# jac0626/Neighbor-Aware-Reinforcement-Learning-Fosters-Cooperation-in-Spatial-Public-Goods-Games-

Measured on NVIDIA B200. Metric: site-updates/s, higher is better.
Workload: dtype f32

## Files before the change

### neighbor-aware-reinforcement-learning-fosters-cooperation-in-spatial-public-goods-games-_b200/csrc/spgg_capi.cu

```cuda
#include "../../include/spgg.h"
#include "spgg_kernels.cuh"
#include "spgg_dispatch.h"
#include "spgg_fast.cuh"
#include "spgg_resident.cuh"

#include <cudaTypedefs.h>

#include <algorithm>
#include <cmath>
#include <cstdarg>
#include <cstdio>
#include <cstdlib>
#include <cstring>
#include <memory>
#include <string>
#include <vector>

using namespace spgg;

static thread_local std::string g_err;

static int fail(int code, const char *fmt, ...) {
  char buf[512];
  va_list ap;
  va_start(ap, fmt);
  vsnprintf(buf, sizeof(buf), fmt, ap);
  va_end(ap);
  g_err = buf;
  return code;
}

#define CUDA_TRY(expr)                                                                  \
  do {                                                                                  \
    cudaError_t e_ = (expr);                                                            \
    if (e_ != cudaSuccess)                                                              \
      return fail(SPGG_E_CUDA, "%s failed: %s (%s:%d)", #expr, cudaGetErrorString(e_),  \
                  __FILE__, __LINE__);                                                  \
  } while (0)


struct spgg_handle {
  int device = 0;
  int n_rep = 1;
  int mode = MODE_F32_I8;
  int M = 1;
  int action = 0;
  std::vector<spgg_params_t> params;
  std::vector<RepConst> rc_host;
  Geom g{};
  int threads = 256;
  int gmax_ctas = 1;
  size_t smem_step = 0, smem_gmax = 0;
  RepConst *d_rc = nullptr;
  double *d_valtab = nullptr;
  bool lean = false;
  int gmax_ctas_gen = 1;
  void *d_Qb[2] = {nullptr, nullptr};
  int qcur = 0;
  void *Qcur() const { return d_Qb[qcur]; }
  bool spec = false;
  bool carry_valid = false;
  float *d_gcarry = nullptr;
  int *d_bad = nullptr;
  CUtensorMap qmaps[2];
  bool spec_on = true;
  long long spec_launches = 0, spec_failures = 0;
  long long spec_iterations = 0;
  bool in_rerun = false;
  float *d_gvec = nullptr;
  void *peer_code[2][2] = {{nullptr, nullptr}, {nullptr, nullptr}};
  void *peer_R[2][2] = {{nullptr, nullptr}, {nullptr, nullptr}};
  uint32_t *peer_S[2][2] = {{nullptr, nullptr}, {nullptr, nullptr}};
  int peer_rows[2] = {0, 0};
  bool peer_on = false;
  std::vector<void *> ipc_opened;
  unsigned *d_ring = nullptr;
  unsigned *ring_peer[SPGG_MAX_RING] = {nullptr};
  int ring_world = 0;
  int gen = 0;
  int last_gen = -1;
  int last_rel = -1, last_upd = 0, last_spec = 0, last_sel = 0;
  int pend_qcur0 = 0;
  std::vector<char> pend_cur_after, pend_q_after;
  void *d_R[2] = {nullptr, nullptr};
  void *d_code[2] = {nullptr, nullptr};
  uint32_t *d_S[2] = {nullptr, nullptr};
  int cur = 0;
  void *d_gmax = nullptr;
  double *d_stats = nullptr;
  double *d_partials = nullptr;
  unsigned *d_tickets = nullptr;
  int *d_stop = nullptr;
  double *d_eps = nullptr;
  uint32_t *d_thr = nullptr;
  int cap = 0;
  double *d_u = nullptr;
  uint8_t *d_b = nullptr;
  uint8_t *d_sc_S = nullptr;
  double *d_sc_R = nullptr, *d_sc_Q = nullptr;
  unsigned long long *d_sc_info = nullptr;
  bool fast = false;
  bool r_wide = false;
  FastMaps fmaps[2];
  bool resident = false;
  ResGeom rgeo{};
  size_t smem_res = 0;
  bool pend_resident = false;
  bool res_grid = false;
  unsigned char *d_gimg = nullptr;
  double *d_gpart = nullptr;
  unsigned *d_gnsel = nullptr;
  int gnsel_cap = 0;
  std::vector<double> eps_host;
  std::vector<uint32_t> thr_host;
  int replay_pairs = 1;
  long long replay_first = 0, replay_n = 0;
  long long iter = 0;
  std::vector<double> eps_cur;
  std::vector<long long> stop_at;
  std::vector<char> stale;
  long long launches = 0;
  bool pending = false;
  long long pend_t0 = 0;
  int pend_n = 0, pend_cur0 = 0, pend_rel = 0;
  cudaStream_t pend_stream = nullptr;
  CclScratch ccl;
  bool ccl_valid = false;
  int64_t ccl_n = 0;
  CclStripScratch ccl_strip;
  bool ccl_local = false;
  int ccl_which = 0, ccl_flags = 0;
  int64_t ccl_local_n = 0;
  unsigned long long *d_pair_cnt = nullptr;
  uint32_t *d_pair_tail = nullptr;
  size_t pair_cnt_n = 0, pair_tail_n = 0;
  void *d_blk = nullptr;
  size_t blk_bytes = 0;
  size_t elem_code() const { return mode == MODE_F64 ? 4 : 1; }
  size_t elem_R() const { return mode == MODE_F64 ? 8 : (mode == MODE_F32_F ? 4 : 1); }
  size_t elem_Q() const { return mode == MODE_F64 ? 8 : 4; }
  size_t elem_val() const { return mode == MODE_F64 ? 8 : 4; }
  int nq() const { return params[0].algorithm == SPGG_ALGO_DOUBLE_QLEARNING ? 8 : 4; }
  ~spgg_handle();
};

static bool int8_quantum(const spgg_params_t &p, double *rq, int *gi, int *li, int *mn, int *mx) {
  for (int k = 0; k <= 4; ++k) {
    const double s = (double)(1 << k);
    const double a = p.rep_gain_C * s, b = p.delta_R_D * s, c = p.R_min * s, d = p.R_max * s;
    if (a == std::floor(a) && b == std::floor(b) && c == std::floor(c) && d == std::floor(d) &&
        std::fabs(c) <= 127 && std::fabs(d) <= 127 && std::fabs(a) <= 127 && std::fabs(b) <= 127 &&
        c - b >= -128 && d + a <= 127) {
      *rq = 1.0 / s; *gi = (int)a; *li = (int)b; *mn = (int)c; *mx = (int)d;
      return true;
    }
  }
  return false;
}

static void build_repconst(const spgg_params_t &p, RepConst *rc) {
  memset(rc, 0, sizeof(*rc));
  rc->rc = p.r * p.c;
  for (int n = 0; n < 6; ++n) rc->g[n] = rc->rc * (double)n / 5.0;
  rc->cost = p.cost;
  rc->lo = p.r - 5.0;
  rc->span = 4.0 * p.r - rc->lo;
  rc->wP = p.wP;
  rc->wR = 1.0 - p.wP;
  rc->alpha = p.alpha; rc->gamma = p.gamma; rc->kappa = p.kappa; rc->leps = p.lambda_eps;
  rc->gainC = p.rep_gain_C; rc->lossD = p.delta_R_D; rc->rmin = p.R_min; rc->rmax = p.R_max;
  rc->alpha_f = (float)p.alpha; rc->gamma_f = (float)p.gamma; rc->kappa_f = (float)p.kappa;
  rc->leps_f = (float)p.lambda_eps;
  rc->gainC_f = (float)p.rep_gain_C; rc->lossD_f = (float)p.delta_R_D;
  rc->rmin_f = (float)p.R_min; rc->rmax_f = (float)p.R_max;
  rc->rq = 1.0;
  int8_quantum(p, &rc->rq, &rc->gain_i, &rc->loss_i, &rc->rmin_i, &rc->rmax_i);
  rc->seed_lo = (uint32_t)p.seed;
  rc->seed_hi = (uint32_t)(p.seed >> 32);
  for (uint32_t r = 0; r < 10; ++r) {
    rc->pkeys[2 * r] = rc->seed_lo + r * 0x9E3779B9u;
    rc->pkeys[2 * r + 1] = rc->seed_hi + r * 0xBB67AE85u;
  }
  rc->has_ratio = (rc->wR != 0.0);
  for (int code = 0; code < 128; ++code) {
    const int sn = code >> 2, C = (code >> 1) & 1, coop = code & 1;
    const double tot = rc->rc * (double)sn / 5.0 - (C ? 5.0 * p.cost : 0.0);
    const double P = (tot - rc->lo) / rc->span;
    const double rew = rc->wP * P + rc->wR * (coop ? 0.5 : 0.0);
    rc->rewtab[code] = (float)rew;
    rc->ratiotab[code] =
        coop ? (float)(std::fabs(rc->wR * 0.5) / (std::fabs(rew) + 1e-9) * 100.0) : 0.0f;
  }
}

template <class F>
static auto with_mode(int mode, F &&f) {
  switch (mode) {
    case MODE_F32_I8: return f(ModeF32I8{});
    case MODE_F32_F: return f(ModeF32F{});
    default: return f(ModeF64{});
  }
}

static size_t step_smem(int mode, int TR) {
  return with_mode(mode, [&](auto md) { return SmemLayout<decltype(md)>(TR).total; });
}

template <class... KArgsT, class... Args>
static cudaError_t launch_pdl(void (*kern)(KArgsT...), int grid, int block, size_t smem, cudaStream_t st,
                              Args... args) {
  cudaLaunchConfig_t cfg = {};
  cfg.gridDim = dim3((unsigned)grid);
  cfg.blockDim = dim3((unsigned)block);
  cfg.dynamicSmemBytes = smem;
  cfg.stream = st;
  cudaLaunchAttribute attr[1];
  attr[0].id = cudaLaunchAttributeProgrammaticStreamSerialization;
  attr[0].val.programmaticStreamSerializationAllowed = 1;
  cfg.attrs = attr;
  cfg.numAttrs = 1;
  return cudaLaunchKernelEx(&cfg, kern, args...);
}

typedef void (*fast_fn_t)(const FastMaps, KArgs);
template <int M, bool ACTION, bool PART>
static fast_fn_t pick_fast3(int upd, int sel) {
  if (upd) return sel ? k_step_fast<M, ACTION, true, true, PART> : k_step_fast<M, ACTION, true, false, PART>;
  return k_step_fast<M, ACTION, false, true, PART>;
}
template <int M, bool ACTION>
static fast_fn_t pick_fast2(int upd, int sel, bool part) {
  return part ? pick_fast3<M, ACTION, true>(upd, sel) : pick_fast3<M, ACTION, false>(upd, sel);
}
static fast_fn_t pick_fast(int M, int action, int upd, int sel, bool part) {
  if (M == 2) return action ? pick_fast2<2, true>(upd, sel, part) : pick_fast2<2, false>(upd, sel, part);
  return action ? pick_fast2<1, true>(upd, sel, part) : pick_fast2<1, false>(upd, sel, part);
}
static size_t fast_smem(int M) { return M == 2 ? FastSmem<2>::kTotal : FastSmem<1>::kTotal; }
typedef void (*gfast_fn_t)(const CUtensorMap, GArgs);
static gfast_fn_t pick_gfast(int M) { return M == 2 ? k_gmax_fast<2> : k_gmax_fast<1>; }
static size_t gfast_smem(int M) { return M == 2 ? GmaxSmem<2>::kTotal : GmaxSmem<1>::kTotal; }

typedef void (*res_fn_t)(RArgs);
template <bool FULL>
static res_fn_t pick_res2(int M, int action) {
  if (M == 2) return action ? k_resident<2, true, FULL> : k_resident<2, false, FULL>;
  return action ? k_resident<1, true, FULL> : k_resident<1, false, FULL>;
}
static res_fn_t pick_res(int M, int action, int L) {
  return (L % 4 == 0) ? pick_res2<true>(M, action) : pick_res2<false>(M, action);
}
template <bool FULL>
static res_fn_t pick_resg2(int M, int action) {
  if (M == 2) return action ? k_resident<2, true, FULL, true> : k_resident<2, false, FULL, true>;
  return action ? k_resident<1, true, FULL, true> : k_resident<1, false, FULL, true>;
}
static res_fn_t pick_res_grid(int M, int action, int L) {
  return (L % 4 == 0) ? pick_resg2<true>(M, action) : pick_resg2<false>(M, action);
}
static ResGeom resident_geom(int L, int cs, size_t smem_limit, int grid = 0) {
  ResGeom rg{};
  rg.grid = grid;
  if (L < 2 * cs) cs = 1;
  rg.rows_max = (L + cs - 1) / cs;
  rg.prow = rg.rows_max + 4;
  rg.QR = (L + 3) / 4;
  rg.pitch = (RG + rg.QR * 4 + RG + 15) / 16 * 16;
  const int quads = rg.rows_max * rg.QR;
  rg.threads = std::max(64, std::min(RES_THREADS, (quads + 31) / 32 * 32));
  rg.CS = (ResSmem(rg).total <= smem_limit) ? cs : 0;
  return rg;
}

static PFN_cuTensorMapEncodeTiled_v12000 tensor_map_encoder() {
  static PFN_cuTensorMapEncodeTiled_v12000 encode = nullptr;
  if (!encode) {
    void *fn = nullptr;
    cudaDriverEntryPointQueryResult q;
    const cudaError_t e = cudaGetDriverEntryPoint("cuTensorMapEncodeTiled", &fn, cudaEnableDefault, &q);
    if (e != cudaSuccess || !fn || q != cudaDriverEntryPointSuccess) {
      fail(SPGG_E_CUDA, "cuTensorMapEncodeTiled not available (%s)", cudaGetErrorString(e));
      return nullptr;
    }
    encode = (PFN_cuTensorMapEncodeTiled_v12000)fn;
  }
  return encode;
}

static int make_map(CUtensorMap *map, void *base, uint64_t row_bytes, uint64_t n_rows, uint64_t n_rep,
                    uint64_t rep_stride_bytes, uint32_t box_bytes, uint32_t box_rows, uint64_t visible_bytes = 0) {
  const PFN_cuTensorMapEncodeTiled_v12000 encode = tensor_map_encoder();
  if (!encode) return SPGG_E_CUDA;
  const cuuint64_t dims[3] = {visible_bytes ? visible_bytes : row_bytes, n_rows, n_rep};
  const cuuint64_t strides[2] = {row_bytes, rep_stride_bytes};
  const cuuint32_t box[3] = {box_bytes, box_rows, 1};
  const cuuint32_t estr[3] = {1, 1, 1};
  CUresult r = encode(map, CU_TENSOR_MAP_DATA_TYPE_UINT8, 3, base, dims, strides, box, estr,
                      CU_TENSOR_MAP_INTERLEAVE_NONE, CU_TENSOR_MAP_SWIZZLE_NONE,
                      CU_TENSOR_MAP_L2_PROMOTION_L2_128B, CU_TENSOR_MAP_FLOAT_OOB_FILL_NONE);
  if (r != CUDA_SUCCESS) return fail(SPGG_E_CUDA, "cuTensorMapEncodeTiled failed (%d)", (int)r);
  return SPGG_OK;
}

static int make_map_q(CUtensorMap *map, void *base, uint64_t L, uint64_t n_rows, uint64_t n_rep) {
  const PFN_cuTensorMapEncodeTiled_v12000 encode = tensor_map_encoder();
  if (!encode) return SPGG_E_CUDA;
  const cuuint64_t dims[4] = {128, L / 8, n_rows, n_rep};
  const cuuint64_t strides[3] = {128, L * 16, n_rows * L * 16};
  const cuuint32_t box[4] = {128, TC / 8, (cuuint32_t)FastSmem<1>::kRowsPerWarp, 1};
  const cuuint32_t estr[4] = {1, 1, 1, 1};
  CUresult r = encode(map, CU_TENSOR_MAP_DATA_TYPE_UINT8, 4, base, dims, strides, box, estr,
                      CU_TENSOR_MAP_INTERLEAVE_NONE, CU_TENSOR_MAP_SWIZZLE_128B,
                      CU_TENSOR_MAP_L2_PROMOTION_L2_128B, CU_TENSOR_MAP_FLOAT_OOB_FILL_NONE);
  if (r != CUDA_SUCCESS) return fail(SPGG_E_CUDA, "cuTensorMapEncodeTiled (Q) failed (%d)", (int)r);
  return SPGG_OK;
}

extern "C" int spgg_abi_version(void) { return SPGG_ABI_VERSION; }
extern "C" const char *spgg_last_error(void) { return g_err.c_str(); }

spgg_handle::~spgg_handle() {
  for (void *p : ipc_opened) cudaIpcCloseMemHandle(p);
  cudaFree(d_rc); cudaFree(d_valtab); cudaFree(d_Qb[0]); cudaFree(d_Qb[1]); cudaFree(d_gcarry); cudaFree(d_bad); cudaFree(d_gvec); cudaFree(d_ring);
  for (int i = 0; i < 2; ++i) { cudaFree(d_R[i]); cudaFree(d_code[i]); cudaFree(d_S[i]); }
  cudaFree(d_gmax); cudaFree(d_stats); cudaFree(d_partials); cudaFree(d_tickets);
  cudaFree(d_stop); cudaFree(d_eps); cudaFree(d_thr); cudaFree(d_u); cudaFree(d_b);
  cudaFree(d_sc_S); cudaFree(d_sc_R); cudaFree(d_sc_Q); cudaFree(d_sc_info);
  cudaFree(d_gimg); cudaFree(d_gpart); cudaFree(d_gnsel);
  ccl_free(&ccl);
  ccl_strip_free(&ccl_strip);
  cudaFree(d_pair_cnt); cudaFree(d_pair_tail);
  cudaFree(d_blk);
}

extern "C" void spgg_destroy(spgg_t *h) {
  if (!h) return;
  cudaSetDevice(h->device);
  cudaDeviceSynchronize();
  delete h;
}

extern "C" int spgg_create(const spgg_params_t *params, int n_replicas, int device, spgg_t **out) {
  if (!params || !out || n_replicas < 1) return fail(SPGG_E_INVALID, "spgg_create: null argument or n_replicas < 1");
  const spgg_params_t &p0 = params[0];
  if (p0.L < 4) return fail(SPGG_E_INVALID, "L must be >= 4 (got %d)", p0.L);
  if (p0.rows < 2 * GH || p0.rows > p0.L)
    return fail(SPGG_E_INVALID, "rows must be in [%d, L] (got %d)", 2 * GH, p0.rows);
  if (p0.M != 1 && p0.M != 2) return fail(SPGG_E_INVALID, "M must be 1 or 2 (got %d)", p0.M);
  if (p0.state_mode != SPGG_STATE_REPUTATION && p0.state_mode != SPGG_STATE_ACTION)
    return fail(SPGG_E_INVALID, "Unknown state_representation code %d", p0.state_mode);
  if (p0.precision != SPGG_PREC_FP32 && p0.precision != SPGG_PREC_FP64)
    return fail(SPGG_E_INVALID, "unknown precision %d", p0.precision);
  if (p0.algorithm != SPGG_ALGO_QLEARNING && p0.algorithm != SPGG_ALGO_SARSA &&
      p0.algorithm != SPGG_ALGO_EXPECTED_SARSA && p0.algorithm != SPGG_ALGO_DOUBLE_QLEARNING)
    return fail(SPGG_E_UNSUPPORTED, "algorithm code %d is not built into the fused kernel", p0.algorithm);
  if (p0.row0 < 0 || p0.row0 + p0.rows > p0.L) return fail(SPGG_E_INVALID, "row0/rows outside the lattice");
  for (int r = 1; r < n_replicas; ++r) {
    const spgg_params_t &p = params[r];
    if (p.L != p0.L || p.rows != p0.rows || p.row0 != p0.row0 || p.M != p0.M ||
        p.state_mode != p0.state_mode || p.precision != p0.precision ||
        p.algorithm != p0.algorithm || p.r_storage != p0.r_storage)
      return fail(SPGG_E_INVALID, "replica %d differs in a batch-invariant field (L, rows, M, state, precision)", r);
  }
  int ndev = 0;
  CUDA_TRY(cudaGetDeviceCount(&ndev));
  if (device < 0 || device >= ndev) return fail(SPGG_E_CUDA, "device %d not available (%d devices)", device, ndev);
  CUDA_TRY(cudaSetDevice(device));

  std::unique_ptr<spgg_handle> hp(new spgg_handle());
  spgg_handle *h = hp.get();
  h->device = device;
  h->n_rep = n_replicas;
  h->params.assign(params, params + n_replicas);
  h->M = p0.M;
  h->action = p0.state_mode == SPGG_STATE_ACTION;
  h->rc_host.resize(n_replicas);
  bool all_i8 = true;
  for (int r = 0; r < n_replicas; ++r) {
    build_repconst(params[r], &h->rc_host[r]);
    double rq; int a, b, c, d;
    all_i8 = all_i8 && int8_quantum(params[r], &rq, &a, &b, &c, &d);
  }
  if (p0.precision == SPGG_PREC_FP64) h->mode = MODE_F64;
  else if (p0.r_storage == SPGG_RSTORE_FP32) h->mode = MODE_F32_F;
  else if (p0.r_storage == SPGG_RSTORE_INT8) {
    if (!all_i8) return fail(SPGG_E_INVALID, "reputation parameters are not representable in int8 units");
    h->mode = MODE_F32_I8;
  } else h->mode = all_i8 ? MODE_F32_I8 : MODE_F32_F;

  Geom &g = h->g;
  g.L = p0.L; g.rows = p0.rows; g.row0 = p0.row0; g.wrap_rows = (p0.rows == p0.L);
  g.pitchB = CPAD + (p0.L + 15) / 16 * 16 + CPAD;
  g.pitchW = WPAD + ((p0.L + 31) / 32 + 3) / 4 * 4 + WPAD;
  {
    bool ok = (h->mode == MODE_F32_I8) && (g.L % 32 == 0) && (g.L >= TC) && (g.rows % FTR == 0) &&
              p0.algorithm == SPGG_ALGO_QLEARNING && getenv("SPGG_NO_FAST") == nullptr;
    for (int r = 0; r < n_replicas && ok; ++r)
      ok = h->rc_host[r].rmin_i >= -15 && h->rc_host[r].rmax_i <= 15 && h->rc_host[r].gain_i >= 0 &&
           h->rc_host[r].loss_i >= 0;
    h->fast = ok;
  }
  {
    cudaDeviceProp prop0;
    CUDA_TRY(cudaGetDeviceProperties(&prop0, device));
    res_fn_t rf = pick_res(h->M, h->action, h->g.L);
    cudaFuncAttributes fa;
    CUDA_TRY(cudaFuncGetAttributes(&fa, rf));
    const size_t lim = prop0.sharedMemPerBlockOptin - fa.sharedSizeBytes - 1024;
    const bool eligible = (h->mode == MODE_F32_I8) && g.wrap_rows && p0.row0 == 0 &&
                          p0.algorithm == SPGG_ALGO_QLEARNING && getenv("SPGG_NO_RESIDENT") == nullptr;
    ResGeom rg = resident_geom(g.L, 8, lim);
    if (eligible && g.L >= 32 && (rg.CS == 0 || n_replicas <= 4) && getenv("SPGG_RES_CS8") == nullptr) {
      const ResGeom rg16 = resident_geom(g.L, 16, lim);
      if (rg16.CS == 16 &&
          cudaFuncSetAttribute(rf, cudaFuncAttributeNonPortableClusterSizeAllowed, 1) == cudaSuccess &&
          cudaFuncSetAttribute(rf, cudaFuncAttributeMaxDynamicSharedMemorySize, (int)lim) == cudaSuccess) {
        cudaLaunchConfig_t cfg = {};
        cfg.gridDim = dim3(16u * (unsigned)n_replicas);
        cfg.blockDim = dim3((unsigned)rg16.threads);
        cfg.dynamicSmemBytes = ResSmem(rg16).total;
        cudaLaunchAttribute attr[1];
        attr[0].id = cudaLaunchAttributeClusterDimension;
        attr[0].val.clusterDim.x = 16; attr[0].val.clusterDim.y = 1; attr[0].val.clusterDim.z = 1;
        cfg.attrs = attr; cfg.numAttrs = 1;
        int n_clusters = 0;
        if (cudaOccupancyMaxActiveClusters(&n_clusters, rf, &cfg) == cudaSuccess && n_clusters >= 1) rg = rg16;
      }
      (void)cudaGetLastError();
    }
    h->resident = eligible && rg.CS > 0;
    if (h->resident) {
      h->rgeo = rg;
      h->smem_res = ResSmem(rg).total;
      CUDA_TRY(cudaFuncSetAttribute(rf, cudaFuncAttributeMaxDynamicSharedMemorySize, (int)lim));
    } else if (eligible && n_replicas == 1 && getenv("SPGG_NO_RESIDENT_GRID") == nullptr) {
      res_fn_t gf = pick_res_grid(h->M, h->action, h->g.L);
      cudaFuncAttributes gfa;
      CUDA_TRY(cudaFuncGetAttributes(&gfa, gf));
      const size_t glim = prop0.sharedMemPerBlockOptin - gfa.sharedSizeBytes - 1024;
      int coop = 0;
      CUDA_TRY(cudaDeviceGetAttribute(&coop, cudaDevAttrCooperativeLaunch, device));
      const int nb_ctas = std::min(prop0.multiProcessorCount, g.L / 2);
      ResGeom gg = resident_geom(g.L, nb_ctas, glim, 1);
      if (coop && nb_ctas >= RES_RING && gg.CS == nb_ctas &&
          cudaFuncSetAttribute(gf, cudaFuncAttributeMaxDynamicSharedMemorySize, (int)glim) == cudaSuccess) {
        int occ_g = 0;
        if (cudaOccupancyMaxActiveBlocksPerMultiprocessor(&occ_g, gf, gg.threads, ResSmem(gg).total) == cudaSuccess &&
            (long long)occ_g * prop0.multiProcessorCount >= nb_ctas) {
          h->resident = true;
          h->res_grid = true;
          h->rgeo = gg;
          h->smem_res = ResSmem(gg).total;
        }
      }
      (void)cudaGetLastError();
    }
  }
  g.TR = h->fast ? FTR : (g.rows >= 512 ? 16 : (g.rows >= 64 ? 8 : 4));
  h->threads = h->fast ? FTHREADS : 32 * std::min(8, g.TR);
  g.n_tx = (g.L + TC - 1) / TC;
  g.n_ty = (g.rows + g.TR - 1) / g.TR;
  g.n_rep = n_replicas;
  g.plane_stride = (long long)(g.rows + 2 * GH) * g.pitchB;
  g.bits_stride = (long long)(g.rows + 2 * GH) * g.pitchW;
  g.site_stride = (long long)g.rows * g.L;
  h->smem_step = step_smem(h->mode, g.TR);
  h->smem_gmax = (h->elem_val() * (size_t)(g.TR + 2 * HR) * SMW + 15) / 16 * 16 + 512;

  cudaDeviceProp prop;
  CUDA_TRY(cudaGetDeviceProperties(&prop, device));
  int occ = 1;
  h->lean = !h->fast && p0.algorithm == 0 && getenv("SPGG_NO_LEAN") == nullptr;
  if (h->lean) h->smem_step = step_smem(h->mode, LEAN_TR_MAX);
  for (int replay = 0; replay < 2; ++replay) {
    step_fn_t f = pick_step(h->mode, h->M, h->action, replay);
    CUDA_TRY(cudaFuncSetAttribute(f, cudaFuncAttributeMaxDynamicSharedMemorySize, (int)h->smem_step));
    if (!replay)
      CUDA_TRY(cudaOccupancyMaxActiveBlocksPerMultiprocessor(&occ, f, h->threads, h->smem_step));
    if (h->lean) {
      step_fn_t fl = pick_lean(h->mode, h->M, h->action, replay);
      CUDA_TRY(cudaFuncSetAttribute(fl, cudaFuncAttributeMaxDynamicSharedMemorySize, (int)h->smem_step));
      if (!replay)
        CUDA_TRY(cudaOccupancyMaxActiveBlocksPerMultiprocessor(&occ, fl, h->threads, h->smem_step));
    }
  }
  if (h->fast) {
    for (int v = 0; v < 3; ++v) {
      fast_fn_t fv = pick_fast(h->M, h->action, v != 2, v != 1, g.L % TC != 0);
      CUDA_TRY(cudaFuncSetAttribute(fv, cudaFuncAttributeMaxDynamicSharedMemorySize, (int)fast_smem(h->M)));
    }
    fast_fn_t ff = pick_fast(h->M, h->action, 1, 1, g.L % TC != 0);
    CUDA_TRY(cudaOccupancyMaxActiveBlocksPerMultiprocessor(&occ, ff, FTHREADS, fast_smem(h->M)));
    CUDA_TRY(cudaFuncSetAttribute(pick_gfast(h->M), cudaFuncAttributeMaxDynamicSharedMemorySize, (int)gfast_smem(h->M)));
    int gocc = 1;
    CUDA_TRY(cudaOccupancyMaxActiveBlocksPerMultiprocessor(&gocc, pick_gfast(h->M), GWARPS * 32, gfast_smem(h->M)));
    const long long n_tiles_g = (long long)((p0.L + TC - 1) / TC) * (p0.rows / FTR);
    h->gmax_ctas = (int)std::max<long long>(1, std::min<long long>((n_tiles_g + GWARPS - 1) / GWARPS,
                       ((long long)prop.multiProcessorCount * std::max(1, gocc)) / n_replicas));
  }
  CUDA_TRY(cudaFuncSetAttribute(pick_gmax_lean(h->mode, h->M), cudaFuncAttributeMaxDynamicSharedMemorySize,
                                (int)h->smem_gmax));
  if (occ < 1) return fail(SPGG_E_CUDA, "kernel does not fit on an SM (smem %zu)", h->smem_step);
  const long long n_tiles = (long long)g.n_tx * g.n_ty;
  long long per_rep = std::max<long long>(1, ((long long)prop.multiProcessorCount * occ) / n_replicas);
  g.ctas_per_rep = (int)std::min<long long>(n_tiles, per_rep);
  {
    int gocc = 1;
    CUDA_TRY(cudaOccupancyMaxActiveBlocksPerMultiprocessor(&gocc, pick_gmax_lean(h->mode, h->M), h->threads, h->smem_gmax));
    h->gmax_ctas_gen = (int)std::min<long long>(n_tiles, std::max<long long>(1, ((long long)prop.multiProcessorCount * std::max(1, gocc)) / n_replicas));
  }
  if (h->fast && (g.site_stride / ((long long)g.ctas_per_rep * FTHREADS)) > 60000) h->fast = false;
  h->spec = h->fast && getenv("SPGG_NO_SPEC") == nullptr;

  const size_t nQ = (size_t)n_replicas * g.site_stride * h->nq() * h->elem_Q();
  const size_t nR = (size_t)n_replicas * g.plane_stride * h->elem_R();
  const size_t nC = (size_t)n_replicas * g.plane_stride * h->elem_code();
  const size_t nS = (size_t)n_replicas * g.bits_stride * 4;
#define ALLOC(ptr, bytes)                                                                   \
  do {                                                                                      \
    cudaError_t e_ = cudaMalloc((void **)&(ptr), (bytes));                                  \
    if (e_ != cudaSuccess)                                                                  \
      return fail(SPGG_E_CUDA, "cudaMalloc(%zu bytes) failed: %s", (size_t)(bytes), cudaGetErrorString(e_)); \
    cudaMemset((ptr), 0, (bytes));                                                          \
  } while (0)
  ALLOC(h->d_rc, sizeof(RepConst) * n_replicas);
  ALLOC(h->d_Qb[0], nQ);
  if (h->spec) { ALLOC(h->d_Qb[1], nQ); ALLOC(h->d_gcarry, sizeof(float) * n_replicas); ALLOC(h->d_bad, sizeof(int)); }
  for (int i = 0; i < 2; ++i) { ALLOC(h->d_R[i], nR); ALLOC(h->d_code[i], nC); ALLOC(h->d_S[i], nS); }
  ALLOC(h->d_partials, sizeof(double) * (size_t)n_replicas * g.ctas_per_rep * NSTAT);
  ALLOC(h->d_tickets, sizeof(unsigned) * n_replicas);
  ALLOC(h->d_stop, sizeof(int) * n_replicas);
  if (h->res_grid) {
    ALLOC(h->d_gimg, (size_t)h->rgeo.CS * 6 * h->rgeo.prow * h->rgeo.pitch);
    ALLOC(h->d_gpart, sizeof(double) * (size_t)RES_RING * h->rgeo.CS * RES_NRED);
  }
#undef ALLOC
  if (h->fast) {
    const int rowsCR = FTR + 2 * h->M, rowsS = FTR + 4;
    const uint64_t nrows = (uint64_t)(g.rows + 2 * GH);
    for (int i = 0; i < 2; ++i) {
      FastMaps &fm = h->fmaps[i];
      int e = make_map(&fm.ld_code, h->d_code[i], (uint64_t)g.pitchB, nrows, n_replicas, (uint64_t)g.plane_stride, FROWB, rowsCR);
      if (!e) e = make_map(&fm.ld_R, h->d_R[i], (uint64_t)g.pitchB, nrows, n_replicas, (uint64_t)g.plane_stride, FROWB, rowsCR);
      if (!e) e = make_map(&fm.ld_S, h->d_S[i], (uint64_t)g.pitchW * 4, nrows, n_replicas, (uint64_t)g.bits_stride * 4, FSROWB, rowsS);
      if (!e) e = make_map(&fm.st_code, h->d_code[i ^ 1], (uint64_t)g.pitchB, nrows, n_replicas, (uint64_t)g.plane_stride, TC, FTR, (uint64_t)(CPAD + g.L));
      if (!e) e = make_map(&fm.st_R, h->d_R[i ^ 1], (uint64_t)g.pitchB, nrows, n_replicas, (uint64_t)g.plane_stride, TC, FTR, (uint64_t)(CPAD + g.L));
      if (!e) e = make_map(&fm.st_S, h->d_S[i ^ 1], (uint64_t)g.pitchW * 4, nrows, n_replicas, (uint64_t)g.bits_stride * 4, TC / 8, FTR);
      if (!e) e = make_map_q(&h->qmaps[i], h->d_Qb[(i == 1 && h->spec) ? 1 : 0], (uint64_t)g.L, (uint64_t)g.rows, (uint64_t)n_replicas);
      if (e) return e;
    }
  }
  CUDA_TRY(cudaMemcpy(h->d_rc, h->rc_host.data(), sizeof(RepConst) * n_replicas, cudaMemcpyHostToDevice));
  if (h->mode == MODE_F64) {
    const size_t vb = sizeof(double) * 2 * ((size_t)n_replicas << VALTAB_BITS);
    if (cudaMalloc((void **)&h->d_valtab, vb) != cudaSuccess)
      return fail(SPGG_E_CUDA, "cudaMalloc(%zu bytes) failed (reward table)", vb);
    CUDA_TRY(launch_build_valtab(h->d_rc, h->d_valtab, n_replicas));
  }
  std::vector<int> neg(n_replicas, -1);
  CUDA_TRY(cudaMemcpy(h->d_stop, neg.data(), sizeof(int) * n_replicas, cudaMemcpyHostToDevice));
  if (h->spec) {
    const int none = 0x7fffffff;
    CUDA_TRY(cudaMemcpy(h->d_bad, &none, sizeof(int), cudaMemcpyHostToDevice));
  }
  h->eps_cur.resize(n_replicas);
  for (int r = 0; r < n_replicas; ++r) h->eps_cur[r] = params[r].epsilon;
  h->stop_at.assign(n_replicas, -1);
  h->stale.assign(n_replicas, 0);
  *out = hp.release();
  return SPGG_OK;
}

static int launch_step(spgg_handle *h, int do_update, int do_select, cudaStream_t st, bool allow_spec);

static int rewind_to_failed_launch(spgg_handle *h, int bad) {
  h->spec_failures += 1;
  if (h->spec_failures > 8 && h->spec_failures * 16 > h->spec_iterations) h->spec_on = false;
  const int none = 0x7fffffff;
  CUDA_TRY(cudaMemcpy(h->d_bad, &none, sizeof(int), cudaMemcpyHostToDevice));
  std::vector<int> stop(h->n_rep);
  CUDA_TRY(cudaMemcpy(stop.data(), h->d_stop, sizeof(int) * h->n_rep, cudaMemcpyDeviceToHost));
  for (int r = 0; r < h->n_rep; ++r)
    if (stop[r] == (int)(h->pend_t0 + bad) + 1) stop[r] = -1;
  CUDA_TRY(cudaMemcpy(h->d_stop, stop.data(), sizeof(int) * h->n_rep, cudaMemcpyHostToDevice));
  h->cur = h->pend_cur_after[bad - 1];
  h->qcur = h->pend_q_after[bad - 1];
  h->carry_valid = true;
  h->pend_rel = bad - 1;
  return SPGG_OK;
}

static int rerun_failed_speculation(spgg_handle *h) {
  for (;;) {
    int bad = 0x7fffffff;
    CUDA_TRY(cudaMemcpy(&bad, h->d_bad, sizeof(int), cudaMemcpyDeviceToHost));
    if (bad == 0x7fffffff) return SPGG_OK;
    if (bad < 1 || bad > h->pend_n) return fail(SPGG_E_STATE, "speculation bookkeeping out of range (%d of %d)", bad, h->pend_n);
    int rcode0 = rewind_to_failed_launch(h, bad);
    if (rcode0) return rcode0;
    h->in_rerun = true;
    const int n = h->pend_n;
    for (int s = bad; s <= n; ++s) {
      h->pend_rel += 1;
      int rcode = launch_step(h, 1, s < n ? 1 : 0, h->pend_stream, true);
      if (rcode) return rcode;
      if (!h->spec_on && s < n) {
        for (++s; s <= n; ++s) {
          rcode = spgg_phase_gmax(h, h->pend_stream);
          if (!rcode) rcode = launch_step(h, 1, s < n ? 1 : 0, h->pend_stream, false);
          if (rcode) return rcode;
        }
      }
    }
    h->in_rerun = false;
    CUDA_TRY(cudaStreamSynchronize(h->pend_stream));
    CUDA_TRY(cudaGetLastError());
  }
}

static int finish_pending(spgg_handle *h) {
  if (!h->pending) return SPGG_OK;
  CUDA_TRY(cudaSetDevice(h->device));
  CUDA_TRY(cudaStreamSynchronize(h->pend_stream));
  CUDA_TRY(cudaGetLastError());
  if (h->spec && h->g.wrap_rows && h->pend_rel == h->pend_n && !h->pend_resident) {
    int rcode = rerun_failed_speculation(h);
    if (rcode) return rcode;
  }
  std::vector<int> stop(h->n_rep);
  CUDA_TRY(cudaMemcpy(stop.data(), h->d_stop, sizeof(int) * h->n_rep, cudaMemcpyDeviceToHost));
  const long long t_end = h->pend_t0 + h->pend_rel;
  for (int r = 0; r < h->n_rep; ++r) {
    h->stop_at[r] = stop[r];
    const long long done = (stop[r] >= 0 && stop[r] < t_end) ? (long long)stop[r] : t_end;
    double e = h->eps_cur[r];
    for (long long t = h->pend_t0; t < done; ++t)
      e = std::max(e * h->params[r].epsilon_decay, h->params[r].epsilon_min);
    h->eps_cur[r] = e;
  }
  if (h->pend_resident) {
    h->iter = (h->n_rep == 1 && stop[0] >= 0 && stop[0] < t_end) ? (long long)stop[0] : t_end;
    h->pend_resident = false;
  } else if (h->n_rep == 1 && stop[0] >= 0 && stop[0] < t_end) {
    h->cur = h->pend_cur0 ^ (int)((stop[0] - h->pend_t0) & 1);
    h->qcur = h->pend_q_after[(size_t)(stop[0] - h->pend_t0)];
    h->iter = stop[0];
  } else {
    if (h->n_rep > 1) {
      for (int r = 0; r < h->n_rep; ++r) {
        if (stop[r] >= 0 && stop[r] < t_end) {
          const long long k = (long long)stop[r] - h->pend_t0;
          const int src = k >= 0 ? (h->pend_cur0 ^ (int)(k & 1)) : h->pend_cur0;
          if (src != h->cur) {
            const Geom &g = h->g;
            CUDA_TRY(cudaMemcpy((char *)h->d_R[h->cur] + (size_t)r * g.plane_stride * h->elem_R(),
                                (char *)h->d_R[src] + (size_t)r * g.plane_stride * h->elem_R(),
                                (size_t)g.plane_stride * h->elem_R(), cudaMemcpyDeviceToDevice));
            CUDA_TRY(cudaMemcpy(h->d_S[h->cur] + (size_t)r * g.bits_stride,
                                h->d_S[src] + (size_t)r * g.bits_stride,
                                (size_t)g.bits_stride * 4, cudaMemcpyDeviceToDevice));
          }
          const int qsrc = k >= 0 ? h->pend_q_after[(size_t)k] : h->pend_qcur0;
          if (qsrc != h->qcur) {
            const size_t qb = (size_t)h->g.site_stride * h->nq() * h->elem_Q();
            CUDA_TRY(cudaMemcpy((char *)h->d_Qb[h->qcur] + (size_t)r * qb, (char *)h->d_Qb[qsrc] + (size_t)r * qb, qb,
                                cudaMemcpyDeviceToDevice));
          }
        }
      }
    }
    h->iter = t_end;
  }
  h->pending = false;
  return SPGG_OK;
}

extern "C" int spgg_sync(spgg_t *h) {
  if (!h) return fail(SPGG_E_INVALID, "null handle");
  return finish_pending(h);
}

static int stage_rows(const spgg_handle *h) {
  const long long budget = 32ll << 20;
  return (int)std::max<long long>(1, std::min<long long>(h->g.rows, budget / h->g.L));
}

static int ensure_scratch(spgg_handle *h, bool want_q) {
  const size_t n = (size_t)stage_rows(h) * h->g.L;
  if (!h->d_sc_S) {
    CUDA_TRY(cudaMalloc((void **)&h->d_sc_S, n));
    CUDA_TRY(cudaMalloc((void **)&h->d_sc_R, n * sizeof(double)));
    CUDA_TRY(cudaMalloc((void **)&h->d_sc_info, 3 * sizeof(unsigned long long)));
  }
  if (want_q && !h->d_sc_Q) CUDA_TRY(cudaMalloc((void **)&h->d_sc_Q, n * h->nq() * sizeof(double)));
  return SPGG_OK;
}

static void begin_new_run(spgg_handle *h, int rep) {
  if (h->iter != 0) {
    h->iter = 0;
    std::fill(h->stale.begin(), h->stale.end(), 1);
  }
  h->stale[rep] = 0;
  h->carry_valid = false;
  if (h->d_ring) {
    cudaMemset(h->d_ring, 0, sizeof(unsigned) * RING_SLOTS * RING_WORDS);
    h->gen = 0;
    h->last_gen = -1;
  }
}

extern "C" int spgg_set_state(spgg_t *h, int rep, const uint8_t *S, const double *R, const double *Q) {
  if (!h || !S || !R || !Q) return fail(SPGG_E_INVALID, "spgg_set_state: null argument");
  if (rep < 0 || rep >= h->n_rep) return fail(SPGG_E_INVALID, "replica %d out of range", rep);
  int rcode = finish_pending(h);
  if (rcode) return rcode;
  h->ccl_valid = h->ccl_local = false;
  CUDA_TRY(cudaSetDevice(h->device));
  rcode = ensure_scratch(h, true);
  if (rcode) return rcode;
  const Geom &g = h->g;
  const RepConst &rc = h->rc_host[rep];
  CUDA_TRY(cudaMemset(h->d_sc_info, 0, 3 * sizeof(unsigned long long)));
  const int chunk = stage_rows(h);
  for (int i0 = 0; i0 < g.rows; i0 += chunk) {
    const int nr = std::min(chunk, g.rows - i0);
    const size_t n = (size_t)nr * g.L, off = (size_t)i0 * g.L;
    CUDA_TRY(cudaMemcpyAsync(h->d_sc_S, S + off, n, cudaMemcpyHostToDevice, 0));
    CUDA_TRY(cudaMemcpyAsync(h->d_sc_R, R + off, n * sizeof(double), cudaMemcpyHostToDevice, 0));
    CUDA_TRY(cudaMemcpyAsync(h->d_sc_Q, Q + off * h->nq(), n * h->nq() * sizeof(double), cudaMemcpyHostToDevice, 0));
    const int grid = (int)std::min<long long>(148 * 16, ((long long)nr * ((g.L + 31) / 32) * 32 + 255) / 256);
    with_mode(h->mode, [&](auto md) {
      k_import_rows<decltype(md)><<<std::max(1, grid), 256>>>(g, rep, i0, nr, h->d_sc_S, h->d_sc_R, h->d_sc_Q,
          h->Qcur(), h->d_R[h->cur], h->d_S[h->cur], rc.rq, h->d_sc_info, h->nq());
    });
    CUDA_TRY(cudaGetLastError());
    h->launches += 1;
  }
  unsigned long long info[3];
  CUDA_TRY(cudaMemcpy(info, h->d_sc_info, sizeof(info), cudaMemcpyDeviceToHost));
  if (info[0] == 1) return fail(SPGG_E_INVALID, "strategy array holds values other than 0/1");
  if (info[0] == 2)
    return fail(SPGG_E_INVALID, "R is not representable in int8 units of %g; use r_storage=FP32", rc.rq);
  if (info[2] && h->fast) {
    if (!g.wrap_rows)
      return fail(SPGG_E_INVALID, "R outside [%g, %g] (int8 units -16..15 of %g): a strip on the fast path "
                  "cannot hold it", -16.0 * rc.rq, 15.0 * rc.rq, rc.rq);
    h->r_wide = true;
  }
  begin_new_run(h, rep);
  h->eps_cur[rep] = h->params[rep].epsilon;
  int stop = -1;
  if (g.wrap_rows && (info[1] == 0 || info[1] == (unsigned long long)g.site_stride))
    stop = (int)h->iter;
  h->stop_at[rep] = stop;
  CUDA_TRY(cudaMemcpy(h->d_stop + rep, &stop, sizeof(int), cudaMemcpyHostToDevice));
  return SPGG_OK;
}

extern "C" int spgg_get_state(spgg_t *h, int rep, uint8_t *S, double *R, double *Q) {
  if (!h) return fail(SPGG_E_INVALID, "null handle");
  if (rep < 0 || rep >= h->n_rep) return fail(SPGG_E_INVALID, "replica %d out of range", rep);
  int rcode = finish_pending(h);
  if (rcode) return rcode;
  CUDA_TRY(cudaSetDevice(h->device));
  rcode = ensure_scratch(h, Q != nullptr);
  if (rcode) return rcode;
  const Geom &g = h->g;
  const RepConst &rc = h->rc_host[rep];
  const int chunk = stage_rows(h);
  for (int i0 = 0; i0 < g.rows; i0 += chunk) {
    const int nr = std::min(chunk, g.rows - i0);
    const size_t n = (size_t)nr * g.L, off = (size_t)i0 * g.L;
    const int grid = (int)std::min<long long>(148 * 16, ((long long)n + 255) / 256);
    with_mode(h->mode, [&](auto md) {
      k_export_rows<decltype(md)><<<std::max(1, grid), 256>>>(g, rep, i0, nr, S ? h->d_sc_S : nullptr,
          R ? h->d_sc_R : nullptr, Q ? h->d_sc_Q : nullptr, h->Qcur(), h->d_R[h->cur], h->d_S[h->cur], rc.rq, h->nq());
    });
    CUDA_TRY(cudaGetLastError());
    h->launches += 1;
    if (S) CUDA_TRY(cudaMemcpyAsync(S + off, h->d_sc_S, n, cudaMemcpyDeviceToHost, 0));
    if (R) CUDA_TRY(cudaMemcpyAsync(R + off, h->d_sc_R, n * sizeof(double), cudaMemcpyDeviceToHost, 0));
    if (Q) CUDA_TRY(cudaMemcpyAsync(Q + off * h->nq(), h->d_sc_Q, n * h->nq() * sizeof(double), cudaMemcpyDeviceToHost, 0));
    CUDA_TRY(cudaStreamSynchronize(0));
  }
  return SPGG_OK;
}

extern "C" int spgg_set_replay(spgg_t *h, int n_steps, const double *u, const uint8_t *b) {
  return spgg_set_replay_pairs(h, n_steps, 1, u, b);
}

extern "C" int spgg_set_replay_pairs(spgg_t *h, int n_steps, int n_pairs, const double *u, const uint8_t *b) {
  if (!h) return fail(SPGG_E_INVALID, "null handle");
  const int want_pairs = h->params[0].algorithm == SPGG_ALGO_SARSA ? 3
                         : (h->params[0].algorithm == SPGG_ALGO_DOUBLE_QLEARNING ? 2 : 1);
  if (n_steps > 0 && n_pairs != want_pairs)
    return fail(SPGG_E_INVALID, "this TD rule consumes %d draw pair(s) per iteration, got %d", want_pairs, n_pairs);
  if (h->n_rep != 1) return fail(SPGG_E_UNSUPPORTED, "replay draws are supported for a single replica");
  int rcode = finish_pending(h);
  if (rcode) return rcode;
  CUDA_TRY(cudaSetDevice(h->device));
  cudaFree(h->d_u); cudaFree(h->d_b);
  h->d_u = nullptr; h->d_b = nullptr; h->replay_n = 0;
  if (n_steps <= 0) return SPGG_OK;
  if (!u || !b) return fail(SPGG_E_INVALID, "spgg_set_replay: null draw arrays");
  const size_t n = (size_t)n_steps * n_pairs * h->g.site_stride;
  h->replay_pairs = n_pairs;
  CUDA_TRY(cudaMalloc((void **)&h->d_u, n * sizeof(double)));
  CUDA_TRY(cudaMalloc((void **)&h->d_b, n));
  CUDA_TRY(cudaMemcpy(h->d_u, u, n * sizeof(double), cudaMemcpyHostToDevice));
  CUDA_TRY(cudaMemcpy(h->d_b, b, n, cudaMemcpyHostToDevice));
  h->replay_first = h->iter;
  h->replay_n = n_steps;
  return SPGG_OK;
}

static int ensure_tables(spgg_handle *h, int n_steps) {
  const int need = n_steps + 1;
  if (need <= h->cap) return SPGG_OK;
  cudaFree(h->d_gmax); cudaFree(h->d_stats); cudaFree(h->d_eps); cudaFree(h->d_thr); cudaFree(h->d_gvec);
  h->d_gmax = nullptr; h->d_stats = nullptr; h->d_eps = nullptr; h->d_thr = nullptr; h->d_gvec = nullptr;
  h->cap = 0;
  CUDA_TRY(cudaMalloc(&h->d_gmax, h->elem_val() * (size_t)h->n_rep * need));
  CUDA_TRY(cudaMalloc((void **)&h->d_stats, sizeof(double) * (size_t)h->n_rep * need * NSTAT));
  CUDA_TRY(cudaMalloc((void **)&h->d_eps, sizeof(double) * (size_t)h->n_rep * (need + 1)));
  CUDA_TRY(cudaMalloc((void **)&h->d_thr, sizeof(uint32_t) * (size_t)h->n_rep * (need + 1)));
  if (h->spec && !h->g.wrap_rows) CUDA_TRY(cudaMalloc((void **)&h->d_gvec, sizeof(float) * 4 * (size_t)need));
  h->cap = need;
  return SPGG_OK;
}

static uint32_t thr24(double eps) {
  double t = std::ceil(eps * 16777216.0);
  if (t < 0) t = 0;
  if (t > 16777216.0) t = 16777216.0;
  return (uint32_t)t;
}

extern "C" int spgg_begin_steps(spgg_t *h, int n_steps, void *stream_) {
  if (!h) return fail(SPGG_E_INVALID, "null handle");
  if (n_steps < 1) return fail(SPGG_E_INVALID, "n_steps must be >= 1");
  int rcode = finish_pending(h);
  if (rcode) return rcode;
  h->ccl_valid = h->ccl_local = false;
  for (int r = 0; r < h->n_rep; ++r)
    if (h->stale[r])
      return fail(SPGG_E_STATE, "replica %d still holds the state of the previous run: give every replica of a "
                                "batch a state (spgg_set_state / spgg_init_random) before stepping", r);
  CUDA_TRY(cudaSetDevice(h->device));
  cudaStream_t st = (cudaStream_t)stream_;
  rcode = ensure_tables(h, n_steps);
  if (rcode) return rcode;
  std::vector<double> &eps = h->eps_host;
  std::vector<uint32_t> &thr = h->thr_host;
  eps.assign((size_t)(h->cap + 1) * h->n_rep, 0.0);
  thr.assign(eps.size(), 0u);
  for (int r = 0; r < h->n_rep; ++r) {
    double e = h->eps_cur[r];
    for (int idx = 1; idx <= n_steps + 1 && idx <= h->cap; ++idx) {
      eps[(size_t)idx * h->n_rep + r] = e;
      thr[(size_t)idx * h->n_rep + r] = thr24(e);
      e = std::max(e * h->params[r].epsilon_decay, h->params[r].epsilon_min);
    }
  }
  CUDA_TRY(cudaMemcpyAsync(h->d_eps, eps.data(), eps.size() * sizeof(double), cudaMemcpyHostToDevice, st));
  CUDA_TRY(cudaMemcpyAsync(h->d_thr, thr.data(), thr.size() * sizeof(uint32_t), cudaMemcpyHostToDevice, st));
  CUDA_TRY(cudaMemsetAsync(h->d_gmax, 0, h->elem_val() * (size_t)h->n_rep * h->cap, st));
  CUDA_TRY(cudaMemsetAsync(h->d_stats, 0, sizeof(double) * (size_t)h->n_rep * h->cap * NSTAT, st));
  if (h->d_gvec) CUDA_TRY(cudaMemsetAsync(h->d_gvec, 0, sizeof(float) * 4 * (size_t)h->cap, st));
  h->pending = true;
  h->pend_t0 = h->iter;
  h->pend_n = n_steps;
  h->pend_cur0 = h->cur;
  h->pend_qcur0 = h->qcur;
  h->in_rerun = false;
  h->pend_cur_after.assign((size_t)n_steps + 1, (char)h->cur);
  h->pend_q_after.assign((size_t)n_steps + 1, (char)h->qcur);
  h->pend_rel = 0;
  h->pend_stream = st;
  return SPGG_OK;
}

static bool launch_replays(const spgg_handle *h, long long j, int do_select) {
  const long long draw = j - h->replay_first;
  return do_select && h->d_u && draw >= 0 && draw < h->replay_n;
}
static bool can_speculate(const spgg_handle *h, int do_select) {
  return h->fast && h->spec && h->spec_on && h->carry_valid &&
         !launch_replays(h, h->pend_t0 + h->pend_rel + 1, do_select);
}

static int launch_step(spgg_handle *h, int do_update, int do_select, cudaStream_t st, bool allow_spec) {
  const long long j = h->pend_t0 + h->pend_rel;
  const long long draw = j - h->replay_first;
  const bool replay = launch_replays(h, j, do_select);
  KArgs a;
  a.g = h->g;
  a.rc = h->d_rc;
  a.Q = h->Qcur();
  a.R_in = h->d_R[h->cur]; a.R_out = h->d_R[h->cur ^ 1];
  a.code_in = h->d_code[h->cur]; a.code_out = h->d_code[h->cur ^ 1];
  a.S_in = h->d_S[h->cur]; a.S_out = h->d_S[h->cur ^ 1];
  a.gmax = h->d_gmax; a.stats = h->d_stats; a.partials = h->d_partials;
  a.valtab = h->d_valtab;
  a.tickets = h->d_tickets; a.stop_at = h->d_stop;
  a.eps_tab = h->d_eps; a.thr_tab = h->d_thr;
  const size_t np_ = (size_t)h->replay_pairs, ss = (size_t)h->g.site_stride;
  a.u = replay ? h->d_u + (size_t)draw * np_ * ss : nullptr;
  a.b = replay ? h->d_b + (size_t)draw * np_ * ss : nullptr;
  a.algo = h->params[0].algorithm;
  const long long ue = j - 1 - h->replay_first;
  const bool upd_replay = do_update && np_ >= 2 && h->d_u && ue >= 0 && ue < h->replay_n;
  a.u2 = upd_replay ? h->d_u + ((size_t)ue * np_ + 1) * ss : nullptr;
  a.b2 = upd_replay ? h->d_b + ((size_t)ue * np_ + 1) * ss : nullptr;
  a.u3 = (upd_replay && np_ == 3) ? h->d_u + ((size_t)ue * 3 + 2) * ss : nullptr;
  a.b3 = (upd_replay && np_ == 3) ? h->d_b + ((size_t)ue * 3 + 2) * ss : nullptr;
  a.j = (int)j; a.rel = h->pend_rel; a.cap = h->cap;
  a.do_update = do_update; a.do_select = do_select;
  const bool use_fast = h->fast && !replay && !(do_select && h->r_wide);
  a.spec = 0; a.gcarry = nullptr; a.bad_at = nullptr; a.gvec = nullptr;
  for (int d = 0; d < 2; ++d) {
    const bool on = h->peer_on && use_fast && do_select;
    a.peer_code[d] = on ? h->peer_code[d][h->cur ^ 1] : nullptr;
    a.peer_R[d] = on ? h->peer_R[d][h->cur ^ 1] : nullptr;
    a.peer_S[d] = on ? h->peer_S[d][h->cur ^ 1] : nullptr;
    a.peer_rows[d] = h->peer_rows[d];
  }
  a.ring_world = 0; a.gen = 0;
  for (int p = 0; p < SPGG_MAX_RING; ++p) a.ring_peer[p] = nullptr;
  if (h->ring_world > 0 && use_fast && h->d_gvec && (do_update || do_select)) {
    a.ring_world = h->ring_world;
    a.gen = h->gen;
    for (int p = 0; p < h->ring_world; ++p) a.ring_peer[p] = h->ring_peer[p];
  }
  if (use_fast && h->spec && !h->g.wrap_rows && h->n_rep == 1) a.gvec = h->d_gvec;
  if (use_fast && h->spec) {
    a.gcarry = h->d_gcarry;
    a.bad_at = h->d_bad;
    a.spec = (allow_spec && do_update && h->spec_on && h->carry_valid) ? 1 : 0;
  }
#ifdef SPGG_TRACE
  {
    static unsigned long long *d_trace = nullptr;
    static int n_dump = 0;
    const int n_cta = h->g.ctas_per_rep * h->n_rep;
    if (!d_trace) { cudaMalloc(&d_trace, sizeof(unsigned long long) * 4 * 65536); cudaMemset(d_trace, 0, sizeof(unsigned long long) * 4 * 65536); }
    else if (getenv("SPGG_TRACE_FILE") && n_dump < 3 && do_update && do_select) {
      std::vector<unsigned long long> t(4 * (size_t)n_cta);
      cudaDeviceSynchronize();
      cudaMemcpy(t.data(), d_trace, t.size() * 8, cudaMemcpyDeviceToHost);
      char name[256]; snprintf(name, sizeof(name), "%s.%d", getenv("SPGG_TRACE_FILE"), n_dump++);
      FILE *f = fopen(name, "wb"); if (f) { fwrite(t.data(), 8, t.size(), f); fclose(f); }
    }
    a.trace = d_trace;
  }
#endif
  if (use_fast) {
    if (!do_update && !do_select) return SPGG_OK;
    fast_fn_t ff = pick_fast(h->M, h->action, do_update, do_select, h->g.L % TC != 0);
    FastMaps fm = h->fmaps[h->cur];
    const int q_out = (do_update && h->spec) ? (h->qcur ^ 1) : h->qcur;
    fm.q_ld = h->qmaps[h->qcur];
    fm.q_st = h->qmaps[q_out];
    if (a.spec) {
      static const int poison = getenv("SPGG_SPEC_TEST_POISON") ? atoi(getenv("SPGG_SPEC_TEST_POISON")) : 0;
      if (poison > 0 && !h->in_rerun && h->spec_launches % poison == poison - 1) a.spec = 2;
    }
    CUDA_TRY(launch_pdl(ff, h->g.ctas_per_rep * h->n_rep, FTHREADS, fast_smem(h->M), st, fm, a));
    h->qcur = q_out;
    if (do_update) {
      h->carry_valid = h->spec;
      if (a.spec) {
        h->spec_launches += 1;
        if (!h->in_rerun) h->spec_iterations += 1;
      }
    }
  } else {
    if (do_update) h->carry_valid = false;
    step_fn_t f = (h->lean && do_update) ? pick_lean(h->mode, h->M, h->action, replay ? 1 : 0)
                                          : pick_step(h->mode, h->M, h->action, replay ? 1 : 0);
    const int grid = h->g.ctas_per_rep * h->n_rep;
    if ((long long)h->g.n_tx * h->g.n_ty * h->n_rep <= 160) CUDA_TRY(launch_pdl(f, grid, h->threads, h->smem_step, st, a));
    else f<<<grid, h->threads, h->smem_step, st>>>(a);
  }
  CUDA_TRY(cudaGetLastError());
  h->launches += 1;
  h->last_rel = h->pend_rel; h->last_upd = do_update; h->last_spec = a.spec; h->last_sel = do_select;
  h->last_gen = a.ring_world > 0 ? h->gen++ : -1;
  if (do_select) {
    h->cur ^= 1;
    h->r_wide = false;
  }
  if (h->pend_rel >= 0 && h->pend_rel < (int)h->pend_cur_after.size()) {
    h->pend_cur_after[h->pend_rel] = (char)h->cur;
    h->pend_q_after[h->pend_rel] = (char)h->qcur;
  }
  return SPGG_OK;
}

extern "C" int spgg_phase_kernel(spgg_t *h, int do_update, int do_select, void *stream_) {
  if (!h || !h->pending) return fail(SPGG_E_STATE, "spgg_phase_kernel outside begin/end");
  return launch_step(h, do_update, do_select, (cudaStream_t)stream_, false);
}

extern "C" int spgg_phase_iteration(spgg_t *h, int do_select, void *stream_) {
  if (!h || !h->pending) return fail(SPGG_E_STATE, "spgg_phase_iteration outside begin/end");
  if (h->pend_rel >= h->pend_n) return fail(SPGG_E_STATE, "the chunk announced to spgg_begin_steps is complete");
  int rcode = SPGG_OK;
  if (can_speculate(h, do_select)) h->pend_rel += 1;
  else rcode = spgg_phase_gmax(h, stream_);
  if (!rcode) rcode = launch_step(h, 1, do_select, (cudaStream_t)stream_, true);
  return rcode;
}

extern "C" int spgg_phase_gmax(spgg_t *h, void *stream_) {
  if (!h || !h->pending) return fail(SPGG_E_STATE, "spgg_phase_gmax outside begin/end");
  cudaStream_t st = (cudaStream_t)stream_;
  h->pend_rel += 1;
  GArgs a;
  a.g = h->g;
  a.rc = h->d_rc;
  a.code_in = h->d_code[h->cur];
  a.gmax = h->d_gmax;
  a.valtab = h->d_valtab;
  a.stop_at = h->d_stop;
  a.j = (int)(h->pend_t0 + h->pend_rel); a.rel = h->pend_rel; a.cap = h->cap;
  if (h->fast) {
    CUDA_TRY(launch_pdl(pick_gfast(h->M), h->gmax_ctas * h->n_rep, GWARPS * 32, gfast_smem(h->M), st,
                        h->fmaps[h->cur].ld_code, a));
  } else {
    gmax_fn_t f = pick_gmax_lean(h->mode, h->M);
    a.g.ctas_per_rep = h->gmax_ctas_gen;
    const int grid = h->gmax_ctas_gen * h->n_rep;
    if ((long long)h->g.n_tx * h->g.n_ty * h->n_rep <= 160) CUDA_TRY(launch_pdl(f, grid, h->threads, h->smem_gmax, st, a));
    else f<<<grid, h->threads, h->smem_gmax, st>>>(a);
  }
  CUDA_TRY(cudaGetLastError());
  h->launches += 1;
  return SPGG_OK;
}

extern "C" void *spgg_gmax_device_ptr(spgg_t *h) {
  if (!h || !h->pending) return nullptr;
  return (char *)h->d_gmax + h->elem_val() * (size_t)h->pend_rel;
}

extern "C" int spgg_end_steps(spgg_t *h, void *stream_) {
  (void)stream_;
  if (!h || !h->pending) return fail(SPGG_E_STATE, "spgg_end_steps without spgg_begin_steps");
  return SPGG_OK;
}

static int resident_chunk(spgg_handle *h, int n_steps, cudaStream_t st) {
  RArgs a;
  a.g = h->g;
  a.rg = h->rgeo;
  a.rc = h->d_rc;
  a.Q = h->Qcur();
  a.R = h->d_R[h->cur];
  a.S = h->d_S[h->cur];
  a.stats = h->d_stats;
  a.stop_at = h->d_stop;
  a.thr_tab = h->d_thr;
  a.t0 = (int)h->pend_t0;
  a.n_steps = n_steps;
  a.cap = h->cap;
#ifdef SPGG_RES_TRACE
  {
    static long long *d_tr = nullptr;
    const int n_cta = h->rgeo.CS * h->n_rep;
    if (!d_tr) { cudaMalloc(&d_tr, sizeof(long long) * 8 * 4096); cudaMemset(d_tr, 0, sizeof(long long) * 8 * 4096); }
    else if (getenv("SPGG_RES_TRACE_PRINT")) {
      std::vector<long long> t(8 * (size_t)n_cta);
      cudaDeviceSynchronize();
      cudaMemcpy(t.data(), d_tr, t.size() * 8, cudaMemcpyDeviceToHost);
      for (int c = 0; c < std::min(n_cta, 16); ++c) {
        fprintf(stderr, "res_trace cta %2d:", c);
        for (int z = 0; z < 7; ++z) fprintf(stderr, " %10lld", t[(size_t)c * 8 + z]);
        fprintf(stderr, "\n");
      }
    }
    a.trace = d_tr;
  }
#endif
  a.gimg = h->d_gimg;
  a.gpart = h->d_gpart;
  a.gnsel = nullptr;
  a.gmaxtab = reinterpret_cast<float *>(h->d_gmax);
  cudaLaunchConfig_t cfg = {};
  cfg.gridDim = dim3((unsigned)(h->rgeo.CS * h->n_rep));
  cfg.blockDim = dim3((unsigned)h->rgeo.threads);
  cfg.dynamicSmemBytes = h->smem_res;
  cfg.stream = st;
  cudaLaunchAttribute attr[1];
  cfg.attrs = attr;
  cfg.numAttrs = 1;
  if (h->res_grid) {
    if (h->gnsel_cap < h->cap) {
      cudaFree(h->d_gnsel);
      h->d_gnsel = nullptr; h->gnsel_cap = 0;
      CUDA_TRY(cudaMalloc((void **)&h->d_gnsel, sizeof(unsigned) * (size_t)h->cap));
      h->gnsel_cap = h->cap;
    }
    CUDA_TRY(cudaMemsetAsync(h->d_gnsel, 0, sizeof(unsigned) * (size_t)h->cap, st));
    a.gnsel = h->d_gnsel;
    attr[0].id = cudaLaunchAttributeCooperative;
    attr[0].val.cooperative = 1;
    CUDA_TRY(cudaLaunchKernelEx(&cfg, pick_res_grid(h->M, h->action, h->g.L), a));
  } else {
    attr[0].id = cudaLaunchAttributeClusterDimension;
    attr[0].val.clusterDim.x = (unsigned)h->rgeo.CS;
    attr[0].val.clusterDim.y = 1;
    attr[0].val.clusterDim.z = 1;
    CUDA_TRY(cudaLaunchKernelEx(&cfg, pick_res(h->M, h->action, h->g.L), a));
  }
  {
    const int n_rows = n_steps + 1, total = n_rows * h->n_rep;
    k_resident_rows<<<(total + 127) / 128, 128, 0, st>>>(h->d_rc, h->d_stats, h->n_rep, h->cap, n_rows);
    CUDA_TRY(cudaGetLastError());
  }
  h->launches += 2;
  h->pend_rel = n_steps;
  h->pend_resident = true;
  return SPGG_OK;
}

extern "C" int spgg_step(spgg_t *h, int n_steps, void *stream_) {
  int rcode = spgg_begin_steps(h, n_steps, stream_);
  if (rcode) return rcode;
  if (h->resident && !h->d_u) {
    rcode = resident_chunk(h, n_steps, (cudaStream_t)stream_);
    if (rcode) return rcode;
    return spgg_end_steps(h, stream_);
  }
  rcode = spgg_phase_kernel(h, 0, 1, stream_);
  for (int s = 1; s <= n_steps && !rcode; ++s) rcode = spgg_phase_iteration(h, s < n_steps ? 1 : 0, stream_);
  if (rcode) return rcode;
  return spgg_end_steps(h, stream_);
}

extern "C" int spgg_get_stats(spgg_t *h, int rep, int first, int n, double *rows_out) {
  if (!h || !rows_out) return fail(SPGG_E_INVALID, "spgg_get_stats: null argument");
  if (rep < 0 || rep >= h->n_rep) return fail(SPGG_E_INVALID, "replica %d out of range", rep);
  int rcode = finish_pending(h);
  if (rcode) return rcode;
  if (first < 0 || n < 0 || first + n > h->cap) return fail(SPGG_E_INVALID, "rows [%d,%d) outside the last chunk (%d rows)", first, first + n, h->cap);
  CUDA_TRY(cudaSetDevice(h->device));
  CUDA_TRY(cudaMemcpy(rows_out, h->d_stats + ((size_t)rep * h->cap + first) * NSTAT,
                      sizeof(double) * (size_t)n * NSTAT, cudaMemcpyDeviceToHost));
  return SPGG_OK;
}

extern "C" int spgg_query(spgg_t *h, int rep, spgg_status_t *out) {
  if (!h || !out) return fail(SPGG_E_INVALID, "spgg_query: null argument");
  if (rep < 0 || rep >= h->n_rep) return fail(SPGG_E_INVALID, "replica %d out of range", rep);
  int rcode = finish_pending(h);
  if (rcode) return rcode;
  out->iteration = (h->stop_at[rep] >= 0 && h->stop_at[rep] < h->iter) ? h->stop_at[rep] : h->iter;
  out->stopped_at = h->stop_at[rep];
  out->epsilon = h->eps_cur[rep];
  out->n_replicas = h->n_rep;
  out->r_is_int8 = h->mode == MODE_F32_I8;
  out->kernel_launches = h->launches;
  out->speculative_launches = h->spec_launches;
  out->speculation_failures = h->spec_failures;
  return SPGG_OK;
}

extern "C" int spgg_describe(spgg_t *h, char *buf, int n) {
  if (!h) return fail(SPGG_E_INVALID, "null handle");
  char tmp[256];
  const char *arith = h->mode == MODE_F64 ? "fp64 Q and R" : (h->mode == MODE_F32_F ? "fp32 Q, fp32 R" : "fp32 Q, int8 R");
  int len;
  if (h->resident && h->res_grid)
    len = snprintf(tmp, sizeof(tmp), "resident: cooperative grid of %d CTAs x %d threads, %zu KB shared memory per CTA, "
                   "ghost rows through L2 (%s)", h->rgeo.CS, h->rgeo.threads, h->smem_res >> 10, arith);
  else if (h->resident)
    len = snprintf(tmp, sizeof(tmp), "resident: cluster of %d CTAs x %d threads per replica, %zu KB shared memory per CTA, "
                   "ghost rows through DSMEM (%s)", h->rgeo.CS, h->rgeo.threads, h->smem_res >> 10, arith);
  else if (h->fast)
    len = snprintf(tmp, sizeof(tmp), "fast: TMA-staged %dx%d tiles, %d persistent CTAs per replica, %s (%s)",
                   FTR, TC, h->g.ctas_per_rep,
                   (h->spec && h->spec_on) ? "one launch per iteration (speculative global maximum, verified)"
                                           : "two launches per iteration (k_gmax_fast + k_step_fast)", arith);
  else
    len = snprintf(tmp, sizeof(tmp), "general: %dx%d tiles, %d CTAs per replica, two launches per iteration (k_gmax_lean + %s) (%s)", h->g.TR, TC,
                   h->g.ctas_per_rep, h->lean ? "k_step_lean" : "k_step", arith);
  if (buf && n > 0) {
    strncpy(buf, tmp, (size_t)n - 1);
    buf[n - 1] = 0;
  }
  return len + 1;
}

extern "C" int spgg_init_random(spgg_t *h, int rep, uint64_t seed) {
  if (!h) return fail(SPGG_E_INVALID, "null handle");
  if (rep < 0 || rep >= h->n_rep) return fail(SPGG_E_INVALID, "replica %d out of range", rep);
  int rcode = finish_pending(h);
  if (rcode) return rcode;
  h->ccl_valid = h->ccl_local = false;
  CUDA_TRY(cudaSetDevice(h->device));
  const uint32_t lo = (uint32_t)seed, hi = (uint32_t)(seed >> 32);
  const int grid = 148 * 8;
  with_mode(h->mode, [&](auto md) {
    k_init_random<decltype(md)><<<grid, 256>>>(h->g, rep, h->Qcur(), h->d_R[h->cur], h->d_S[h->cur], lo, hi, h->nq());
  });
  CUDA_TRY(cudaGetLastError());
  CUDA_TRY(cudaDeviceSynchronize());
  h->launches += 1;
  begin_new_run(h, rep);
  h->eps_cur[rep] = h->params[rep].epsilon;
  int stop = -1;
  h->stop_at[rep] = -1;
  CUDA_TRY(cudaMemcpy(h->d_stop + rep, &stop, sizeof(int), cudaMemcpyHostToDevice));
  return SPGG_OK;
}

extern "C" int spgg_set_progress(spgg_t *h, int64_t iteration, const double *epsilon) {
  if (!h || !epsilon) return fail(SPGG_E_INVALID, "spgg_set_progress: null argument");
  if (iteration < 0 || iteration > 0x7fffffff - (1 << 20))
    return fail(SPGG_E_INVALID, "iteration %lld outside the 31-bit Philox counter word", (long long)iteration);
  int rcode = finish_pending(h);
  if (rcode) return rcode;
  for (int r = 0; r < h->n_rep; ++r) {
    if (h->stale[r]) return fail(SPGG_E_STATE, "replica %d has no state of the run being resumed", r);
    if (!(epsilon[r] >= 0.0 && epsilon[r] <= 1.0)) return fail(SPGG_E_INVALID, "epsilon[%d] = %g outside [0, 1]", r, epsilon[r]);
  }
  if (h->iter != 0) return fail(SPGG_E_STATE, "spgg_set_progress follows the state uploads of a resumed run");
  h->ccl_valid = h->ccl_local = false;
  CUDA_TRY(cudaSetDevice(h->device));
  h->iter = (long long)iteration;
  h->replay_first = h->iter;
  for (int r = 0; r < h->n_rep; ++r) {
    h->eps_cur[r] = epsilon[r];
    if (h->stop_at[r] >= 0) h->stop_at[r] = h->iter;
  }
  std::vector<int> stop(h->stop_at.begin(), h->stop_at.end());
  CUDA_TRY(cudaMemcpy(h->d_stop, stop.data(), sizeof(int) * h->n_rep, cudaMemcpyHostToDevice));
  return SPGG_OK;
}

extern "C" int spgg_state_digest(spgg_t *h, int rep, uint64_t out[3]) {
  if (!h || !out) return fail(SPGG_E_INVALID, "spgg_state_digest: null argument");
  if (rep < 0 || rep >= h->n_rep) return fail(SPGG_E_INVALID, "replica %d out of range", rep);
  int rcode = finish_pending(h);
  if (rcode) return rcode;
  CUDA_TRY(cudaSetDevice(h->device));
  unsigned long long *d_out = nullptr;
  CUDA_TRY(cudaMalloc((void **)&d_out, 3 * sizeof(unsigned long long)));
  CUDA_TRY(cudaMemset(d_out, 0, 3 * sizeof(unsigned long long)));
  const int grid = 148 * 8;
  const double rq = h->rc_host[rep].rq;
  with_mode(h->mode, [&](auto md) {
    k_state_digest<decltype(md)><<<grid, 256>>>(h->g, rep, h->Qcur(), h->d_R[h->cur], h->d_S[h->cur], h->nq(), rq, d_out);
  });
  cudaError_t e = cudaGetLastError();
  if (e == cudaSuccess) e = cudaMemcpy(out, d_out, 3 * sizeof(unsigned long long), cudaMemcpyDeviceToHost);
  cudaFree(d_out);
  if (e != cudaSuccess) return fail(SPGG_E_CUDA, "spgg_state_digest: %s", cudaGetErrorString(e));
  h->launches += 1;
  return SPGG_OK;
}

extern "C" int spgg_r_histogram(spgg_t *h, int rep, int n_bins, const double *edges, int64_t *counts) {
  if (!h || !edges || !counts) return fail(SPGG_E_INVALID, "spgg_r_histogram: null argument");
  if (rep < 0 || rep >= h->n_rep) return fail(SPGG_E_INVALID, "replica %d out of range", rep);
  if (n_bins < 1 || n_bins > 64) return fail(SPGG_E_INVALID, "n_bins must be in [1, 64] (got %d)", n_bins);
  int rcode = finish_pending(h);
  if (rcode) return rcode;
  CUDA_TRY(cudaSetDevice(h->device));
  double *d_edges = nullptr;
  unsigned long long *d_cnt = nullptr;
  CUDA_TRY(cudaMalloc((void **)&d_edges, sizeof(double) * 65));
  if (cudaMalloc((void **)&d_cnt, sizeof(unsigned long long) * 64) != cudaSuccess) { cudaFree(d_edges); return fail(SPGG_E_CUDA, "cudaMalloc failed"); }
  cudaMemcpy(d_edges, edges, sizeof(double) * (n_bins + 1), cudaMemcpyHostToDevice);
  cudaMemset(d_cnt, 0, sizeof(unsigned long long) * 64);
  const double rq = h->rc_host[rep].rq;
  const int grid = 148 * 8;
  with_mode(h->mode, [&](auto md) {
    k_r_histogram<decltype(md)><<<grid, 256>>>(h->g, rep, h->d_R[h->cur], rq, n_bins, d_edges, d_cnt);
  });
  unsigned long long host_cnt[64];
  cudaError_t e = cudaGetLastError();
  if (e == cudaSuccess) e = cudaMemcpy(host_cnt, d_cnt, sizeof(unsigned long long) * 64, cudaMemcpyDeviceToHost);
  cudaFree(d_edges); cudaFree(d_cnt);
  if (e != cudaSuccess) return fail(SPGG_E_CUDA, "spgg_r_histogram: %s", cudaGetErrorString(e));
  for (int i = 0; i < n_bins; ++i) counts[i] = (int64_t)host_cnt[i];
  h->launches += 1;
  return SPGG_OK;
}

extern "C" int spgg_clusters(spgg_t *h, int rep, int which, int flags, int64_t *n_clusters) {
  if (!h || !n_clusters) return fail(SPGG_E_INVALID, "spgg_clusters: null argument");
  if (rep < 0 || rep >= h->n_rep) return fail(SPGG_E_INVALID, "replica %d out of range", rep);
  if (which != 0 && which != 1) return fail(SPGG_E_INVALID, "which must be 0 (cooperators) or 1 (defectors), got %d", which);
  if (flags & ~SPGG_CLUSTER_PERIODIC) return fail(SPGG_E_INVALID, "unknown cluster flags 0x%x", flags);
  if (!h->g.wrap_rows) return fail(SPGG_E_UNSUPPORTED, "cluster labelling needs the whole lattice (rows == L), not a strip");
  if ((long long)h->g.rows * h->g.L >= (1ll << 31)) return fail(SPGG_E_UNSUPPORTED, "cluster labelling needs rows*L < 2^31");
  int rcode = finish_pending(h);
  if (rcode) return rcode;
  h->ccl_valid = h->ccl_local = false;
  CUDA_TRY(cudaSetDevice(h->device));
  cudaError_t e = ccl_alloc(&h->ccl, h->g.rows, h->g.L);
  if (e != cudaSuccess) {
    (void)cudaGetLastError();
    return fail(SPGG_E_CUDA, "spgg_clusters: scratch for L=%d: %s", h->g.L, cudaGetErrorString(e));
  }
  const Geom &g = h->g;
  const uint32_t *S = h->d_S[h->cur] + (size_t)rep * g.bits_stride + (size_t)GH * g.pitchW + WPAD;
  int64_t n = 0;
  e = launch_clusters(h->ccl, S, g.pitchW, which, flags & SPGG_CLUSTER_PERIODIC, &n);
  if (e != cudaSuccess) return fail(SPGG_E_CUDA, "spgg_clusters: %s", cudaGetErrorString(e));
  h->launches += 5;
  h->ccl.base = 0;
  h->ccl_n = n;
  h->ccl_valid = true;
  *n_clusters = n;
  return SPGG_OK;
}

extern "C" int spgg_cluster_sizes(spgg_t *h, int64_t *sizes, int64_t n) {
  if (!h || !sizes) return fail(SPGG_E_INVALID, "spgg_cluster_sizes: null argument");
  if (!h->ccl_valid) return fail(SPGG_E_STATE, "spgg_cluster_sizes: no spgg_clusters result for the current state");
  if (n != h->ccl_n) return fail(SPGG_E_INVALID, "spgg_cluster_sizes: n = %lld, the labelling found %lld clusters", (long long)n, (long long)h->ccl_n);
  CUDA_TRY(cudaSetDevice(h->device));
  if (n > 0) CUDA_TRY(cudaMemcpy(sizes, h->ccl.sizes, sizeof(int64_t) * (size_t)n, cudaMemcpyDeviceToHost));
  return SPGG_OK;
}

extern "C" int spgg_cluster_labels(spgg_t *h, int32_t *labels) {
  if (!h || !labels) return fail(SPGG_E_INVALID, "spgg_cluster_labels: null argument");
  if (!h->ccl_valid) return fail(SPGG_E_STATE, "spgg_cluster_labels: no spgg_clusters result for the current state");
  CUDA_TRY(cudaSetDevice(h->device));
  cudaError_t e = launch_cluster_labels(h->ccl);
  if (e == cudaSuccess)
    e = cudaMemcpy(labels, h->ccl.total, sizeof(int32_t) * (size_t)h->g.rows * h->g.L, cudaMemcpyDeviceToHost);
  if (e != cudaSuccess) return fail(SPGG_E_CUDA, "spgg_cluster_labels: %s", cudaGetErrorString(e));
  h->launches += 1;
  return SPGG_OK;
}

static int strip_clusters_supported(spgg_t *h, const char *fn) {
  if (h->n_rep != 1) return fail(SPGG_E_UNSUPPORTED, "%s: strip labelling serves single-replica handles", fn);
  if ((long long)h->g.L * h->g.L >= (1ll << 31))
    return fail(SPGG_E_UNSUPPORTED, "%s: global site indices need L*L < 2^31 (L=%d)", fn, h->g.L);
  return SPGG_OK;
}

extern "C" int64_t spgg_strip_cluster_record_bytes(spgg_t *h) {
  if (!h) return fail(SPGG_E_INVALID, "null handle");
  int rcode = strip_clusters_supported(h, "spgg_strip_cluster_record_bytes");
  return rcode ? rcode : ccl_record_bytes(h->g.L);
}

extern "C" int spgg_strip_clusters(spgg_t *h, int which, int flags, void *dev_record) {
  if (!h || !dev_record) return fail(SPGG_E_INVALID, "spgg_strip_clusters: null argument");
  if (which != 0 && which != 1) return fail(SPGG_E_INVALID, "which must be 0 (cooperators) or 1 (defectors), got %d", which);
  if (flags & ~SPGG_CLUSTER_PERIODIC) return fail(SPGG_E_INVALID, "unknown cluster flags 0x%x", flags);
  int rcode = strip_clusters_supported(h, "spgg_strip_clusters");
  if (rcode) return rcode;
  rcode = finish_pending(h);
  if (rcode) return rcode;
  h->ccl_valid = h->ccl_local = false;
  CUDA_TRY(cudaSetDevice(h->device));
  const Geom &g = h->g;
  cudaError_t e = ccl_alloc(&h->ccl, g.rows, g.L);
  if (e == cudaSuccess) e = ccl_strip_alloc(&h->ccl_strip, g.L, 0);
  if (e != cudaSuccess) {
    (void)cudaGetLastError();
    return fail(SPGG_E_CUDA, "spgg_strip_clusters: scratch for %d x %d sites: %s", g.rows, g.L, cudaGetErrorString(e));
  }
  const uint32_t *S = h->d_S[h->cur] + (size_t)GH * g.pitchW + WPAD;
  e = launch_strip_clusters(h->ccl, h->ccl_strip, S, g.pitchW, g.row0, which, flags & SPGG_CLUSTER_PERIODIC, dev_record,
                            &h->ccl_local_n);
  if (e != cudaSuccess) return fail(SPGG_E_CUDA, "spgg_strip_clusters: %s", cudaGetErrorString(e));
  h->launches += 9;
  h->ccl_local = true;
  h->ccl_which = which;
  h->ccl_flags = flags;
  return SPGG_OK;
}

extern "C" int spgg_strip_clusters_resolve(spgg_t *h, int world, int rank, const void *dev_records, int64_t *n_owned,
                                           int64_t *first_label, int64_t *n_total) {
  if (!h || !dev_records || !n_owned || !first_label || !n_total)
    return fail(SPGG_E_INVALID, "spgg_strip_clusters_resolve: null argument");
  if (world < 1 || rank < 0 || rank >= world) return fail(SPGG_E_INVALID, "rank %d outside a world of %d", rank, world);
  if (!h->ccl_local) return fail(SPGG_E_STATE, "spgg_strip_clusters_resolve: no spgg_strip_clusters pass of the current state");
  const Geom &g = h->g;
  const long long rb = ccl_record_bytes(g.L);
  std::vector<int> hd((size_t)world * CCL_REC_HDR);
  CUDA_TRY(cudaSetDevice(h->device));
  CUDA_TRY(cudaMemcpy2D(hd.data(), CCL_REC_HDR * sizeof(int), dev_records, (size_t)rb, CCL_REC_HDR * sizeof(int), world,
                        cudaMemcpyDeviceToHost));
  int next = 0;
  for (int k = 0; k < world; ++k) {
    const int *r = hd.data() + (size_t)k * CCL_REC_HDR;
    if (r[CCL_H_MAGIC] != CCL_REC_MAGIC) return fail(SPGG_E_INVALID, "record %d is not a strip cluster record", k);
    if (r[CCL_H_L] != g.L) return fail(SPGG_E_INVALID, "record %d: L = %d, this handle's L = %d", k, r[CCL_H_L], g.L);
    if (r[CCL_H_WHICH] != h->ccl_which || r[CCL_H_FLAGS] != h->ccl_flags)
      return fail(SPGG_E_INVALID, "record %d: which %d / flags 0x%x, this strip labelled which %d / flags 0x%x", k,
                  r[CCL_H_WHICH], r[CCL_H_FLAGS], h->ccl_which, h->ccl_flags);
    if (r[CCL_H_ROW0] != next || r[CCL_H_ROWS] < 1 || r[CCL_H_ROWS] > g.L - next)
      return fail(SPGG_E_INVALID, "record %d: rows [%d, %d) do not continue the strips above at row %d", k, r[CCL_H_ROW0],
                  r[CCL_H_ROW0] + r[CCL_H_ROWS], next);
    if (r[CCL_H_NPARTS] < 0 || r[CCL_H_NPARTS] > 2 * g.L || r[CCL_H_NLOCAL] < r[CCL_H_NPARTS])
      return fail(SPGG_E_INVALID, "record %d: %d boundary roots of %d roots", k, r[CCL_H_NPARTS], r[CCL_H_NLOCAL]);
    next += r[CCL_H_ROWS];
  }
  if (next != g.L) return fail(SPGG_E_INVALID, "the %d records cover rows [0, %d) of %d", world, next, g.L);
  const int *mine = hd.data() + (size_t)rank * CCL_REC_HDR;
  if (mine[CCL_H_ROW0] != g.row0 || mine[CCL_H_ROWS] != g.rows || mine[CCL_H_NLOCAL] != h->ccl_local_n)
    return fail(SPGG_E_INVALID, "record %d is not this strip's (rows [%d, %d))", rank, g.row0, g.row0 + g.rows);
  cudaError_t e = ccl_strip_alloc(&h->ccl_strip, g.L, world);
  if (e != cudaSuccess) {
    (void)cudaGetLastError();
    return fail(SPGG_E_CUDA, "spgg_strip_clusters_resolve: scratch for %d records: %s", world, cudaGetErrorString(e));
  }
  h->ccl_local = false;
  e = launch_strip_resolve(h->ccl, h->ccl_strip, dev_records, world, rank, h->ccl_flags & SPGG_CLUSTER_PERIODIC, n_owned,
                           first_label, n_total);
  if (e != cudaSuccess) return fail(SPGG_E_CUDA, "spgg_strip_clusters_resolve: %s", cudaGetErrorString(e));
  h->launches += 10;
  h->ccl_n = *n_owned;
  h->ccl_valid = true;
  return SPGG_OK;
}

static int pair_max_d(spgg_t *h, int max_d, const char *fn) {
  if (max_d < 1 || max_d > h->g.L / 2) return fail(SPGG_E_INVALID, "%s: max_d = %d outside [1, L/2 = %d]", fn, max_d, h->g.L / 2);
  return SPGG_OK;
}

static int pair_scratch(spgg_handle *h, int max_d, size_t tail_words) {
  const size_t n = 4 * (size_t)(max_d + 1);
  if (h->pair_cnt_n < n) {
    cudaFree(h->d_pair_cnt);
    h->d_pair_cnt = nullptr;
    h->pair_cnt_n = 0;
    CUDA_TRY(cudaMalloc((void **)&h->d_pair_cnt, n * sizeof(unsigned long long)));
    h->pair_cnt_n = n;
  }
  if (h->pair_tail_n < tail_words) {
    cudaFree(h->d_pair_tail);
    h->d_pair_tail = nullptr;
    h->pair_tail_n = 0;
    CUDA_TRY(cudaMalloc((void **)&h->d_pair_tail, tail_words * sizeof(uint32_t)));
    h->pair_tail_n = tail_words;
  }
  return SPGG_OK;
}

static const uint32_t *pair_plane(const spgg_handle *h, int rep) {
  const Geom &g = h->g;
  return h->d_S[h->cur] + (size_t)rep * g.bits_stride + (size_t)GH * g.pitchW + WPAD;
}

extern "C" int spgg_pair_counts(spgg_t *h, int rep, int max_d, int64_t *out) {
  if (!h || !out) return fail(SPGG_E_INVALID, "spgg_pair_counts: null argument");
  if (rep < 0 || rep >= h->n_rep) return fail(SPGG_E_INVALID, "replica %d out of range", rep);
  if (!h->g.wrap_rows)
    return fail(SPGG_E_UNSUPPORTED, "spgg_pair_counts needs the whole lattice (rows == L), not a strip: see spgg_strip_pair_counts");
  int rcode = pair_max_d(h, max_d, "spgg_pair_counts");
  if (rcode) return rcode;
  rcode = finish_pending(h);
  if (rcode) return rcode;
  CUDA_TRY(cudaSetDevice(h->device));
  rcode = pair_scratch(h, max_d, 0);
  if (rcode) return rcode;
  const Geom &g = h->g;
  const uint32_t *S = pair_plane(h, rep);
  cudaError_t e = launch_pair_counts(S, g.pitchW, g.rows, g.L, S, g.pitchW, max_d, h->d_pair_cnt, out);
  if (e != cudaSuccess) return fail(SPGG_E_CUDA, "spgg_pair_counts: %s", cudaGetErrorString(e));
  h->launches += 2;
  return SPGG_OK;
}

static int strip_pairs_supported(spgg_t *h, int max_d, int max_rows, const char *fn) {
  if (h->n_rep != 1) return fail(SPGG_E_UNSUPPORTED, "%s: strip pair counts serve single-replica handles", fn);
  int rcode = pair_max_d(h, max_d, fn);
  if (rcode) return rcode;
  if (max_rows < std::min(max_d, h->g.rows) || max_rows > max_d)
    return fail(SPGG_E_INVALID, "%s: max_rows = %d outside [min(max_d, rows) = %d, max_d = %d]", fn, max_rows,
                std::min(max_d, h->g.rows), max_d);
  return SPGG_OK;
}

extern "C" int64_t spgg_strip_pair_record_bytes(spgg_t *h, int max_d, int max_rows) {
  if (!h) return fail(SPGG_E_INVALID, "null handle");
  int rcode = strip_pairs_supported(h, max_d, max_rows, "spgg_strip_pair_record_bytes");
  return rcode ? rcode : pair_record_bytes(h->g.L, max_rows);
}

extern "C" int spgg_strip_pair_record(spgg_t *h, int max_d, int max_rows, void *dev_record) {
  if (!h || !dev_record) return fail(SPGG_E_INVALID, "spgg_strip_pair_record: null argument");
  int rcode = strip_pairs_supported(h, max_d, max_rows, "spgg_strip_pair_record");
  if (rcode) return rcode;
  rcode = finish_pending(h);
  if (rcode) return rcode;
  CUDA_TRY(cudaSetDevice(h->device));
  const Geom &g = h->g;
  cudaError_t e = launch_pair_record(pair_plane(h, 0), g.pitchW, g.row0, g.rows, g.L, max_d, max_rows, dev_record);
  if (e == cudaSuccess) e = cudaStreamSynchronize(0);
  if (e != cudaSuccess) return fail(SPGG_E_CUDA, "spgg_strip_pair_record: %s", cudaGetErrorString(e));
  h->launches += 1;
  return SPGG_OK;
}

extern "C" int spgg_strip_pair_counts(spgg_t *h, int world, int rank, const void *dev_records, int max_d, int max_rows,
                                      int64_t *out) {
  if (!h || !dev_records || !out) return fail(SPGG_E_INVALID, "spgg_strip_pair_counts: null argument");
  if (world < 1 || rank < 0 || rank >= world) return fail(SPGG_E_INVALID, "rank %d outside a world of %d", rank, world);
  int rcode = strip_pairs_supported(h, max_d, max_rows, "spgg_strip_pair_counts");
  if (rcode) return rcode;
  const Geom &g = h->g;
  const long long rb = pair_record_bytes(g.L, max_rows);
  std::vector<int> hd((size_t)world * PAIR_REC_HDR);
  CUDA_TRY(cudaSetDevice(h->device));
  for (int k = 0; k < world; ++k)
    CUDA_TRY(cudaMemcpy(hd.data() + (size_t)k * PAIR_REC_HDR, (const char *)dev_records + k * rb, PAIR_REC_HDR * sizeof(int),
                        cudaMemcpyDeviceToHost));
  int next = 0;
  for (int k = 0; k < world; ++k) {
    const int *r = hd.data() + (size_t)k * PAIR_REC_HDR;
    if (r[PAIR_H_MAGIC] != PAIR_REC_MAGIC) return fail(SPGG_E_INVALID, "record %d is not a strip pair record", k);
    if (r[PAIR_H_L] != g.L) return fail(SPGG_E_INVALID, "record %d: L = %d, this handle's L = %d", k, r[PAIR_H_L], g.L);
    if (r[PAIR_H_MAXD] != max_d || r[PAIR_H_MAXROWS] != max_rows)
      return fail(SPGG_E_INVALID, "record %d: max_d %d / max_rows %d, this call's max_d %d / max_rows %d", k, r[PAIR_H_MAXD],
                  r[PAIR_H_MAXROWS], max_d, max_rows);
    if (r[PAIR_H_ROW0] != next || r[PAIR_H_ROWS] < 1 || r[PAIR_H_ROWS] > g.L - next)
      return fail(SPGG_E_INVALID, "record %d: rows [%d, %d) do not continue the strips above at row %d", k, r[PAIR_H_ROW0],
                  r[PAIR_H_ROW0] + r[PAIR_H_ROWS], next);
    if (r[PAIR_H_NROWS] != std::min(max_d, r[PAIR_H_ROWS]) || r[PAIR_H_NROWS] > max_rows)
      return fail(SPGG_E_INVALID, "record %d holds %d rows, not min(max_d, rows) = %d within max_rows = %d", k,
                  r[PAIR_H_NROWS], std::min(max_d, r[PAIR_H_ROWS]), max_rows);
    next += r[PAIR_H_ROWS];
  }
  if (next != g.L) return fail(SPGG_E_INVALID, "the %d records cover rows [0, %d) of %d", world, next, g.L);
  const int *mine = hd.data() + (size_t)rank * PAIR_REC_HDR;
  if (mine[PAIR_H_ROW0] != g.row0 || mine[PAIR_H_ROWS] != g.rows)
    return fail(SPGG_E_INVALID, "record %d is not this strip's (rows [%d, %d))", rank, g.row0, g.row0 + g.rows);
  rcode = finish_pending(h);
  if (rcode) return rcode;
  const int nW = (g.L + 31) / 32;
  rcode = pair_scratch(h, max_d, (size_t)max_d * nW);
  if (rcode) return rcode;
  for (int t = 0, k = (rank + 1) % world; t < max_d; k = (k + 1) % world) {
    const int n = std::min(hd[(size_t)k * PAIR_REC_HDR + PAIR_H_NROWS], max_d - t);
    CUDA_TRY(cudaMemcpy(h->d_pair_tail + (size_t)t * nW, (const char *)dev_records + k * rb + PAIR_REC_HDR * sizeof(int),
                        (size_t)n * nW * sizeof(uint32_t), cudaMemcpyDeviceToDevice));
    t += n;
  }
  cudaError_t e = launch_pair_counts(pair_plane(h, 0), g.pitchW, g.rows, g.L, h->d_pair_tail, nW, max_d, h->d_pair_cnt, out);
  if (e != cudaSuccess) return fail(SPGG_E_CUDA, "spgg_strip_pair_counts: %s", cudaGetErrorString(e));
  h->launches += 2;
  return SPGG_OK;
}

extern "C" int spgg_block_fields(spgg_t *h, int rep, int b, int flags, int64_t *counts, double *sums) {
  if (!h || !counts || (flags && !sums)) return fail(SPGG_E_INVALID, "spgg_block_fields: null argument");
  if (rep < 0 || rep >= h->n_rep) return fail(SPGG_E_INVALID, "replica %d out of range", rep);
  if (flags & ~(SPGG_BLOCK_R | SPGG_BLOCK_Q)) return fail(SPGG_E_INVALID, "spgg_block_fields: unknown flags 0x%x", flags);
  const Geom &g = h->g;
  if (b < 1 || b > g.L) return fail(SPGG_E_INVALID, "spgg_block_fields: b = %d outside [1, L = %d]", b, g.L);
  const long long B = (g.L + b - 1) / b;
  if (B * B > BLK_MAX_BLOCKS)
    return fail(SPGG_E_INVALID, "spgg_block_fields: %lld x %lld blocks exceed 2^24 (b = %d, L = %d)", B, B, b, g.L);
  int rcode = finish_pending(h);
  if (rcode) return rcode;
  CUDA_TRY(cudaSetDevice(h->device));
  const bool want_r = flags & SPGG_BLOCK_R, want_q = flags & SPGG_BLOCK_Q;
  const BlockGeom q = block_geom(g.L, g.row0, g.rows, b);
  const size_t need = block_scratch_bytes(q, (want_r ? 1 : 0) + (want_q ? h->nq() : 0));
  if (h->blk_bytes < need) {
    cudaFree(h->d_blk);
    h->d_blk = nullptr;
    h->blk_bytes = 0;
    CUDA_TRY(cudaMalloc(&h->d_blk, need));
    h->blk_bytes = need;
  }
  const uint32_t *S = h->d_S[h->cur] + (size_t)rep * g.bits_stride + (size_t)GH * g.pitchW + WPAD;
  const void *R = (const char *)h->d_R[h->cur] + ((size_t)rep * g.plane_stride + (size_t)GH * g.pitchB + CPAD) * h->elem_R();
  const void *Q = (const char *)h->Qcur() + (size_t)rep * g.site_stride * h->nq() * h->elem_Q();
  const double rq = h->rc_host[rep].rq;
  const cudaError_t e = with_mode(h->mode, [&](auto md) {
    return launch_block_fields<decltype(md)>(q, g.pitchW, g.pitchB, S, R, Q, rq, h->nq(), want_r, want_q, h->d_blk,
                                             counts, sums);
  });
  if (e != cudaSuccess) return fail(SPGG_E_CUDA, "spgg_block_fields: %s", cudaGetErrorString(e));
  h->launches += flags ? 2 + (q.nrc * q.ncs > 1) : 1;
  return SPGG_OK;
}

extern "C" int spgg_ipc_export(spgg_t *h, unsigned char *handles ) {
  if (!h || !handles) return fail(SPGG_E_INVALID, "spgg_ipc_export: null argument");
  static_assert(sizeof(cudaIpcMemHandle_t) == 64, "IPC handle size");
  CUDA_TRY(cudaSetDevice(h->device));
  void *ptrs[6] = {h->d_code[0], h->d_code[1], h->d_R[0], h->d_R[1], h->d_S[0], h->d_S[1]};
  for (int i = 0; i < 6; ++i) {
    cudaIpcMemHandle_t hd;
    CUDA_TRY(cudaIpcGetMemHandle(&hd, ptrs[i]));
    memcpy(handles + 64 * i, &hd, 64);
  }
  return SPGG_OK;
}

extern "C" int spgg_ipc_attach(spgg_t *h, int which, const unsigned char *handles, int peer_rows, int same_as_other) {
  if (!h || (which != 0 && which != 1)) return fail(SPGG_E_INVALID, "spgg_ipc_attach: bad argument");
  if (!h->fast || h->n_rep != 1 || h->g.wrap_rows) return fail(SPGG_E_UNSUPPORTED, "peer-mapped halos serve single-replica strips on the TMA fast path");
  int rcode = finish_pending(h);
  if (rcode) return rcode;
  CUDA_TRY(cudaSetDevice(h->device));
  void *ptrs[6];
  if (same_as_other) {
    const int o = which ^ 1;
    ptrs[0] = h->peer_code[o][0]; ptrs[1] = h->peer_code[o][1]; ptrs[2] = h->peer_R[o][0];
    ptrs[3] = h->peer_R[o][1]; ptrs[4] = h->peer_S[o][0]; ptrs[5] = h->peer_S[o][1];
    if (!ptrs[0]) return fail(SPGG_E_STATE, "the other neighbour is not attached yet");
  } else {
    if (!handles) return fail(SPGG_E_INVALID, "spgg_ipc_attach: null handles");
    for (int i = 0; i < 6; ++i) {
      cudaIpcMemHandle_t hd;
      memcpy(&hd, handles + 64 * i, 64);
      cudaError_t e = cudaIpcOpenMemHandle(&ptrs[i], hd, cudaIpcMemLazyEnablePeerAccess);
      if (e != cudaSuccess) {
        (void)cudaGetLastError();
        return fail(SPGG_E_CUDA, "cudaIpcOpenMemHandle failed: %s", cudaGetErrorString(e));
      }
      h->ipc_opened.push_back(ptrs[i]);
    }
  }
  h->peer_code[which][0] = ptrs[0]; h->peer_code[which][1] = ptrs[1];
  h->peer_R[which][0] = ptrs[2]; h->peer_R[which][1] = ptrs[3];
  h->peer_S[which][0] = (uint32_t *)ptrs[4]; h->peer_S[which][1] = (uint32_t *)ptrs[5];
  h->peer_rows[which] = peer_rows;
  h->peer_on = h->peer_code[0][0] != nullptr && h->peer_code[1][0] != nullptr;
  return SPGG_OK;
}

extern "C" int spgg_ring_export(spgg_t *h, unsigned char *handle64) {
  if (!h || !handle64) return fail(SPGG_E_INVALID, "spgg_ring_export: null argument");
  CUDA_TRY(cudaSetDevice(h->device));
  if (!h->d_ring) {
    CUDA_TRY(cudaMalloc((void **)&h->d_ring, 2 << 20));
    CUDA_TRY(cudaMemset(h->d_ring, 0, 2 << 20));
  }
  cudaIpcMemHandle_t hd;
  CUDA_TRY(cudaIpcGetMemHandle(&hd, h->d_ring));
  memcpy(handle64, &hd, 64);
  return SPGG_OK;
}

extern "C" int spgg_ring_attach(spgg_t *h, int world, int rank, const unsigned char *handles ) {
  if (!h || !handles || world < 2 || world > SPGG_MAX_RING || rank < 0 || rank >= world)
    return fail(SPGG_E_INVALID, "spgg_ring_attach: bad argument (world %d, at most %d)", world, SPGG_MAX_RING);
  if (!h->d_ring || !h->peer_on) return fail(SPGG_E_STATE, "spgg_ring_attach follows spgg_ring_export and the neighbours' spgg_ipc_attach");
  CUDA_TRY(cudaSetDevice(h->device));
  for (int p = 0; p < world; ++p) {
    if (p == rank) { h->ring_peer[p] = h->d_ring; continue; }
    cudaIpcMemHandle_t hd;
    memcpy(&hd, handles + 64 * p, 64);
    void *ptr = nullptr;
    cudaError_t e = cudaIpcOpenMemHandle(&ptr, hd, cudaIpcMemLazyEnablePeerAccess);
    if (e != cudaSuccess) {
      (void)cudaGetLastError();
      h->ring_world = 0;
      return fail(SPGG_E_CUDA, "cudaIpcOpenMemHandle (ring of rank %d) failed: %s", p, cudaGetErrorString(e));
    }
    h->ipc_opened.push_back(ptr);
    h->ring_peer[p] = (unsigned *)ptr;
  }
  h->ring_world = world;
  h->gen = 0;
  return SPGG_OK;
}

extern "C" int spgg_strip_can_speculate(spgg_t *h, int do_select) {
  return (h && h->pending && h->d_gvec && h->n_rep == 1 && can_speculate(h, do_select)) ? 1 : 0;
}

extern "C" int spgg_strip_iteration(spgg_t *h, int do_select, void *stream_) {
  if (!h || !h->pending) return fail(SPGG_E_STATE, "spgg_strip_iteration outside begin/end");
  if (!spgg_strip_can_speculate(h, do_select)) return fail(SPGG_E_STATE, "this strip cannot guess the maximum now: run the exact pair");
  h->pend_rel += 1;
  return launch_step(h, 1, do_select, (cudaStream_t)stream_, true);
}

extern "C" void *spgg_strip_report_ptr(spgg_t *h) {
  if (!h || !h->pending || !h->d_gvec || h->last_rel < 0) return nullptr;
  return h->d_gvec + 4 * (size_t)h->last_rel;
}

extern "C" int spgg_strip_verify(spgg_t *h, void *stream_) {
  if (!h || !h->pending || !h->d_gvec || h->last_rel < 0) return fail(SPGG_E_STATE, "spgg_strip_verify: no strip launch to verify");
  if (h->last_gen >= 0)
    k_ring_verify<<<1, 32, 0, (cudaStream_t)stream_>>>(h->d_ring, h->last_gen, h->ring_world, h->d_gvec, h->last_rel,
                                                      (int)(h->pend_t0 + h->last_rel), h->last_upd, h->last_spec, h->last_sel,
                                                      h->d_gcarry, reinterpret_cast<float *>(h->d_gmax), h->d_bad, h->d_stop);
  else
    k_strip_verify<<<1, 32, 0, (cudaStream_t)stream_>>>(h->d_gvec, h->last_rel, (int)(h->pend_t0 + h->last_rel), h->last_upd,
                                                         h->last_spec, h->last_sel, h->d_gcarry,
                                                         reinterpret_cast<float *>(h->d_gmax), h->d_bad, h->d_stop);
  CUDA_TRY(cudaGetLastError());
  h->launches += 1;
  if (h->last_upd) h->carry_valid = true;
  return SPGG_OK;
}

extern "C" int spgg_strip_failed(spgg_t *h) {
  if (!h || !h->d_bad) return 0;
  int bad = 0x7fffffff;
  if (cudaMemcpy(&bad, h->d_bad, sizeof(int), cudaMemcpyDeviceToHost) != cudaSuccess) return fail(SPGG_E_CUDA, "spgg_strip_failed: copy failed");
  return bad == 0x7fffffff ? 0 : bad;
}

extern "C" int spgg_strip_rewind(spgg_t *h, int bad) {
  if (!h || !h->pending || !h->d_bad) return fail(SPGG_E_STATE, "spgg_strip_rewind outside a chunk");
  if (bad < 1 || bad > h->pend_n) return fail(SPGG_E_INVALID, "launch %d outside the chunk of %d", bad, h->pend_n);
  h->in_rerun = true;
  h->ccl_valid = h->ccl_local = false;
  if (h->d_ring) {
    CUDA_TRY(cudaMemset(h->d_ring, 0, sizeof(unsigned) * RING_SLOTS * RING_WORDS));
    h->gen = 0;
    h->last_gen = -1;
  }
  return rewind_to_failed_launch(h, bad);
}

extern "C" int64_t spgg_halo_bytes(spgg_t *h) {
  if (!h) return 0;
  const Geom &g = h->g;
  const int64_t per_rep = (int64_t)GH * g.pitchB * (int64_t)(h->elem_code() + h->elem_R()) + (int64_t)GH * g.pitchW * 4;
  return per_rep * h->n_rep;
}

extern "C" int spgg_halo_pack(spgg_t *h, void *to_up, void *to_down, void *stream_) {
  if (!h || !to_up || !to_down) return fail(SPGG_E_INVALID, "spgg_halo_pack: null argument");
  cudaStream_t st = (cudaStream_t)stream_;
  const long long rep_bytes = spgg_halo_bytes(h) / h->n_rep;
  const dim3 grid(std::max(1, std::min(64, (GH * h->g.pitchB + 255) / 256)), h->n_rep);
  with_mode(h->mode, [&](auto md) {
    k_halo_pack<decltype(md)><<<grid, 256, 0, st>>>(h->g, h->d_code[h->cur], h->d_R[h->cur], h->d_S[h->cur],
        (unsigned char *)to_up, (unsigned char *)to_down, rep_bytes);
  });
  CUDA_TRY(cudaGetLastError());
  h->launches += 1;
  return SPGG_OK;
}

extern "C" int spgg_halo_unpack(spgg_t *h, const void *from_up, const void *from_down, void *stream_) {
  if (!h || !from_up || !from_down) return fail(SPGG_E_INVALID, "spgg_halo_unpack: null argument");
  cudaStream_t st = (cudaStream_t)stream_;
  const long long rep_bytes = spgg_halo_bytes(h) / h->n_rep;
  const dim3 grid(std::max(1, std::min(64, (GH * h->g.pitchB + 255) / 256)), h->n_rep);
  with_mode(h->mode, [&](auto md) {
    k_halo_unpack<decltype(md)><<<grid, 256, 0, st>>>(h->g, h->d_code[h->cur], h->d_R[h->cur], h->d_S[h->cur],
        (const unsigned char *)from_up, (const unsigned char *)from_down, rep_bytes);
  });
  CUDA_TRY(cudaGetLastError());
  h->launches += 1;
  return SPGG_OK;
}
```

### neighbor-aware-reinforcement-learning-fosters-cooperation-in-spatial-public-goods-games-_b200/csrc/spgg_fast.cuh

```cuda
#pragma once
#include <cuda.h>

#include "spgg_kernels.cuh"

namespace spgg {

constexpr int FTR = 16;
constexpr int FROWB = 160;
constexpr int FROWW = FROWB / 4;
constexpr int FSROWB = 48;
constexpr int FTHREADS = 256;

template <int M>
struct FastSmem {
  static constexpr int kRowsCR = FTR + 2 * M;
  static constexpr int kRowsS = FTR + 4;
  static constexpr int kStageCode = 0;
  static constexpr int kStageR = (kRowsCR * FROWB + 127) / 128 * 128;
  static constexpr int kStageS = kStageR + (kRowsCR * FROWB + 127) / 128 * 128;
  static constexpr int kStageBytes = kStageS + (kRowsS * FSROWB + 127) / 128 * 128;
  static constexpr int kTxBytes = 2 * kRowsCR * FROWB + kRowsS * FSROWB;
  static constexpr int kOutCode = 2 * kStageBytes;
  static constexpr int kOutR = kOutCode + FTR * TC;
  static constexpr int kOutS = kOutR + FTR * TC;
  static constexpr int kOffC = kOutS + 256 + FROWB;
  static constexpr int kOffVal = kOffC + (FTR + 4) * FROWB + FROWB;
  static constexpr int kOffTab = kOffVal + kRowsCR * FROWB * 4;
  static constexpr int kOffBar = kOffTab + 256 * 4;
  static constexpr int kOffFlag = kOffBar + 40 * 8;
  static constexpr int kOffRc = kOffFlag + 16;
  static constexpr int kOffRed = (kOffRc + (int)sizeof(RepConst) + 127) / 128 * 128;
  static constexpr int kRowsPerWarp = FTR / (FTHREADS / 32);
  static constexpr int kQBufs = 2;
  static constexpr int kQBufBytes = kRowsPerWarp * TC * 16;
  static constexpr int kOffQ = (kOffRed + 8 * NSTAT * 8 + 1023) / 1024 * 1024;
  static constexpr int kTotal = kOffQ + (FTHREADS / 32) * kQBufs * kQBufBytes + 1024;
};

__device__ __forceinline__ uint32_t smem_u32(const void *p) {
  return (uint32_t)__cvta_generic_to_shared(p);
}
__device__ __forceinline__ void mbar_init(uint64_t *bar, uint32_t count) {
  asm volatile("mbarrier.init.shared::cta.b64 [%0], %1;" ::"r"(smem_u32(bar)), "r"(count));
}
__device__ __forceinline__ void mbar_expect_tx(uint64_t *bar, uint32_t bytes) {
  asm volatile("mbarrier.arrive.expect_tx.shared::cta.b64 _, [%0], %1;" ::"r"(smem_u32(bar)), "r"(bytes)
               : "memory");
}
__device__ __forceinline__ void mbar_wait(uint64_t *bar, uint32_t parity) {
  uint32_t done;
  uint32_t spins = 0;
  do {
    asm volatile(
        "{\n"
        ".reg .pred p;\n"
        "mbarrier.try_wait.parity.shared::cta.b64 p, [%1], %2;\n"
        "selp.u32 %0, 1, 0, p;\n"
        "}\n"
        : "=r"(done)
        : "r"(smem_u32(bar)), "r"(parity)
        : "memory");
    if (!done && ++spins > (1u << 28)) __trap();
  } while (!done);
}
__device__ __forceinline__ void tma_load_3d(void *dst, const CUtensorMap *map, uint64_t *bar, int c0,
                                            int c1, int c2) {
  asm volatile(
      "cp.async.bulk.tensor.3d.shared::cluster.global.mbarrier::complete_tx::bytes [%0], [%1, {%3, %4, %5}], [%2];"
      ::"r"(smem_u32(dst)), "l"(map), "r"(smem_u32(bar)), "r"(c0), "r"(c1), "r"(c2)
      : "memory");
}

__device__ __forceinline__ void bulk_load_1d(void *dst, const void *src, uint32_t bytes, uint64_t *bar) {
  asm volatile(
      "cp.async.bulk.shared::cluster.global.mbarrier::complete_tx::bytes [%0], [%1], %2, [%3];"
      ::"r"(smem_u32(dst)), "l"(src), "r"(bytes), "r"(smem_u32(bar))
      : "memory");
}
__device__ __forceinline__ void tma_store_3d(const CUtensorMap *map, const void *src, int c0, int c1, int c2) {
  asm volatile("cp.async.bulk.tensor.3d.global.shared::cta.bulk_group [%0, {%2, %3, %4}], [%1];"
               ::"l"(map), "r"(smem_u32(src)), "r"(c0), "r"(c1), "r"(c2)
               : "memory");
}
__device__ __forceinline__ uint64_t l2_evict_first_policy() {
  uint64_t pol;
  asm volatile("createpolicy.fractional.L2::evict_first.b64 %0, 1.0;" : "=l"(pol));
  return pol;
}
__device__ __forceinline__ void tma_load_4d_hint(void *dst, const CUtensorMap *map, uint64_t *bar, int c0,
                                                 int c1, int c2, int c3, uint64_t pol) {
  asm volatile(
      "cp.async.bulk.tensor.4d.shared::cluster.global.mbarrier::complete_tx::bytes.L2::cache_hint"
      " [%0], [%1, {%3, %4, %5, %6}], [%2], %7;"
      ::"r"(smem_u32(dst)), "l"(map), "r"(smem_u32(bar)), "r"(c0), "r"(c1), "r"(c2), "r"(c3), "l"(pol)
      : "memory");
}
__device__ __forceinline__ void tma_store_4d_hint(const CUtensorMap *map, const void *src, int c0, int c1,
                                                  int c2, int c3, uint64_t pol) {
  asm volatile(
      "cp.async.bulk.tensor.4d.global.shared::cta.bulk_group.L2::cache_hint [%0, {%2, %3, %4, %5}], [%1], %6;"
      ::"l"(map), "r"(smem_u32(src)), "r"(c0), "r"(c1), "r"(c2), "r"(c3), "l"(pol)
      : "memory");
}
template <int N>
__device__ __forceinline__ void tma_store_wait_read_n() {
  asm volatile("cp.async.bulk.wait_group.read %0;" ::"n"(N) : "memory");
}
__device__ __forceinline__ void tma_store_commit() { asm volatile("cp.async.bulk.commit_group;" ::: "memory"); }
__device__ __forceinline__ void tma_store_wait_read() { asm volatile("cp.async.bulk.wait_group.read 0;" ::: "memory"); }
__device__ __forceinline__ void tma_store_wait_all() { asm volatile("cp.async.bulk.wait_group 0;" ::: "memory"); }
__device__ __forceinline__ void fence_proxy_async() { asm volatile("fence.proxy.async.shared::cta;" ::: "memory"); }

__device__ __forceinline__ uint32_t sh_l1(uint32_t prev, uint32_t cur) { return __byte_perm(prev, cur, 0x6543); }
__device__ __forceinline__ uint32_t sh_r1(uint32_t cur, uint32_t next) { return __byte_perm(cur, next, 0x4321); }
__device__ __forceinline__ uint32_t sh_2(uint32_t a, uint32_t b) { return __byte_perm(a, b, 0x5432); }

struct FastMaps {
  CUtensorMap ld_code, ld_R, ld_S;
  CUtensorMap st_code, st_R, st_S;
  CUtensorMap q_ld, q_st;
};

template <int M, bool ACTION, bool UPD, bool SEL, bool PART = false>
__device__ __forceinline__ void step_fast_body(const FastMaps &tm, const KArgs &a) {
  typedef FastSmem<M> SM;
  constexpr int NK = (M == 2) ? 12 : 4;
  constexpr bool upd = UPD, sel = SEL;
  const Geom &g = a.g;
  const int rep = blockIdx.x / g.ctas_per_rep, cta = blockIdx.x % g.ctas_per_rep;

  extern __shared__ __align__(1024) unsigned char smem_fast[];
  unsigned char *smem = smem_fast + ((1024u - (smem_u32(smem_fast) & 1023u)) & 1023u);
  uint32_t *wC = reinterpret_cast<uint32_t *>(smem + SM::kOffC);
  float *sm_val = reinterpret_cast<float *>(smem + SM::kOffVal);
  float *sm_tab = reinterpret_cast<float *>(smem + SM::kOffTab);
  float *sm_ratio = sm_tab + 128;
  double *sm_red = reinterpret_cast<double *>(smem + SM::kOffRed);
  uint64_t *bars = reinterpret_cast<uint64_t *>(smem + SM::kOffBar);
  uint8_t *out_code = smem + SM::kOutCode;
  int8_t *out_R = reinterpret_cast<int8_t *>(smem + SM::kOutR);
  uint32_t *out_S = reinterpret_cast<uint32_t *>(smem + SM::kOutS);
  RepConst &s_rc = *reinterpret_cast<RepConst *>(smem + SM::kOffRc);
  int &s_is_last = *reinterpret_cast<int *>(smem + SM::kOffFlag);

  const int tid = threadIdx.x, lane = tid & 31, warp = tid >> 5;
#ifdef SPGG_TRACE
  unsigned long long t_start = 0;
  if (tid == 0) asm volatile("mov.u64 %0, %%globaltimer;" : "=l"(t_start));
#endif
  for (int i = tid; i < (int)(sizeof(RepConst) / 4); i += FTHREADS)
    reinterpret_cast<uint32_t *>(&s_rc)[i] = reinterpret_cast<const uint32_t *>(a.rc + rep)[i];
  if (tid == 0) {
    mbar_init(&bars[0], 1);
    mbar_init(&bars[1], 1);
    asm volatile("fence.mbarrier_init.release.cluster;" ::: "memory");
  }
  __syncthreads();
  for (int i = tid; i < 128; i += FTHREADS) {
    sm_tab[i] = s_rc.rewtab[i];
    sm_ratio[i] = s_rc.ratiotab[i];
  }
  const RepConst &rc = s_rc;

  float4 *Qp = reinterpret_cast<float4 *>(a.Q) + (long long)rep * g.site_stride;

  float inv_den = 0.f, gm_used = 0.f;
  if (upd) {
    gm_used = a.spec ? a.gcarry[rep] : reinterpret_cast<const float *>(a.gmax)[(long long)rep * a.cap + a.rel];
    if (a.spec == 2) gm_used = 123.0f;
    inv_den = __fdiv_rn(1.0f, __fadd_rn(gm_used, rc.leps_f));
  }
  float gbest = 0.f;
  const uint32_t thr = sel ? a.thr_tab[(long long)(a.rel + 1) * g.n_rep + rep] : 0u;
  const float alpha = rc.alpha_f, gamma = rc.gamma_f, kappa = rc.kappa_f;
  const int g31 = min(rc.gain_i, 31), l31 = min(rc.loss_i, 31);
  const uint32_t r_dsum = (uint32_t)(g31 + l31);
  const uint32_t r_k = (uint32_t)(32 - l31) * 0x01010101u;
  const uint32_t r_lo = (uint32_t)(rc.rmin_i + 48) * 0x01010101u, r_hi = (uint32_t)(rc.rmax_i + 48) * 0x01010101u;
  const bool has_ratio = rc.has_ratio != 0;

  uint32_t cls_n[4] = {0, 0, 0, 0}, cls_sn[4] = {0, 0, 0, 0};
  uint32_t grp[6] = {0, 0, 0, 0, 0, 0};
  uint32_t pk_best = 0;
  uint32_t n_sel = 0;
  int sum_r = 0;
  float sq0 = 0.f, sq1 = 0.f, sq2 = 0.f, sq3 = 0.f, sc0 = 0.f, sc1 = 0.f, sc2 = 0.f, sc3 = 0.f;
  float s_ni = 0.f, s_ratio = 0.f;

  const int n_tiles = g.n_tx * g.n_ty;
  const int d_ty = g.ctas_per_rep / g.n_tx, d_tx = g.ctas_per_rep - d_ty * g.n_tx;
  const int d_skew = (d_tx + d_ty) % g.n_tx;
  auto issue = [&](int ty_, int tx_, int st) {
    const int r0 = ty_ * FTR, c0 = tx_ * TC;
    unsigned char *base = smem + st * SM::kStageBytes;
    mbar_expect_tx(&bars[st], SM::kTxBytes);
    tma_load_3d(base + SM::kStageCode, &tm.ld_code, &bars[st], c0, r0 + GH - M, rep);
    tma_load_3d(base + SM::kStageR, &tm.ld_R, &bars[st], c0, r0 + GH - M, rep);
    tma_load_3d(base + SM::kStageS, &tm.ld_S, &bars[st], c0 >> 3, r0 + GH - 2, rep);
  };
  int ty = cta / g.n_tx, txs = cta - ty * g.n_tx;
  int tx = (txs + ty) % g.n_tx;
  if (tid == 0 && cta < n_tiles) issue(ty, tx, 0);

  uint64_t *qbar = bars + 2 + warp * SM::kQBufs;
  unsigned char *sQ = smem + SM::kOffQ + warp * (SM::kQBufs * SM::kQBufBytes);
  const uint64_t pol = l2_evict_first_policy();
  if (lane == 0) {
#pragma unroll
    for (int b = 0; b < SM::kQBufs; ++b) mbar_init(&qbar[b], 1);
    asm volatile("fence.mbarrier_init.release.cluster;" ::: "memory");
  }
  __syncwarp();
  auto q_issue = [&](int col8, int row, int buf) {
    mbar_expect_tx(&qbar[buf], SM::kQBufBytes);
    tma_load_4d_hint(sQ + buf * SM::kQBufBytes, &tm.q_ld, &qbar[buf], 0, col8, row, rep, pol);
  };
  int qoff[4];
#pragma unroll
  for (int k = 0; k < 4; ++k)
    qoff[k] = (lane >> 1) * 128 + ((((lane & 1) * 4 + k) ^ ((lane >> 1) & 7)) << 4);
  if (lane == 0 && cta < n_tiles) q_issue((tx * TC) >> 3, ty * FTR + warp * SM::kRowsPerWarp, 0);

  int tiles_done = 0, stage = 0;
  for (int tile = cta; tile < n_tiles; tile += g.ctas_per_rep, ++tiles_done, stage ^= 1) {
    const int r0 = ty * FTR, c0 = tx * TC;
    int nty = ty + d_ty, ntxs = txs + d_tx, ntx = tx + d_skew;
    if (ntxs >= g.n_tx) { ntxs -= g.n_tx; ++nty; ++ntx; }
    if (ntx >= g.n_tx) ntx -= g.n_tx;
    const bool has_next = tile + g.ctas_per_rep < n_tiles;
    if (tid == 0) {
      if (has_next) issue(nty, ntx, stage ^ 1);
      if (sel) tma_store_wait_read();
    }
    mbar_wait(&bars[stage], (uint32_t)(tiles_done >> 1) & 1u);
    const bool lv = !PART || (c0 + 4 * lane < g.L);
    const uint32_t vm = lv ? 0x01010101u : 0u;
    const unsigned char *st_base = smem + stage * SM::kStageBytes;
    const uint32_t *st_code = reinterpret_cast<const uint32_t *>(st_base + SM::kStageCode);
    const uint32_t *st_R = reinterpret_cast<const uint32_t *>(st_base + SM::kStageR);
    const uint32_t *st_S = reinterpret_cast<const uint32_t *>(st_base + SM::kStageS);

    const int t1 = tid - (FTHREADS - 128);
    if (t1 >= 0 && t1 < (FTR + 4) * 6) {
      const int row = t1 / 6, bw = t1 - row * 6 + 3;
      const uint32_t bits = ~st_S[row * (FSROWB / 4) + bw];
      uint32_t *dst = wC + row * FROWW + (bw - 4) * 8 + 4;
      if (bw == 3) {
        dst[7] = ((bits >> 28) * 0x00204081u) & 0x01010101u;
      } else if (bw == 8) {
        dst[0] = ((bits & 0xFu) * 0x00204081u) & 0x01010101u;
      } else {
        uint4 lo, hi;
        lo.x = (((bits >> 0) & 0xFu) * 0x00204081u) & 0x01010101u;
        lo.y = (((bits >> 4) & 0xFu) * 0x00204081u) & 0x01010101u;
        lo.z = (((bits >> 8) & 0xFu) * 0x00204081u) & 0x01010101u;
        lo.w = (((bits >> 12) & 0xFu) * 0x00204081u) & 0x01010101u;
        hi.x = (((bits >> 16) & 0xFu) * 0x00204081u) & 0x01010101u;
        hi.y = (((bits >> 20) & 0xFu) * 0x00204081u) & 0x01010101u;
        hi.z = (((bits >> 24) & 0xFu) * 0x00204081u) & 0x01010101u;
        hi.w = ((bits >> 28) * 0x00204081u) & 0x01010101u;
        *reinterpret_cast<uint4 *>(dst) = lo;
        *reinterpret_cast<uint4 *>(dst + 4) = hi;
      }
    }
    if (upd) {
      for (int e = tid; e < SM::kRowsCR * FROWW; e += FTHREADS) {
        const uint32_t cw = st_code[e];
        float4 v;
        v.x = sm_tab[(cw >> 1) & 0x7Fu];
        v.y = sm_tab[(cw >> 9) & 0x7Fu];
        v.z = sm_tab[(cw >> 17) & 0x7Fu];
        v.w = sm_tab[(cw >> 25) & 0x7Fu];
        *reinterpret_cast<float4 *>(sm_val + e * 4) = v;
      }
    }
    if (upd) {
      const int t2 = tid - 64;
      if (t2 >= 0 && t2 < FTR * 4 && (!PART || (c0 >> 5) + (t2 & 3) < ((g.L + 31) >> 5))) {
        const int row = (t2 >> 2) + 2, bw = (t2 & 3) + 4;
        const uint32_t *bp = st_S + row * (FSROWB / 4) + bw;
        const uint32_t c = bp[0], u = bp[-(FSROWB / 4)], d = bp[FSROWB / 4];
        const uint32_t l = (c << 1) | (bp[-1] >> 31), r = (c >> 1) | (bp[1] << 31);
        const uint32_t s1 = c ^ u ^ d, c1 = (c & u) | (d & (c | u));
        const uint32_t b0 = s1 ^ l ^ r, c2 = (s1 & l) | (r & (s1 | l));
        const uint32_t b1 = c1 ^ c2, b2 = c1 & c2;
        grp[0] += __popc(~b0 & ~b1 & ~b2); grp[1] += __popc(b0 & ~b1 & ~b2);
        grp[2] += __popc(~b0 & b1 & ~b2);  grp[3] += __popc(b0 & b1 & ~b2);
        grp[4] += __popc(~b0 & ~b1 & b2);  grp[5] += __popc(b0 & ~b1 & b2);
      }
    }
    __syncthreads();
    const uint8_t *bCode = reinterpret_cast<const uint8_t *>(st_code);
    const int qb = stage;
    __syncwarp();
    if (lane == 0) {
      if (upd) tma_store_wait_read_n<0>();
      if (has_next) q_issue((ntx * TC) >> 3, nty * FTR + warp * SM::kRowsPerWarp, qb ^ 1);
    }
    mbar_wait(&qbar[qb], (uint32_t)(tiles_done >> 1) & 1u);
#pragma unroll
    for (int r2 = 0; r2 < SM::kRowsPerWarp; ++r2) {
      const int rr = warp * SM::kRowsPerWarp + r2;
      uint32_t w4[4] = {0, 0, 0, 0};
      if (sel) {
        philox4x32_10_keys((uint32_t)((c0 >> 2) + lane), (uint32_t)(g.row0 + r0 + rr),
                           (uint32_t)(a.j + 1), 0u, s_rc.pkeys, w4);
      }
      const int wo = rr * FROWW + (CPAD / 4) + lane;
      const uint32_t RW = st_R[wo + M * FROWW];
      const uint32_t CW = wC[wo + 2 * FROWW];
      uint32_t StW;
      if constexpr (ACTION) {
        StW = CW;
      } else {
        const uint32_t *rp = st_R + wo + M * FROWW;
        auto bias = [](uint32_t x) { return (x ^ 0x10101010u) & 0x1F1F1F1Fu; };
        const uint32_t c = bias(RW), l = bias(rp[-1]), r = bias(rp[1]);
        const uint32_t u1 = bias(rp[-FROWW]), d1 = bias(rp[FROWW]);
        uint32_t sumA = c + u1 + d1 + sh_l1(l, c) + sh_r1(c, r);
        if constexpr (M == 1) {
          StW = ((sumA + 0x2F2F2F2Fu) >> 7) & 0x01010101u;
        } else {
          const uint32_t ul = bias(rp[-FROWW - 1]), ur = bias(rp[-FROWW + 1]);
          const uint32_t dl = bias(rp[FROWW - 1]), dr = bias(rp[FROWW + 1]);
          const uint32_t sumB = bias(rp[-2 * FROWW]) + bias(rp[2 * FROWW]) + sh_2(l, c) + sh_2(c, r) +
                                sh_l1(ul, u1) + sh_r1(u1, ur) + sh_l1(dl, d1);
          sumA += sh_r1(d1, dr);
          const uint32_t lo = (sumA & 0x00FF00FFu) + (sumB & 0x00FF00FFu);
          const uint32_t hi = ((sumA >> 8) & 0x00FF00FFu) + ((sumB >> 8) & 0x00FF00FFu);
          const uint32_t flo = ((lo + (0x8000u - 209u) * 0x00010001u) >> 15) & 0x00010001u;
          const uint32_t fhi = ((hi + (0x8000u - 209u) * 0x00010001u) >> 15) & 0x00010001u;
          StW = flo | (fhi << 8);
        }
      }
      sum_r = __dp4a((int)RW, (int)vm, sum_r);
      uint32_t codeW = 0;
      float vc[4], vu[4], vd[4], vl[2], vr[2], vu2[4], vd2[4], vul = 0.f, vur = 0.f, vdl = 0.f, vdr = 0.f;
      const int vb = (rr + M) * FROWB + CPAD + 4 * lane;
      if (upd) {
        codeW = st_code[wo + M * FROWW];
        {
          const uint32_t Cb = (codeW >> 2) & 0x01010101u, Ab = (codeW >> 1) & 0x01010101u;
          const uint32_t m3 = Cb & Ab & vm, m2 = (Cb & vm) ^ m3, m1 = (Ab & vm) ^ m3, m0 = vm & ~(Cb | Ab);
          const uint32_t sn = (codeW >> 3) & 0x1F1F1F1Fu;
          cls_n[0] = __dp4a(m0, 0x01010101u, cls_n[0]); cls_sn[0] = __dp4a(sn, m0, cls_sn[0]);
          cls_n[1] = __dp4a(m1, 0x01010101u, cls_n[1]); cls_sn[1] = __dp4a(sn, m1, cls_sn[1]);
          cls_n[2] = __dp4a(m2, 0x01010101u, cls_n[2]); cls_sn[2] = __dp4a(sn, m2, cls_sn[2]);
          cls_n[3] = __dp4a(m3, 0x01010101u, cls_n[3]); cls_sn[3] = __dp4a(sn, m3, cls_sn[3]);
        }
        const float4 c4 = *reinterpret_cast<const float4 *>(sm_val + vb);
        const float4 u4 = *reinterpret_cast<const float4 *>(sm_val + vb - FROWB);
        const float4 d4 = *reinterpret_cast<const float4 *>(sm_val + vb + FROWB);
        vc[0] = c4.x; vc[1] = c4.y; vc[2] = c4.z; vc[3] = c4.w;
        vu[0] = u4.x; vu[1] = u4.y; vu[2] = u4.z; vu[3] = u4.w;
        vd[0] = d4.x; vd[1] = d4.y; vd[2] = d4.z; vd[3] = d4.w;
        if constexpr (M == 2) {
          const float2 l2 = *reinterpret_cast<const float2 *>(sm_val + vb - 2);
          const float2 r2 = *reinterpret_cast<const float2 *>(sm_val + vb + 4);
          vl[0] = l2.x; vl[1] = l2.y; vr[0] = r2.x; vr[1] = r2.y;
          const float4 uu = *reinterpret_cast<const float4 *>(sm_val + vb - 2 * FROWB);
          const float4 dd = *reinterpret_cast<const float4 *>(sm_val + vb + 2 * FROWB);
          vu2[0] = uu.x; vu2[1] = uu.y; vu2[2] = uu.z; vu2[3] = uu.w;
          vd2[0] = dd.x; vd2[1] = dd.y; vd2[2] = dd.z; vd2[3] = dd.w;
          vul = sm_val[vb - FROWB - 1]; vur = sm_val[vb - FROWB + 4];
          vdl = sm_val[vb + FROWB - 1]; vdr = sm_val[vb + FROWB + 4];
        } else {
          vl[0] = 0.f; vl[1] = sm_val[vb - 1]; vr[0] = sm_val[vb + 4]; vr[1] = 0.f;
        }
      }
      unsigned char *qbuf = sQ + qb * SM::kQBufBytes + r2 * (TC * 16);
      uint32_t coopW = 0, rnewW = 0;
      float qfin[4];
      int eidx[4];
      const uint32_t rowoffW = StW << 3;
      const uint32_t coopCW = (codeW >> 1) & 0x01010101u;
      const uint32_t hitW = ~(StW ^ codeW) & 0x01010101u;
      const uint32_t hitCW = hitW & coopCW, hitDW = hitW ^ hitCW;
      if (upd) {
        float qe[4], na[4], nb_[4];
        const uint32_t eoffW = ((codeW & 0x01010101u) << 3) | ((((codeW >> 1) & 0x01010101u) ^ 0x01010101u) << 2);
#pragma unroll
        for (int k = 0; k < 4; ++k) {
          const unsigned char *qs = qbuf + qoff[k];
          eidx[k] = (int)__byte_perm(eoffW, 0, 0x4440 + k);
          qe[k] = *reinterpret_cast<const float *>(qs + eidx[k]);
          const float2 nrow = *reinterpret_cast<const float2 *>(qs + __byte_perm(rowoffW, 0, 0x4440 + k));
          na[k] = nrow.x; nb_[k] = nrow.y;
        }
#pragma unroll
        for (int k = 0; k < 4; ++k) {
          const uint32_t code = (codeW >> (8 * k)) & 0xFFu;
          const float vx = vc[k];
          float nv[NK];
          int no[NK];
          nv[0] = vu[k]; no[0] = -FROWB;
          nv[1] = vd[k]; no[1] = FROWB;
          nv[2] = (k == 0) ? vl[1] : vc[(k + 3) & 3]; no[2] = -1;
          nv[3] = (k == 3) ? vr[0] : vc[(k + 1) & 3]; no[3] = 1;
          if constexpr (M == 2) {
            nv[4] = vu2[k]; no[4] = -2 * FROWB;
            nv[5] = vd2[k]; no[5] = 2 * FROWB;
            nv[6] = (k == 0) ? vl[0] : (k == 1) ? vl[1] : vc[(k + 2) & 3]; no[6] = -2;
            nv[7] = (k == 2) ? vr[0] : (k == 3) ? vr[1] : vc[(k + 2) & 3]; no[7] = 2;
            nv[8] = (k == 0) ? vul : vu[(k + 3) & 3]; no[8] = -FROWB - 1;
            nv[9] = (k == 3) ? vur : vu[(k + 1) & 3]; no[9] = -FROWB + 1;
            nv[10] = (k == 0) ? vdl : vd[(k + 3) & 3]; no[10] = FROWB - 1;
            nv[11] = (k == 3) ? vdr : vd[(k + 1) & 3]; no[11] = FROWB + 1;
          }
          float best = __fsub_rn(nv[0], vx);
          int boff = no[0];
          bool second = false;
#pragma unroll
          for (int q = 1; q < NK; ++q) {
            const float d = __fsub_rn(nv[q], vx);
            if (d > best) { best = d; boff = no[q]; if constexpr (M == 2) second = (q >= 4); }
          }
          if (lv) gbest = fmaxf(gbest, best);
          const bool same = ((((uint32_t)bCode[vb + k + boff] ^ code) >> 1) & 1u) == 0u;
          const float td = __fsub_rn(__fmaf_rn(gamma, fmaxf(na[k], nb_[k]), vx), qe[k]);
          const float qtd = __fmaf_rn(alpha, td, qe[k]);
          const float lam = __fmul_rn(__fmul_rn(kappa, fmaxf(0.0f, best)), inv_den);
          const float nu = same ? lam : -lam;
          const float na2 = ((hitCW >> (8 * k)) & 1u) ? qtd : na[k];
          const float nb2 = ((hitDW >> (8 * k)) & 1u) ? qtd : nb_[k];
          const float td2 = __fsub_rn(__fmaf_rn(gamma, fmaxf(na2, nb2), vx), qtd);
          qfin[k] = __fadd_rn(qtd, nu);
          const float an = fabsf(nu);
          if (lv) {
            s_ni += __fdividef(an, fabsf(alpha * td2) + an + 1e-8f);
            if (has_ratio) s_ratio += sm_ratio[code >> 1];
            if (best > 0.f) pk_best += second ? 0x10001u : 1u;
          }
        }
#pragma unroll
        for (int k = 0; k < 4; ++k) *reinterpret_cast<float *>(qbuf + qoff[k] + eidx[k]) = qfin[k];
#pragma unroll
        for (int k = 0; k < 4; ++k) {
          const float4 qn = *reinterpret_cast<const float4 *>(qbuf + qoff[k]);
          const float m = ((codeW >> (8 * k + 2)) & 1u) ? 1.0f : 0.0f;
          if (lv) {
            sq0 += qn.x; sq1 += qn.y; sq2 += qn.z; sq3 += qn.w;
            sc0 = fmaf(m, qn.x, sc0); sc1 = fmaf(m, qn.y, sc1); sc2 = fmaf(m, qn.z, sc2); sc3 = fmaf(m, qn.w, sc3);
          }
        }
      }
      if (sel) {
#pragma unroll
        for (int k = 0; k < 4; ++k) {
          const float2 grow = *reinterpret_cast<const float2 *>(
              qbuf + qoff[k] + __byte_perm(rowoffW, 0, 0x4440 + k));
          const bool explore = (w4[k] >> 8) < thr;
          const int rnd = (int)(w4[k] & 1u);
          const int greedy = (grow.y > grow.x) ? 1 : 0;
          const int a_new = explore ? rnd : greedy;
          coopW |= (uint32_t)(a_new ^ 1) << (8 * k);
        }
        uint32_t x = ((RW ^ 0x10101010u) & 0x1F1F1F1Fu) + coopW * r_dsum + r_k;
        uint32_t m = ((((x | 0x80808080u) - r_lo) >> 7) & 0x01010101u) * 0xFFu;
        x = (x & m) | (r_lo & ~m);
        m = ((((r_hi | 0x80808080u) - x) >> 7) & 0x01010101u) * 0xFFu;
        x = (x & m) | (r_hi & ~m);
        rnewW = (x + 0x50505050u) ^ 0x80808080u;
      }
      if (sel) {
        const uint32_t *cp = wC + wo + 2 * FROWW;
        const uint32_t cl = cp[-1], cr = cp[1];
        const uint32_t u1 = cp[-FROWW], ul = cp[-FROWW - 1], ur = cp[-FROWW + 1];
        const uint32_t d1 = cp[FROWW], dl = cp[FROWW - 1], dr = cp[FROWW + 1];
        const uint32_t ring = u1 + d1 + sh_l1(cl, CW) + sh_r1(CW, cr) + sh_l1(ul, u1) + sh_r1(u1, ur) +
                              sh_l1(dl, d1) + sh_r1(d1, dr);
        const uint32_t far4 = cp[-2 * FROWW] + cp[2 * FROWW] + sh_2(cl, CW) + sh_2(CW, cr);
        const uint32_t SNW = 5u * CW + 2u * ring + far4;
        const int oo = rr * (TC / 4) + lane;
        reinterpret_cast<uint32_t *>(out_code)[oo] = (SNW << 3) | (CW << 2) | (coopW << 1) | StW;
        reinterpret_cast<uint32_t *>(out_R)[oo] = rnewW;
        const uint32_t nib = lv ? (((coopW * 0x01020408u) >> 24) & 0xFu) : 0u;
        uint32_t coopbits = nib << ((lane & 7) * 4);
        coopbits |= __shfl_xor_sync(0xffffffffu, coopbits, 1);
        coopbits |= __shfl_xor_sync(0xffffffffu, coopbits, 2);
        coopbits |= __shfl_xor_sync(0xffffffffu, coopbits, 4);
        if ((lane & 7) == 0) {
          out_S[rr * 4 + (lane >> 3)] = ~coopbits;
          n_sel += __popc(coopbits);
        }
      }
    }
    if (upd) {
      fence_proxy_async();
      __syncwarp();
      if (lane == 0) {
        tma_store_4d_hint(&tm.q_st, sQ + qb * SM::kQBufBytes, 0, c0 >> 3, r0 + warp * SM::kRowsPerWarp, rep, pol);
        tma_store_commit();
      }
    }
    if (sel) fence_proxy_async();
    __syncthreads();
    if (sel) {
      if (tid == 0) {
        tma_store_3d(&tm.st_code, out_code, CPAD + c0, r0 + GH, rep);
        tma_store_3d(&tm.st_R, out_R, CPAD + c0, r0 + GH, rep);
        if (!PART || c0 + TC <= g.L) tma_store_3d(&tm.st_S, out_S, (WPAD * 4) + (c0 >> 3), r0 + GH, rep);
        tma_store_commit();
      }
      const bool ecol0 = tx == 0, ecol1 = tx == g.n_tx - 1;
      const bool erow0 = g.wrap_rows && ty == 0, erow1 = g.wrap_rows && ty == g.n_ty - 1;
      const bool prow0 = a.peer_code[0] != nullptr && ty == 0, prow1 = a.peer_code[1] != nullptr && ty == g.n_ty - 1;
      const bool edge = ecol0 || ecol1 || erow0 || erow1 || prow0 || prow1;
      if (edge) {
        uint8_t *code_out = reinterpret_cast<uint8_t *>(a.code_out) + (long long)rep * g.plane_stride;
        int8_t *R_out = reinterpret_cast<int8_t *>(a.R_out) + (long long)rep * g.plane_stride;
        uint32_t *S_out = a.S_out + (long long)rep * g.bits_stride;
        for (int e = tid; e < 2 * FTR * GC + 2 * GH * TC; e += FTHREADS) {
          int rr, cc;
          bool on, peer = false;
          int side = 0;
          if (e < 2 * FTR * GC) {
            side = e >= FTR * GC;
            const int q = side ? e - FTR * GC : e;
            rr = q / GC;
            const int wl = PART ? min(TC, g.L - c0) : TC;
            cc = side ? wl - GC + (q % GC) : q % GC;
            on = side ? ecol1 : ecol0;
          } else {
            const int q0 = e - 2 * FTR * GC;
            side = q0 >= GH * TC;
            const int q = side ? q0 - GH * TC : q0;
            rr = side ? FTR - GH + q / TC : q / TC;
            cc = q % TC;
            const bool exists = !PART || c0 + cc < g.L;
            on = exists && (side ? erow1 : erow0);
            peer = exists && (side ? prow1 : prow0);
          }
          const int o = rr * TC + cc;
          if (on) {
            store_cell<uint8_t>(code_out, g, r0 + rr, c0 + cc, out_code[o]);
            store_cell<int8_t>(R_out, g, r0 + rr, c0 + cc, out_R[o]);
          }
          if (peer) {
            const int pi = side ? (rr - FTR) : (a.peer_rows[0] + rr);
            store_cell<uint8_t>(reinterpret_cast<uint8_t *>(a.peer_code[side]), g, pi, c0 + cc, out_code[o]);
            store_cell<int8_t>(reinterpret_cast<int8_t *>(a.peer_R[side]), g, pi, c0 + cc, out_R[o]);
          }
        }
        for (int e = tid; e < FTR * 4; e += FTHREADS) {
          const int rr = e >> 2, wi = (c0 >> 5) + (e & 3);
          if (PART && wi >= ((g.L + 31) >> 5)) continue;
          if (ecol0 || ecol1 || erow0 || erow1) store_bits_word(S_out, g, r0 + rr, wi, out_S[e]);
          if (prow0 && rr < GH) store_bits_word(a.peer_S[0], g, a.peer_rows[0] + rr, wi, out_S[e]);
          if (prow1 && rr >= FTR - GH) store_bits_word(a.peer_S[1], g, rr - FTR, wi, out_S[e]);
        }
        __syncthreads();
      }
    }
    ty = nty; txs = ntxs; tx = ntx;
  }

#ifdef SPGG_TRACE
  if (tid == 0 && a.trace) {
    unsigned long long t_end; unsigned smid;
    asm volatile("mov.u64 %0, %%globaltimer;" : "=l"(t_end));
    asm volatile("mov.u32 %0, %%smid;" : "=r"(smid));
    unsigned long long *tr = a.trace + (size_t)blockIdx.x * 4;
    tr[0] = t_start; tr[1] = t_end; tr[2] = smid; tr[3] = (unsigned long long)tiles_done;
  }
#endif
  double v[NSTAT];
#pragma unroll
  for (int z = 0; z < NSTAT; ++z) v[z] = 0.0;
  const double n0 = (double)cls_n[0], n1 = (double)cls_n[1], n2 = (double)cls_n[2], n3 = (double)cls_n[3];
  v[ST_NC_OLD] = n2 + n3; v[ST_N_CD] = n2; v[ST_N_DC] = n1; v[ST_NC_NEW] = n1 + n3;
  v[ST_SUM_P] = n0; v[ST_SUM_P_C] = n1; v[ST_SUM_P_D] = n2; v[ST_SUM_WP_P] = n3;
#pragma unroll
  for (int z = 0; z < 4; ++z) v[ST_X_SN0 + z] = (double)cls_sn[z];
  v[ST_SUM_RATIO] = (double)s_ratio;
#pragma unroll
  for (int z = 0; z < 6; ++z) v[ST_GROUP0 + z] = (double)grp[z];
  v[ST_SUM_R] = (double)sum_r;
  v[ST_SUM_Q + 0] = (double)sq0; v[ST_SUM_Q + 1] = (double)sq1; v[ST_SUM_Q + 2] = (double)sq2; v[ST_SUM_Q + 3] = (double)sq3;
  v[ST_SUM_Q_C + 0] = (double)sc0; v[ST_SUM_Q_C + 1] = (double)sc1; v[ST_SUM_Q_C + 2] = (double)sc2; v[ST_SUM_Q_C + 3] = (double)sc3;
  v[ST_SUM_NI] = (double)s_ni * 100.0;
  v[ST_N_BEST_POS] = (double)(pk_best & 0xffffu);
  v[ST_N_BEST_2ND] = (double)(pk_best >> 16);
  v[ST_X_NSEL] = (double)n_sel;
  __syncthreads();
  block_reduce_bfly<NSTAT>(v, sm_red);
  double *part = a.partials + ((long long)rep * g.ctas_per_rep + cta) * NSTAT;
  if (tid < NSTAT) part[tid] = sm_red[tid];
  if (a.peer_code[0] != nullptr || a.peer_code[1] != nullptr) __threadfence_system();
  if (upd) {
#pragma unroll
    for (int o = 16; o > 0; o >>= 1) gbest = fmaxf(gbest, __shfl_down_sync(0xffffffffu, gbest, o));
    if (lane == 0) atomicMax(reinterpret_cast<unsigned int *>(const_cast<void *>(a.gmax)) + (long long)rep * a.cap + a.rel,
                             __float_as_uint(gbest));
  }
  __threadfence();
  if (lane == 0 && (upd || (tid == 0 && sel))) tma_store_wait_all();
  __syncthreads();
  if (tid == 0) {
    const unsigned t = atomicInc(a.tickets + rep, (unsigned)g.ctas_per_rep - 1u);
    s_is_last = (t == (unsigned)g.ctas_per_rep - 1u);
  }
  __syncthreads();
  if (!s_is_last) return;
  __threadfence();
  fold_partials(a.partials + (long long)rep * g.ctas_per_rep * NSTAT, g.ctas_per_rep, sm_red);
  if (tid == 0) {
    double *row = a.stats + ((long long)rep * a.cap + a.rel) * NSTAT;
    double *s = sm_red;
    s[ST_SUM_R] *= rc.rq;
    if (upd) {
      double Pc[4];
      const double nc[4] = {s[ST_SUM_P], s[ST_SUM_P_C], s[ST_SUM_P_D], s[ST_SUM_WP_P]};
      for (int z = 0; z < 4; ++z) {
        const double C = (z >> 1) ? 1.0 : 0.0;
        Pc[z] = ((rc.rc * s[ST_X_SN0 + z] / 5.0 - 5.0 * rc.cost * C * nc[z]) - rc.lo * nc[z]) / rc.span;
      }
      s[ST_SUM_P] = Pc[0] + Pc[1] + Pc[2] + Pc[3];
      s[ST_SUM_P_C] = Pc[2] + Pc[3];
      s[ST_SUM_P_D] = Pc[0] + Pc[1];
      s[ST_SUM_WP_P] = rc.wP * s[ST_SUM_P];
      s[ST_SUM_REW_C] = rc.wP * (Pc[1] + Pc[3]) + rc.wR * 0.5 * (nc[1] + nc[3]);
      s[ST_SUM_REW_D] = rc.wP * (Pc[0] + Pc[2]);
      for (int z = 0; z < 4; ++z) s[ST_SUM_Q_D + z] = s[ST_SUM_Q + z] - s[ST_SUM_Q_C + z];
      const float g_exact = __ldcg(reinterpret_cast<const float *>(a.gmax) + (long long)rep * a.cap + a.rel);
      s[ST_GMAX] = (double)g_exact;
      if (a.gvec) {
        a.gvec[4 * a.rel + 0] = g_exact;
      } else {
        if (a.gcarry) a.gcarry[rep] = g_exact;
        if (a.spec && g_exact != gm_used) atomicMin(a.bad_at, a.rel);
      }
      for (int z = 0; z < ST_X_SN0; ++z) row[z] = s[z];
    } else {
      row[ST_SUM_R] = s[ST_SUM_R];
    }
    if (sel && g.wrap_rows) {
      const double nsel = s[ST_X_NSEL];
      if (nsel == 0.0 || nsel == (double)g.site_stride) a.stop_at[rep] = a.j + 1;
    }
    if (a.gvec) {
      const double nsel = s[ST_X_NSEL];
      const float anyD = (sel && nsel == (double)g.site_stride) ? 0.0f : 1.0f;
      const float anyC = (sel && nsel == 0.0) ? 0.0f : 1.0f;
      a.gvec[4 * a.rel + 1] = anyD;
      a.gvec[4 * a.rel + 2] = anyC;
      if (a.ring_world > 0) {
        const unsigned mbits = upd ? __float_as_uint(a.gvec[4 * a.rel + 0]) : 0u;
        const int so = (a.gen & (RING_SLOTS - 1)) * RING_WORDS;
        __threadfence_system();
        for (int p = 0; p < a.ring_world; ++p) {
          unsigned *slot = a.ring_peer[p] + so;
          atomicMax_system(slot + 0, mbits);
          if (anyD != 0.0f) atomicMax_system(slot + 1, 1u);
          if (anyC != 0.0f) atomicMax_system(slot + 2, 1u);
        }
        __threadfence_system();
        for (int p = 0; p < a.ring_world; ++p) atomicAdd_system(a.ring_peer[p] + so + 3, 1u);
      }
    }
  }
}

template <int M, bool ACTION, bool UPD, bool SEL, bool PART = false>
__global__ void __launch_bounds__(FTHREADS, 2)
k_step_fast(const __grid_constant__ FastMaps tm, KArgs a) {
  pdl_launch_dependents();
  pdl_wait();
  const int rep = blockIdx.x / a.g.ctas_per_rep;
  if (a.bad_at && *a.bad_at < a.rel) return;
  const int stop = a.stop_at[rep];
  if (stop >= 0 && a.j > stop) return;
  if (SEL && stop >= 0 && a.j == stop) {
    if constexpr (UPD) step_fast_body<M, ACTION, true, false, PART>(tm, a);
    return;
  }
  step_fast_body<M, ACTION, UPD, SEL, PART>(tm, a);
}

constexpr int GWARPS = 8;
template <int M>
struct GmaxSmem {
  static constexpr int kRowsCR = FTR + 2 * M;
  static constexpr int kStageBytes = (kRowsCR * FROWB + 127) / 128 * 128;
  static constexpr int kOffTab = GWARPS * 2 * kStageBytes;
  static constexpr int kOffBar = kOffTab + 128 * 32 * 4;
  static constexpr int kTotal = kOffBar + GWARPS * 2 * 8 + 128;
};

template <int M>
__global__ void __launch_bounds__(GWARPS * 32, 3)
k_gmax_fast(const __grid_constant__ CUtensorMap ld_code, GArgs a) {
  typedef GmaxSmem<M> SM;
  const Geom &g = a.g;
  const int ctas = gridDim.x / g.n_rep;
  const int rep = blockIdx.x / ctas, cta = blockIdx.x - rep * ctas;
  pdl_launch_dependents();
  extern __shared__ __align__(128) unsigned char smem_gfast[];
  unsigned char *smem = smem_gfast + ((128u - (smem_u32(smem_gfast) & 127u)) & 127u);
  float *tab32 = reinterpret_cast<float *>(smem + SM::kOffTab);
  __shared__ float s_wmax[GWARPS];
  const int tid = threadIdx.x, lane = tid & 31, warp = tid >> 5;
  uint64_t *bars = reinterpret_cast<uint64_t *>(smem + SM::kOffBar) + warp * 2;
  unsigned char *stg = smem + warp * (2 * SM::kStageBytes);
  __shared__ float s_tab[128];
  if (tid < 128) s_tab[tid] = a.rc[rep].rewtab[tid];
  if (lane == 0) {
    mbar_init(&bars[0], 1);
    mbar_init(&bars[1], 1);
    asm volatile("fence.mbarrier_init.release.cluster;" ::: "memory");
  }
  __syncthreads();
  pdl_wait();
  const int stop = a.stop_at[rep];
  if (stop >= 0 && a.j > stop) return;
  if (lane == 0 && cta * GWARPS + warp < g.n_tx * g.n_ty) {
    const int t0 = cta * GWARPS + warp;
    mbar_expect_tx(&bars[0], SM::kRowsCR * FROWB);
    tma_load_3d(stg, &ld_code, &bars[0], (t0 % g.n_tx) * TC, (t0 / g.n_tx) * FTR + GH - M, rep);
  }
#pragma unroll 4
  for (int i = tid; i < 128 * 32; i += GWARPS * 32) tab32[i] = s_tab[i >> 5];
  __syncthreads();
  const float *tl = tab32 + lane;
  const int n_tiles = g.n_tx * g.n_ty;
  const int gw = cta * GWARPS + warp, n_gw = ctas * GWARPS;
  auto issue = [&](int tile, int st) {
    const int r0 = (tile / g.n_tx) * FTR, c0 = (tile % g.n_tx) * TC;
    mbar_expect_tx(&bars[st], SM::kRowsCR * FROWB);
    tma_load_3d(stg + st * SM::kStageBytes, &ld_code, &bars[st], c0, r0 + GH - M, rep);
  };
  float lmax4[4] = {0.f, 0.f, 0.f, 0.f};
  auto upd = [&](int k, float x, float y) { lmax4[k] = fmaxf(lmax4[k], fabsf(__fsub_rn(x, y))); };
  int done = 0, stage = 0;
  for (int tile = gw; tile < n_tiles; tile += n_gw, ++done, stage ^= 1) {
    __syncwarp();
    if (lane == 0 && tile + n_gw < n_tiles) issue(tile + n_gw, stage ^ 1);
    mbar_wait(&bars[stage], (uint32_t)(done >> 1) & 1u);
    const uint32_t *cw = reinterpret_cast<const uint32_t *>(stg + stage * SM::kStageBytes) + (CPAD / 4);
    const bool lv = (tile % g.n_tx) * TC + 4 * lane < g.L;
    float u1[4] = {0.f, 0.f, 0.f, 0.f}, u2[4] = {0.f, 0.f, 0.f, 0.f};
    float u1l = 0.f, u1r = 0.f;
#pragma unroll 3
    for (int s = 0; s < FTR + M; ++s) {
      const uint32_t w = cw[s * FROWW + lane];
      const uint32_t wl = cw[s * FROWW - 1];
      float c[4];
#pragma unroll
      for (int k = 0; k < 4; ++k) c[k] = tl[((w >> (8 * k + 1)) & 0x7Fu) << 5];
      float l1 = __shfl_up_sync(0xffffffffu, c[3], 1);
      const float hl1 = tl[((wl >> 25) & 0x7Fu) << 5];
      if (lane == 0) l1 = hl1;
      float l2 = 0.f, r1 = 0.f;
      if constexpr (M == 2) {
        l2 = __shfl_up_sync(0xffffffffu, c[2], 1);
        const float hl2 = tl[((wl >> 17) & 0x7Fu) << 5];
        if (lane == 0) l2 = hl2;
        const uint32_t wr = cw[s * FROWW + 32];
        r1 = __shfl_down_sync(0xffffffffu, c[0], 1);
        const float hr1 = tl[((wr >> 1) & 0x7Fu) << 5];
        if (lane == 31) r1 = hr1;
      }
      if (s >= M && lv) {
#pragma unroll
        for (int k = 0; k < 4; ++k) {
          upd(k, u1[k], c[k]);
          upd(k, k == 0 ? l1 : c[(k + 3) & 3], c[k]);
          if constexpr (M == 2) {
            upd(k, u2[k], c[k]);
            upd(k, k == 0 ? l2 : (k == 1 ? l1 : c[(k + 2) & 3]), c[k]);
            upd(k, k == 0 ? u1l : u1[(k + 3) & 3], c[k]);
            upd(k, k == 3 ? u1r : u1[(k + 1) & 3], c[k]);
          }
        }
      }
#pragma unroll
      for (int k = 0; k < 4; ++k) { u2[k] = u1[k]; u1[k] = c[k]; }
      u1l = l1; u1r = r1;
    }
  }
  float lmax = fmaxf(fmaxf(lmax4[0], lmax4[1]), fmaxf(lmax4[2], lmax4[3]));
#pragma unroll
  for (int o = 16; o > 0; o >>= 1) lmax = fmaxf(lmax, __shfl_down_sync(0xffffffffu, lmax, o));
  if (lane == 0) s_wmax[warp] = lmax;
  __syncthreads();
  if (tid == 0) {
    float m = s_wmax[0];
    for (int w = 1; w < GWARPS; ++w) m = fmaxf(m, s_wmax[w]);
    atomicMax(reinterpret_cast<unsigned int *>(a.gmax) + (long long)rep * a.cap + a.rel, __float_as_uint(m));
  }
}

}
```

Baseline: 129.1 billion.

## Run chunks of iterations in one cooperative persistent launch with grid sync

After: 132.2 billion (median of 6 runs). 2.3% higher.

```diff
diff --git a/neighbor-aware-reinforcement-learning-fosters-cooperation-in-spatial-public-goods-games-_b200/csrc/spgg_capi.cu b/neighbor-aware-reinforcement-learning-fosters-cooperation-in-spatial-public-goods-games-_b200/csrc/spgg_capi.cu
--- a/neighbor-aware-reinforcement-learning-fosters-cooperation-in-spatial-public-goods-games-_b200/csrc/spgg_capi.cu
+++ b/neighbor-aware-reinforcement-learning-fosters-cooperation-in-spatial-public-goods-games-_b200/csrc/spgg_capi.cu
@@ -67,6 +67,10 @@
   long long spec_launches = 0, spec_failures = 0;
   long long spec_iterations = 0;
   bool in_rerun = false;
+  bool persist = false;
+  const char *persist_off = nullptr;
+  double *d_chunk_part = nullptr;
+  unsigned *d_nsel = nullptr;
   float *d_gvec = nullptr;
   void *peer_code[2][2] = {{nullptr, nullptr}, {nullptr, nullptr}};
   void *peer_R[2][2] = {{nullptr, nullptr}, {nullptr, nullptr}};
@@ -237,6 +241,11 @@
   return action ? pick_fast2<1, true>(upd, sel, part) : pick_fast2<1, false>(upd, sel, part);
 }
 static size_t fast_smem(int M) { return M == 2 ? FastSmem<2>::kTotal : FastSmem<1>::kTotal; }
+typedef void (*chunk_fn_t)(const FastMaps, const FastMaps, KArgs, const ChunkArgs);
+static chunk_fn_t pick_chunk(int action, bool part) {
+  if (action) return part ? k_chunk_fast<1, true, true> : k_chunk_fast<1, true, false>;
+  return part ? k_chunk_fast<1, false, true> : k_chunk_fast<1, false, false>;
+}
 typedef void (*gfast_fn_t)(const CUtensorMap, GArgs);
 static gfast_fn_t pick_gfast(int M) { return M == 2 ? k_gmax_fast<2> : k_gmax_fast<1>; }
 static size_t gfast_smem(int M) { return M == 2 ? GmaxSmem<2>::kTotal : GmaxSmem<1>::kTotal; }
@@ -322,6 +331,7 @@
 spgg_handle::~spgg_handle() {
   for (void *p : ipc_opened) cudaIpcCloseMemHandle(p);
   cudaFree(d_rc); cudaFree(d_valtab); cudaFree(d_Qb[0]); cudaFree(d_Qb[1]); cudaFree(d_gcarry); cudaFree(d_bad); cudaFree(d_gvec); cudaFree(d_ring);
+  cudaFree(d_chunk_part); cudaFree(d_nsel);
   for (int i = 0; i < 2; ++i) { cudaFree(d_R[i]); cudaFree(d_code[i]); cudaFree(d_S[i]); }
   cudaFree(d_gmax); cudaFree(d_stats); cudaFree(d_partials); cudaFree(d_tickets);
   cudaFree(d_stop); cudaFree(d_eps); cudaFree(d_thr); cudaFree(d_u); cudaFree(d_b);
@@ -511,6 +521,16 @@
   }
   if (h->fast && (g.site_stride / ((long long)g.ctas_per_rep * FTHREADS)) > 60000) h->fast = false;
   h->spec = h->fast && getenv("SPGG_NO_SPEC") == nullptr;
+  if (h->spec && n_replicas == 1 && g.wrap_rows && h->M == 1 && getenv("SPGG_NO_PERSIST") == nullptr) {
+    const chunk_fn_t cf = pick_chunk(h->action, g.L % TC != 0);
+    int coop = 0, occ_c = 0;
+    CUDA_TRY(cudaDeviceGetAttribute(&coop, cudaDevAttrCooperativeLaunch, device));
+    CUDA_TRY(cudaFuncSetAttribute(cf, cudaFuncAttributeMaxDynamicSharedMemorySize, (int)fast_smem(h->M)));
+    CUDA_TRY(cudaOccupancyMaxActiveBlocksPerMultiprocessor(&occ_c, cf, FTHREADS, fast_smem(h->M)));
+    if (!coop) h->persist_off = "no cooperative launch on this device";
+    else if ((long long)occ_c * prop.multiProcessorCount < g.ctas_per_rep) h->persist_off = "k_chunk_fast grid not co-resident";
+    else h->persist = true;
+  }
 
   const size_t nQ = (size_t)n_replicas * g.site_stride * h->nq() * h->elem_Q();
   const size_t nR = (size_t)n_replicas * g.plane_stride * h->elem_R();
@@ -530,6 +550,7 @@
   ALLOC(h->d_partials, sizeof(double) * (size_t)n_replicas * g.ctas_per_rep * NSTAT);
   ALLOC(h->d_tickets, sizeof(unsigned) * n_replicas);
   ALLOC(h->d_stop, sizeof(int) * n_replicas);
+  if (h->persist) ALLOC(h->d_chunk_part, sizeof(double) * (size_t)CHUNK_MAX * g.ctas_per_rep * NSTAT);
   if (h->res_grid) {
     ALLOC(h->d_gimg, (size_t)h->rgeo.CS * 6 * h->rgeo.prow * h->rgeo.pitch);
     ALLOC(h->d_gpart, sizeof(double) * (size_t)RES_RING * h->rgeo.CS * RES_NRED);
@@ -819,14 +840,15 @@
 static int ensure_tables(spgg_handle *h, int n_steps) {
   const int need = n_steps + 1;
   if (need <= h->cap) return SPGG_OK;
-  cudaFree(h->d_gmax); cudaFree(h->d_stats); cudaFree(h->d_eps); cudaFree(h->d_thr); cudaFree(h->d_gvec);
-  h->d_gmax = nullptr; h->d_stats = nullptr; h->d_eps = nullptr; h->d_thr = nullptr; h->d_gvec = nullptr;
+  cudaFree(h->d_gmax); cudaFree(h->d_stats); cudaFree(h->d_eps); cudaFree(h->d_thr); cudaFree(h->d_gvec); cudaFree(h->d_nsel);
+  h->d_gmax = nullptr; h->d_stats = nullptr; h->d_eps = nullptr; h->d_thr = nullptr; h->d_gvec = nullptr; h->d_nsel = nullptr;
   h->cap = 0;
   CUDA_TRY(cudaMalloc(&h->d_gmax, h->elem_val() * (size_t)h->n_rep * need));
   CUDA_TRY(cudaMalloc((void **)&h->d_stats, sizeof(double) * (size_t)h->n_rep * need * NSTAT));
   CUDA_TRY(cudaMalloc((void **)&h->d_eps, sizeof(double) * (size_t)h->n_rep * (need + 1)));
   CUDA_TRY(cudaMalloc((void **)&h->d_thr, sizeof(uint32_t) * (size_t)h->n_rep * (need + 1)));
   if (h->spec && !h->g.wrap_rows) CUDA_TRY(cudaMalloc((void **)&h->d_gvec, sizeof(float) * 4 * (size_t)need));
+  if (h->persist) CUDA_TRY(cudaMalloc((void **)&h->d_nsel, sizeof(unsigned) * (size_t)need));
   h->cap = need;
   return SPGG_OK;
 }
@@ -889,6 +911,11 @@
 static bool can_speculate(const spgg_handle *h, int do_select) {
   return h->fast && h->spec && h->spec_on && h->carry_valid &&
          !launch_replays(h, h->pend_t0 + h->pend_rel + 1, do_select);
+}
+
+static int spec_test_poison() {
+  static const int poison = getenv("SPGG_SPEC_TEST_POISON") ? atoi(getenv("SPGG_SPEC_TEST_POISON")) : 0;
+  return poison;
 }
 
 static int launch_step(spgg_handle *h, int do_update, int do_select, cudaStream_t st, bool allow_spec) {
@@ -964,7 +991,7 @@
     fm.q_ld = h->qmaps[h->qcur];
     fm.q_st = h->qmaps[q_out];
     if (a.spec) {
-      static const int poison = getenv("SPGG_SPEC_TEST_POISON") ? atoi(getenv("SPGG_SPEC_TEST_POISON")) : 0;
+      const int poison = spec_test_poison();
       if (poison > 0 && !h->in_rerun && h->spec_launches % poison == poison - 1) a.spec = 2;
     }
     CUDA_TRY(launch_pdl(ff, h->g.ctas_per_rep * h->n_rep, FTHREADS, fast_smem(h->M), st, fm, a));
@@ -1126,6 +1153,65 @@
   return SPGG_OK;
 }
 
+static int chunk_launch(spgg_handle *h, int s, int last, cudaStream_t st, bool *ran) {
+  *ran = false;
+  const int n_idx = last - s + 1;
+  KArgs a = {};
+  a.g = h->g;
+  a.rc = h->d_rc;
+  a.gmax = h->d_gmax; a.stats = h->d_stats; a.stop_at = h->d_stop; a.thr_tab = h->d_thr;
+  a.j = (int)(h->pend_t0 + s); a.rel = s; a.cap = h->cap;
+  a.gcarry = h->d_gcarry; a.bad_at = h->d_bad;
+  ChunkArgs c;
+  c.rel_end = last;
+  c.n_steps = h->pend_n;
+  c.poison = h->in_rerun ? 0 : spec_test_poison();
+  c.poison_off = c.poison > 0 ? (int)(h->spec_launches % c.poison) : 0;
+  const int cur = h->cur, qcur = h->qcur;
+  c.out0 = FastOut{h->d_code[cur ^ 1], h->d_R[cur ^ 1], h->d_S[cur ^ 1]};
+  c.out1 = FastOut{h->d_code[cur], h->d_R[cur], h->d_S[cur]};
+  c.ring = h->d_chunk_part;
+  c.nsel = h->d_nsel;
+  FastMaps tm[2] = {h->fmaps[cur], h->fmaps[cur ^ 1]};
+  const int u0 = s == 0 ? 1 : 0;
+  tm[u0].q_ld = h->qmaps[qcur];     tm[u0].q_st = h->qmaps[qcur ^ 1];
+  tm[u0 ^ 1].q_ld = h->qmaps[qcur ^ 1]; tm[u0 ^ 1].q_st = h->qmaps[qcur];
+  CUDA_TRY(cudaMemsetAsync(h->d_nsel + s, 0, sizeof(unsigned) * (size_t)n_idx, st));
+  cudaLaunchConfig_t cfg = {};
+  cfg.gridDim = dim3((unsigned)h->g.ctas_per_rep);
+  cfg.blockDim = dim3((unsigned)FTHREADS);
+  cfg.dynamicSmemBytes = fast_smem(h->M);
+  cfg.stream = st;
+  cudaLaunchAttribute attr[1];
+  attr[0].id = cudaLaunchAttributeCooperative;
+  attr[0].val.cooperative = 1;
+  cfg.attrs = attr;
+  cfg.numAttrs = 1;
+  if (cudaLaunchKernelEx(&cfg, pick_chunk(h->action, h->g.L % TC != 0), tm[0], tm[1], a, c) != cudaSuccess) {
+    (void)cudaGetLastError();
+    h->persist = false;
+    h->persist_off = "cooperative chunk launch refused";
+    return SPGG_OK;
+  }
+  k_chunk_rows<<<n_idx, FTHREADS, 0, st>>>(a, h->d_chunk_part);
+  CUDA_TRY(cudaGetLastError());
+  *ran = true;
+  h->launches += 2;
+  for (int r = s; r <= last; ++r) {
+    if (r > 0) {
+      h->qcur ^= 1;
+      h->spec_launches += 1;
+      if (!h->in_rerun) h->spec_iterations += 1;
+    }
+    if (r < h->pend_n) h->cur ^= 1;
+    h->pend_cur_after[r] = (char)h->cur;
+    h->pend_q_after[r] = (char)h->qcur;
+  }
+  h->carry_valid = true;
+  h->pend_rel = last;
+  return SPGG_OK;
+}
+
 extern "C" int spgg_step(spgg_t *h, int n_steps, void *stream_) {
   int rcode = spgg_begin_steps(h, n_steps, stream_);
   if (rcode) return rcode;
@@ -1134,8 +1220,18 @@
     if (rcode) return rcode;
     return spgg_end_steps(h, stream_);
   }
-  rcode = spgg_phase_kernel(h, 0, 1, stream_);
-  for (int s = 1; s <= n_steps && !rcode; ++s) rcode = spgg_phase_iteration(h, s < n_steps ? 1 : 0, stream_);
+  const bool chunked = n_steps >= 2 && !h->d_u;
+  for (int s = 0; s <= n_steps && !rcode;) {
+    if (chunked && s < n_steps && h->persist && h->spec_on && h->carry_valid && !h->r_wide) {
+      const int last = std::min(n_steps, s + CHUNK_MAX - 1);
+      bool ran = false;
+      rcode = chunk_launch(h, s, last, (cudaStream_t)stream_, &ran);
+      if (ran) s = last + 1;
+      if (ran || rcode) continue;
+    }
+    rcode = s == 0 ? spgg_phase_kernel(h, 0, 1, stream_) : spgg_phase_iteration(h, s < n_steps ? 1 : 0, stream_);
+    ++s;
+  }
   if (rcode) return rcode;
   return spgg_end_steps(h, stream_);
 }
@@ -1170,7 +1266,7 @@
 
 extern "C" int spgg_describe(spgg_t *h, char *buf, int n) {
   if (!h) return fail(SPGG_E_INVALID, "null handle");
-  char tmp[256];
+  char tmp[384];
   const char *arith = h->mode == MODE_F64 ? "fp64 Q and R" : (h->mode == MODE_F32_F ? "fp32 Q, fp32 R" : "fp32 Q, int8 R");
   int len;
   if (h->resident && h->res_grid)
@@ -1179,11 +1275,16 @@
   else if (h->resident)
     len = snprintf(tmp, sizeof(tmp), "resident: cluster of %d CTAs x %d threads per replica, %zu KB shared memory per CTA, "
                    "ghost rows through DSMEM (%s)", h->rgeo.CS, h->rgeo.threads, h->smem_res >> 10, arith);
+  else if (h->fast && h->persist && h->spec_on)
+    len = snprintf(tmp, sizeof(tmp), "fast: TMA-staged %dx%d tiles, %d persistent CTAs per replica, up to %d iterations "
+                   "per cooperative launch (k_chunk_fast, speculative global maximum, verified) (%s)",
+                   FTR, TC, h->g.ctas_per_rep, CHUNK_MAX, arith);
   else if (h->fast)
-    len = snprintf(tmp, sizeof(tmp), "fast: TMA-staged %dx%d tiles, %d persistent CTAs per replica, %s (%s)",
+    len = snprintf(tmp, sizeof(tmp), "fast: TMA-staged %dx%d tiles, %d persistent CTAs per replica, %s (%s)%s%s",
                    FTR, TC, h->g.ctas_per_rep,
                    (h->spec && h->spec_on) ? "one launch per iteration (speculative global maximum, verified)"
-                                           : "two launches per iteration (k_gmax_fast + k_step_fast)", arith);
+                                           : "two launches per iteration (k_gmax_fast + k_step_fast)", arith,
+                   h->persist_off ? "; whole-chunk launch off: " : "", h->persist_off ? h->persist_off : "");
   else
     len = snprintf(tmp, sizeof(tmp), "general: %dx%d tiles, %d CTAs per replica, two launches per iteration (k_gmax_lean + %s) (%s)", h->g.TR, TC,
                    h->g.ctas_per_rep, h->lean ? "k_step_lean" : "k_step", arith);
diff --git a/neighbor-aware-reinforcement-learning-fosters-cooperation-in-spatial-public-goods-games-_b200/csrc/spgg_fast.cuh b/neighbor-aware-reinforcement-learning-fosters-cooperation-in-spatial-public-goods-games-_b200/csrc/spgg_fast.cuh
--- a/neighbor-aware-reinforcement-learning-fosters-cooperation-in-spatial-public-goods-games-_b200/csrc/spgg_fast.cuh
+++ b/neighbor-aware-reinforcement-learning-fosters-cooperation-in-spatial-public-goods-games-_b200/csrc/spgg_fast.cuh
@@ -1,4 +1,5 @@
 #pragma once
+#include <cooperative_groups.h>
 #include <cuda.h>
 
 #include "spgg_kernels.cuh"
@@ -110,6 +111,7 @@
 __device__ __forceinline__ void tma_store_wait_read() { asm volatile("cp.async.bulk.wait_group.read 0;" ::: "memory"); }
 __device__ __forceinline__ void tma_store_wait_all() { asm volatile("cp.async.bulk.wait_group 0;" ::: "memory"); }
 __device__ __forceinline__ void fence_proxy_async() { asm volatile("fence.proxy.async.shared::cta;" ::: "memory"); }
+__device__ __forceinline__ void fence_proxy_async_global() { asm volatile("fence.proxy.async.global;" ::: "memory"); }
 
 __device__ __forceinline__ uint32_t sh_l1(uint32_t prev, uint32_t cur) { return __byte_perm(prev, cur, 0x6543); }
 __device__ __forceinline__ uint32_t sh_r1(uint32_t cur, uint32_t next) { return __byte_perm(cur, next, 0x4321); }
@@ -121,64 +123,38 @@
   CUtensorMap q_ld, q_st;
 };
 
-template <int M, bool ACTION, bool UPD, bool SEL, bool PART = false>
-__device__ __forceinline__ void step_fast_body(const FastMaps &tm, const KArgs &a) {
+__device__ __forceinline__ unsigned char *fast_smem_base() {
+  extern __shared__ __align__(1024) unsigned char smem_fast[];
+  return smem_fast + ((1024u - (smem_u32(smem_fast) & 1023u)) & 1023u);
+}
+
+template <int M>
+__device__ __forceinline__ void fast_prologue(const RepConst *rc_g) {
   typedef FastSmem<M> SM;
-  constexpr int NK = (M == 2) ? 12 : 4;
-  constexpr bool upd = UPD, sel = SEL;
-  const Geom &g = a.g;
-  const int rep = blockIdx.x / g.ctas_per_rep, cta = blockIdx.x % g.ctas_per_rep;
-
-  extern __shared__ __align__(1024) unsigned char smem_fast[];
-  unsigned char *smem = smem_fast + ((1024u - (smem_u32(smem_fast) & 1023u)) & 1023u);
-  uint32_t *wC = reinterpret_cast<uint32_t *>(smem + SM::kOffC);
-  float *sm_val = reinterpret_cast<float *>(smem + SM::kOffVal);
+  unsigned char *smem = fast_smem_base();
   float *sm_tab = reinterpret_cast<float *>(smem + SM::kOffTab);
-  float *sm_ratio = sm_tab + 128;
-  double *sm_red = reinterpret_cast<double *>(smem + SM::kOffRed);
   uint64_t *bars = reinterpret_cast<uint64_t *>(smem + SM::kOffBar);
-  uint8_t *out_code = smem + SM::kOutCode;
-  int8_t *out_R = reinterpret_cast<int8_t *>(smem + SM::kOutR);
-  uint32_t *out_S = reinterpret_cast<uint32_t *>(smem + SM::kOutS);
   RepConst &s_rc = *reinterpret_cast<RepConst *>(smem + SM::kOffRc);
-  int &s_is_last = *reinterpret_cast<int *>(smem + SM::kOffFlag);
-
   const int tid = threadIdx.x, lane = tid & 31, warp = tid >> 5;
-#ifdef SPGG_TRACE
-  unsigned long long t_start = 0;
-  if (tid == 0) asm volatile("mov.u64 %0, %%globaltimer;" : "=l"(t_start));
-#endif
   for (int i = tid; i < (int)(sizeof(RepConst) / 4); i += FTHREADS)
-    reinterpret_cast<uint32_t *>(&s_rc)[i] = reinterpret_cast<const uint32_t *>(a.rc + rep)[i];
+    reinterpret_cast<uint32_t *>(&s_rc)[i] = reinterpret_cast<const uint32_t *>(rc_g)[i];
   if (tid == 0) {
     mbar_init(&bars[0], 1);
     mbar_init(&bars[1], 1);
-    asm volatile("fence.mbarrier_init.release.cluster;" ::: "memory");
-  }
+  }
+  if (lane == 0) {
+#pragma unroll
+    for (int b = 0; b < SM::kQBufs; ++b) mbar_init(&bars[2 + warp * SM::kQBufs + b], 1);
+  }
+  if (tid == 0 || lane == 0) asm volatile("fence.mbarrier_init.release.cluster;" ::: "memory");
   __syncthreads();
   for (int i = tid; i < 128; i += FTHREADS) {
     sm_tab[i] = s_rc.rewtab[i];
-    sm_ratio[i] = s_rc.ratiotab[i];
-  }
-  const RepConst &rc = s_rc;
-
-  float4 *Qp = reinterpret_cast<float4 *>(a.Q) + (long long)rep * g.site_stride;
-
-  float inv_den = 0.f, gm_used = 0.f;
-  if (upd) {
-    gm_used = a.spec ? a.gcarry[rep] : reinterpret_cast<const float *>(a.gmax)[(long long)rep * a.cap + a.rel];
-    if (a.spec == 2) gm_used = 123.0f;
-    inv_den = __fdiv_rn(1.0f, __fadd_rn(gm_used, rc.leps_f));
-  }
-  float gbest = 0.f;
-  const uint32_t thr = sel ? a.thr_tab[(long long)(a.rel + 1) * g.n_rep + rep] : 0u;
-  const float alpha = rc.alpha_f, gamma = rc.gamma_f, kappa = rc.kappa_f;
-  const int g31 = min(rc.gain_i, 31), l31 = min(rc.loss_i, 31);
-  const uint32_t r_dsum = (uint32_t)(g31 + l31);
-  const uint32_t r_k = (uint32_t)(32 - l31) * 0x01010101u;
-  const uint32_t r_lo = (uint32_t)(rc.rmin_i + 48) * 0x01010101u, r_hi = (uint32_t)(rc.rmax_i + 48) * 0x01010101u;
-  const bool has_ratio = rc.has_ratio != 0;
-
+    sm_tab[128 + i] = s_rc.ratiotab[i];
+  }
+}
+
+struct FastAcc {
   uint32_t cls_n[4] = {0, 0, 0, 0}, cls_sn[4] = {0, 0, 0, 0};
   uint32_t grp[6] = {0, 0, 0, 0, 0, 0};
   uint32_t pk_best = 0;
@@ -186,6 +162,54 @@
   int sum_r = 0;
   float sq0 = 0.f, sq1 = 0.f, sq2 = 0.f, sq3 = 0.f, sc0 = 0.f, sc1 = 0.f, sc2 = 0.f, sc3 = 0.f;
   float s_ni = 0.f, s_ratio = 0.f;
+  float gbest = 0.f;
+};
+
+struct FastOut {
+  void *code, *R;
+  uint32_t *S;
+};
+
+template <int M, bool ACTION, bool UPD, bool SEL, bool PART>
+__device__ __forceinline__ void fast_tiles(const FastMaps &tm, const CUtensorMap &q_ld, const FastOut &out,
+                                           const KArgs &a, int j, int rel, float gm_used, FastAcc &acc,
+                                           int &tiles_done) {
+  typedef FastSmem<M> SM;
+  constexpr int NK = (M == 2) ? 12 : 4;
+  constexpr bool upd = UPD, sel = SEL;
+  const Geom &g = a.g;
+  const int rep = blockIdx.x / g.ctas_per_rep, cta = blockIdx.x % g.ctas_per_rep;
+
+  unsigned char *smem = fast_smem_base();
+  uint32_t *wC = reinterpret_cast<uint32_t *>(smem + SM::kOffC);
+  float *sm_val = reinterpret_cast<float *>(smem + SM::kOffVal);
+  float *sm_tab = reinterpret_cast<float *>(smem + SM::kOffTab);
+  float *sm_ratio = sm_tab + 128;
+  uint64_t *bars = reinterpret_cast<uint64_t *>(smem + SM::kOffBar);
+  uint8_t *out_code = smem + SM::kOutCode;
+  int8_t *out_R = reinterpret_cast<int8_t *>(smem + SM::kOutR);
+  uint32_t *out_S = reinterpret_cast<uint32_t *>(smem + SM::kOutS);
+  const RepConst &rc = *reinterpret_cast<const RepConst *>(smem + SM::kOffRc);
+  const RepConst &s_rc = rc;
+  const int tid = threadIdx.x, lane = tid & 31, warp = tid >> 5;
+
+  float inv_den = 0.f;
+  if (upd) inv_den = __fdiv_rn(1.0f, __fadd_rn(gm_used, rc.leps_f));
+  float &gbest = acc.gbest;
+  const uint32_t thr = sel ? a.thr_tab[(long long)(rel + 1) * g.n_rep + rep] : 0u;
+  const float alpha = rc.alpha_f, gamma = rc.gamma_f, kappa = rc.kappa_f;
+  const int g31 = min(rc.gain_i, 31), l31 = min(rc.loss_i, 31);
+  const uint32_t r_dsum = (uint32_t)(g31 + l31);
+  const uint32_t r_k = (uint32_t)(32 - l31) * 0x01010101u;
+  const uint32_t r_lo = (uint32_t)(rc.rmin_i + 48) * 0x01010101u, r_hi = (uint32_t)(rc.rmax_i + 48) * 0x01010101u;
+  const bool has_ratio = rc.has_ratio != 0;
+
+  uint32_t (&cls_n)[4] = acc.cls_n, (&cls_sn)[4] = acc.cls_sn, (&grp)[6] = acc.grp;
+  uint32_t &pk_best = acc.pk_best, &n_sel = acc.n_sel;
+  int &sum_r = acc.sum_r;
+  float &sq0 = acc.sq0, &sq1 = acc.sq1, &sq2 = acc.sq2, &sq3 = acc.sq3;
+  float &sc0 = acc.sc0, &sc1 = acc.sc1, &sc2 = acc.sc2, &sc3 = acc.sc3;
+  float &s_ni = acc.s_ni, &s_ratio = acc.s_ratio;
 
   const int n_tiles = g.n_tx * g.n_ty;
   const int d_ty = g.ctas_per_rep / g.n_tx, d_tx = g.ctas_per_rep - d_ty * g.n_tx;
@@ -200,28 +224,22 @@
   };
   int ty = cta / g.n_tx, txs = cta - ty * g.n_tx;
   int tx = (txs + ty) % g.n_tx;
-  if (tid == 0 && cta < n_tiles) issue(ty, tx, 0);
+  int stage = tiles_done & 1;
+  if (tid == 0 && cta < n_tiles) issue(ty, tx, stage);
 
   uint64_t *qbar = bars + 2 + warp * SM::kQBufs;
   unsigned char *sQ = smem + SM::kOffQ + warp * (SM::kQBufs * SM::kQBufBytes);
   const uint64_t pol = l2_evict_first_policy();
-  if (lane == 0) {
-#pragma unroll
-    for (int b = 0; b < SM::kQBufs; ++b) mbar_init(&qbar[b], 1);
-    asm volatile("fence.mbarrier_init.release.cluster;" ::: "memory");
-  }
-  __syncwarp();
   auto q_issue = [&](int col8, int row, int buf) {
     mbar_expect_tx(&qbar[buf], SM::kQBufBytes);
-    tma_load_4d_hint(sQ + buf * SM::kQBufBytes, &tm.q_ld, &qbar[buf], 0, col8, row, rep, pol);
+    tma_load_4d_hint(sQ + buf * SM::kQBufBytes, &q_ld, &qbar[buf], 0, col8, row, rep, pol);
   };
   int qoff[4];
 #pragma unroll
   for (int k = 0; k < 4; ++k)
     qoff[k] = (lane >> 1) * 128 + ((((lane & 1) * 4 + k) ^ ((lane >> 1) & 7)) << 4);
-  if (lane == 0 && cta < n_tiles) q_issue((tx * TC) >> 3, ty * FTR + warp * SM::kRowsPerWarp, 0);
-
-  int tiles_done = 0, stage = 0;
+  if (lane == 0 && cta < n_tiles) q_issue((tx * TC) >> 3, ty * FTR + warp * SM::kRowsPerWarp, stage);
+
   for (int tile = cta; tile < n_tiles; tile += g.ctas_per_rep, ++tiles_done, stage ^= 1) {
     const int r0 = ty * FTR, c0 = tx * TC;
     int nty = ty + d_ty, ntxs = txs + d_tx, ntx = tx + d_skew;
@@ -304,7 +322,7 @@
       uint32_t w4[4] = {0, 0, 0, 0};
       if (sel) {
         philox4x32_10_keys((uint32_t)((c0 >> 2) + lane), (uint32_t)(g.row0 + r0 + rr),
-                           (uint32_t)(a.j + 1), 0u, s_rc.pkeys, w4);
+                           (uint32_t)(j + 1), 0u, s_rc.pkeys, w4);
       }
       const int wo = rr * FROWW + (CPAD / 4) + lane;
       const uint32_t RW = st_R[wo + M * FROWW];
@@ -507,9 +525,9 @@
       const bool prow0 = a.peer_code[0] != nullptr && ty == 0, prow1 = a.peer_code[1] != nullptr && ty == g.n_ty - 1;
       const bool edge = ecol0 || ecol1 || erow0 || erow1 || prow0 || prow1;
       if (edge) {
-        uint8_t *code_out = reinterpret_cast<uint8_t *>(a.code_out) + (long long)rep * g.plane_stride;
-        int8_t *R_out = reinterpret_cast<int8_t *>(a.R_out) + (long long)rep * g.plane_stride;
-        uint32_t *S_out = a.S_out + (long long)rep * g.bits_stride;
+        uint8_t *code_out = reinterpret_cast<uint8_t *>(out.code) + (long long)rep * g.plane_stride;
+        int8_t *R_out = reinterpret_cast<int8_t *>(out.R) + (long long)rep * g.plane_stride;
+        uint32_t *S_out = out.S + (long long)rep * g.bits_stride;
         for (int e = tid; e < 2 * FTR * GC + 2 * GH * TC; e += FTHREADS) {
           int rr, cc;
           bool on, peer = false;
@@ -554,6 +572,85 @@
     }
     ty = nty; txs = ntxs; tx = ntx;
   }
+}
+
+__device__ __forceinline__ void fast_cta_stats(const FastAcc &acc, double *sm_red) {
+  double v[NSTAT];
+#pragma unroll
+  for (int z = 0; z < NSTAT; ++z) v[z] = 0.0;
+  const double n0 = (double)acc.cls_n[0], n1 = (double)acc.cls_n[1], n2 = (double)acc.cls_n[2], n3 = (double)acc.cls_n[3];
+  v[ST_NC_OLD] = n2 + n3; v[ST_N_CD] = n2; v[ST_N_DC] = n1; v[ST_NC_NEW] = n1 + n3;
+  v[ST_SUM_P] = n0; v[ST_SUM_P_C] = n1; v[ST_SUM_P_D] = n2; v[ST_SUM_WP_P] = n3;
+#pragma unroll
+  for (int z = 0; z < 4; ++z) v[ST_X_SN0 + z] = (double)acc.cls_sn[z];
+  v[ST_SUM_RATIO] = (double)acc.s_ratio;
+#pragma unroll
+  for (int z = 0; z < 6; ++z) v[ST_GROUP0 + z] = (double)acc.grp[z];
+  v[ST_SUM_R] = (double)acc.sum_r;
+  v[ST_SUM_Q + 0] = (double)acc.sq0; v[ST_SUM_Q + 1] = (double)acc.sq1; v[ST_SUM_Q + 2] = (double)acc.sq2; v[ST_SUM_Q + 3] = (double)acc.sq3;
+  v[ST_SUM_Q_C + 0] = (double)acc.sc0; v[ST_SUM_Q_C + 1] = (double)acc.sc1; v[ST_SUM_Q_C + 2] = (double)acc.sc2; v[ST_SUM_Q_C + 3] = (double)acc.sc3;
+  v[ST_SUM_NI] = (double)acc.s_ni * 100.0;
+  v[ST_N_BEST_POS] = (double)(acc.pk_best & 0xffffu);
+  v[ST_N_BEST_2ND] = (double)(acc.pk_best >> 16);
+  v[ST_X_NSEL] = (double)acc.n_sel;
+  __syncthreads();
+  block_reduce_bfly<NSTAT>(v, sm_red);
+}
+
+__device__ __forceinline__ void fast_gmax_atomic(float gbest, unsigned *slot) {
+#pragma unroll
+  for (int o = 16; o > 0; o >>= 1) gbest = fmaxf(gbest, __shfl_down_sync(0xffffffffu, gbest, o));
+  if ((threadIdx.x & 31) == 0) atomicMax(slot, __float_as_uint(gbest));
+}
+
+__device__ __forceinline__ void fast_finish_row(double *s, double *row, const RepConst &rc, bool upd, float g_exact) {
+  s[ST_SUM_R] *= rc.rq;
+  if (upd) {
+    double Pc[4];
+    const double nc[4] = {s[ST_SUM_P], s[ST_SUM_P_C], s[ST_SUM_P_D], s[ST_SUM_WP_P]};
+    for (int z = 0; z < 4; ++z) {
+      const double C = (z >> 1) ? 1.0 : 0.0;
+      Pc[z] = ((rc.rc * s[ST_X_SN0 + z] / 5.0 - 5.0 * rc.cost * C * nc[z]) - rc.lo * nc[z]) / rc.span;
+    }
+    s[ST_SUM_P] = Pc[0] + Pc[1] + Pc[2] + Pc[3];
+    s[ST_SUM_P_C] = Pc[2] + Pc[3];
+    s[ST_SUM_P_D] = Pc[0] + Pc[1];
+    s[ST_SUM_WP_P] = rc.wP * s[ST_SUM_P];
+    s[ST_SUM_REW_C] = rc.wP * (Pc[1] + Pc[3]) + rc.wR * 0.5 * (nc[1] + nc[3]);
+    s[ST_SUM_REW_D] = rc.wP * (Pc[0] + Pc[2]);
+    for (int z = 0; z < 4; ++z) s[ST_SUM_Q_D + z] = s[ST_SUM_Q + z] - s[ST_SUM_Q_C + z];
+    s[ST_GMAX] = (double)g_exact;
+    for (int z = 0; z < ST_X_SN0; ++z) row[z] = s[z];
+  } else {
+    row[ST_SUM_R] = s[ST_SUM_R];
+  }
+}
+
+template <int M, bool ACTION, bool UPD, bool SEL, bool PART = false>
+__device__ __forceinline__ void step_fast_body(const FastMaps &tm, const KArgs &a) {
+  typedef FastSmem<M> SM;
+  constexpr bool upd = UPD, sel = SEL;
+  const Geom &g = a.g;
+  const int rep = blockIdx.x / g.ctas_per_rep, cta = blockIdx.x % g.ctas_per_rep;
+  unsigned char *smem = fast_smem_base();
+  double *sm_red = reinterpret_cast<double *>(smem + SM::kOffRed);
+  const RepConst &rc = *reinterpret_cast<const RepConst *>(smem + SM::kOffRc);
+  int &s_is_last = *reinterpret_cast<int *>(smem + SM::kOffFlag);
+  const int tid = threadIdx.x, lane = tid & 31;
+#ifdef SPGG_TRACE
+  unsigned long long t_start = 0;
+  if (tid == 0) asm volatile("mov.u64 %0, %%globaltimer;" : "=l"(t_start));
+#endif
+  fast_prologue<M>(a.rc + rep);
+  float gm_used = 0.f;
+  if (upd) {
+    gm_used = a.spec ? a.gcarry[rep] : reinterpret_cast<const float *>(a.gmax)[(long long)rep * a.cap + a.rel];
+    if (a.spec == 2) gm_used = 123.0f;
+  }
+  FastAcc acc;
+  int tiles_done = 0;
+  fast_tiles<M, ACTION, UPD, SEL, PART>(tm, tm.q_ld, FastOut{a.code_out, a.R_out, a.S_out}, a, a.j, a.rel, gm_used,
+                                        acc, tiles_done);
 
 #ifdef SPGG_TRACE
   if (tid == 0 && a.trace) {
@@ -564,35 +661,11 @@
     tr[0] = t_start; tr[1] = t_end; tr[2] = smid; tr[3] = (unsigned long long)tiles_done;
   }
 #endif
-  double v[NSTAT];
-#pragma unroll
-  for (int z = 0; z < NSTAT; ++z) v[z] = 0.0;
-  const double n0 = (double)cls_n[0], n1 = (double)cls_n[1], n2 = (double)cls_n[2], n3 = (double)cls_n[3];
-  v[ST_NC_OLD] = n2 + n3; v[ST_N_CD] = n2; v[ST_N_DC] = n1; v[ST_NC_NEW] = n1 + n3;
-  v[ST_SUM_P] = n0; v[ST_SUM_P_C] = n1; v[ST_SUM_P_D] = n2; v[ST_SUM_WP_P] = n3;
-#pragma unroll
-  for (int z = 0; z < 4; ++z) v[ST_X_SN0 + z] = (double)cls_sn[z];
-  v[ST_SUM_RATIO] = (double)s_ratio;
-#pragma unroll
-  for (int z = 0; z < 6; ++z) v[ST_GROUP0 + z] = (double)grp[z];
-  v[ST_SUM_R] = (double)sum_r;
-  v[ST_SUM_Q + 0] = (double)sq0; v[ST_SUM_Q + 1] = (double)sq1; v[ST_SUM_Q + 2] = (double)sq2; v[ST_SUM_Q + 3] = (double)sq3;
-  v[ST_SUM_Q_C + 0] = (double)sc0; v[ST_SUM_Q_C + 1] = (double)sc1; v[ST_SUM_Q_C + 2] = (double)sc2; v[ST_SUM_Q_C + 3] = (double)sc3;
-  v[ST_SUM_NI] = (double)s_ni * 100.0;
-  v[ST_N_BEST_POS] = (double)(pk_best & 0xffffu);
-  v[ST_N_BEST_2ND] = (double)(pk_best >> 16);
-  v[ST_X_NSEL] = (double)n_sel;
-  __syncthreads();
-  block_reduce_bfly<NSTAT>(v, sm_red);
+  fast_cta_stats(acc, sm_red);
   double *part = a.partials + ((long long)rep * g.ctas_per_rep + cta) * NSTAT;
   if (tid < NSTAT) part[tid] = sm_red[tid];
   if (a.peer_code[0] != nullptr || a.peer_code[1] != nullptr) __threadfence_system();
-  if (upd) {
-#pragma unroll
-    for (int o = 16; o > 0; o >>= 1) gbest = fmaxf(gbest, __shfl_down_sync(0xffffffffu, gbest, o));
-    if (lane == 0) atomicMax(reinterpret_cast<unsigned int *>(const_cast<void *>(a.gmax)) + (long long)rep * a.cap + a.rel,
-                             __float_as_uint(gbest));
-  }
+  if (upd) fast_gmax_atomic(acc.gbest, reinterpret_cast<unsigned int *>(const_cast<void *>(a.gmax)) + (long long)rep * a.cap + a.rel);
   __threadfence();
   if (lane == 0 && (upd || (tid == 0 && sel))) tma_store_wait_all();
   __syncthreads();
@@ -605,34 +678,16 @@
   __threadfence();
   fold_partials(a.partials + (long long)rep * g.ctas_per_rep * NSTAT, g.ctas_per_rep, sm_red);
   if (tid == 0) {
-    double *row = a.stats + ((long long)rep * a.cap + a.rel) * NSTAT;
     double *s = sm_red;
-    s[ST_SUM_R] *= rc.rq;
+    const float g_exact = upd ? __ldcg(reinterpret_cast<const float *>(a.gmax) + (long long)rep * a.cap + a.rel) : 0.f;
+    fast_finish_row(s, a.stats + ((long long)rep * a.cap + a.rel) * NSTAT, rc, upd, g_exact);
     if (upd) {
-      double Pc[4];
-      const double nc[4] = {s[ST_SUM_P], s[ST_SUM_P_C], s[ST_SUM_P_D], s[ST_SUM_WP_P]};
-      for (int z = 0; z < 4; ++z) {
-        const double C = (z >> 1) ? 1.0 : 0.0;
-        Pc[z] = ((rc.rc * s[ST_X_SN0 + z] / 5.0 - 5.0 * rc.cost * C * nc[z]) - rc.lo * nc[z]) / rc.span;
-      }
-      s[ST_SUM_P] = Pc[0] + Pc[1] + Pc[2] + Pc[3];
-      s[ST_SUM_P_C] = Pc[2] + Pc[3];
-      s[ST_SUM_P_D] = Pc[0] + Pc[1];
-      s[ST_SUM_WP_P] = rc.wP * s[ST_SUM_P];
-      s[ST_SUM_REW_C] = rc.wP * (Pc[1] + Pc[3]) + rc.wR * 0.5 * (nc[1] + nc[3]);
-      s[ST_SUM_REW_D] = rc.wP * (Pc[0] + Pc[2]);
-      for (int z = 0; z < 4; ++z) s[ST_SUM_Q_D + z] = s[ST_SUM_Q + z] - s[ST_SUM_Q_C + z];
-      const float g_exact = __ldcg(reinterpret_cast<const float *>(a.gmax) + (long long)rep * a.cap + a.rel);
-      s[ST_GMAX] = (double)g_exact;
       if (a.gvec) {
         a.gvec[4 * a.rel + 0] = g_exact;
       } else {
         if (a.gcarry) a.gcarry[rep] = g_exact;
         if (a.spec && g_exact != gm_used) atomicMin(a.bad_at, a.rel);
       }
-      for (int z = 0; z < ST_X_SN0; ++z) row[z] = s[z];
-    } else {
-      row[ST_SUM_R] = s[ST_SUM_R];
     }
     if (sel && g.wrap_rows) {
       const double nsel = s[ST_X_NSEL];
@@ -675,6 +730,118 @@
     return;
   }
   step_fast_body<M, ACTION, UPD, SEL, PART>(tm, a);
+}
+
+constexpr int CHUNK_MAX = 128;
+
+struct ChunkArgs {
+  int rel_end;
+  int n_steps;
+  int poison, poison_off;
+  FastOut out0, out1;
+  double *ring;
+  unsigned *nsel;
+};
+
+template <int M, bool ACTION, bool PART>
+__global__ void __launch_bounds__(FTHREADS, 2)
+k_chunk_fast(const __grid_constant__ FastMaps tm0, const __grid_constant__ FastMaps tm1, KArgs a,
+             const __grid_constant__ ChunkArgs c) {
+  typedef FastSmem<M> SM;
+  cooperative_groups::grid_group grid = cooperative_groups::this_grid();
+  const Geom &g = a.g;
+  const int cta = blockIdx.x, tid = threadIdx.x, lane = tid & 31;
+  if (__ldcg(a.bad_at) < a.rel) return;
+  unsigned char *smem = fast_smem_base();
+  double *sm_red = reinterpret_cast<double *>(smem + SM::kOffRed);
+  volatile int *s_loop = reinterpret_cast<volatile int *>(smem + SM::kOffFlag);
+  if (tid == 0) {
+    s_loop[0] = a.rel;
+    s_loop[1] = __ldcg(a.stop_at);
+  }
+  fast_prologue<M>(a.rc);
+  const int rel_upd0 = max(a.rel, 1);
+  struct It { int rel, i, j; bool upd, sel; };
+  auto it_of = [&](int rel, int stop) {
+    It t;
+    t.rel = rel; t.i = rel - a.rel; t.j = a.j + t.i;
+    t.upd = rel > 0;
+    t.sel = rel < c.n_steps && !(stop >= 0 && t.j == stop);
+    return t;
+  };
+  int tiles_done = 0;
+  for (;;) {
+    It t = it_of(s_loop[0], s_loop[1]);
+    if (t.rel > c.rel_end || (s_loop[1] >= 0 && t.j > s_loop[1])) break;
+    if (!t.upd && !t.sel) {
+      __syncthreads();
+      if (tid == 0) s_loop[0] = t.rel + 1;
+      __syncthreads();
+      continue;
+    }
+    float gm_used = 0.f;
+    if (t.upd) {
+      gm_used = t.rel == rel_upd0 ? __ldcg(a.gcarry) : __ldcg(reinterpret_cast<const float *>(a.gmax) + t.rel - 1);
+      if (c.poison > 0 && (c.poison_off + t.rel - rel_upd0) % c.poison == c.poison - 1) gm_used = 123.0f;
+      if (tid == 0) s_loop[2] = __float_as_int(gm_used);
+    }
+    FastAcc acc;
+    {
+      const FastMaps &tm = (t.i & 1) ? tm1 : tm0;
+      const FastOut &out = (t.i & 1) ? c.out1 : c.out0;
+      if (t.upd && t.sel) fast_tiles<M, ACTION, true, true, PART>(tm, tm.q_ld, out, a, t.j, t.rel, gm_used, acc, tiles_done);
+      else if (t.upd) fast_tiles<M, ACTION, true, false, PART>(tm, tm.q_ld, out, a, t.j, t.rel, gm_used, acc, tiles_done);
+      else fast_tiles<M, ACTION, false, true, PART>(tm, tm1.q_ld, out, a, t.j, t.rel, 0.f, acc, tiles_done);
+    }
+    t = it_of(s_loop[0], s_loop[1]);
+    fast_cta_stats(acc, sm_red);
+    if (tid < NSTAT) c.ring[((long long)t.i * g.ctas_per_rep + cta) * NSTAT + tid] = sm_red[tid];
+    if (t.upd) fast_gmax_atomic(acc.gbest, reinterpret_cast<unsigned *>(const_cast<void *>(a.gmax)) + t.rel);
+    if (t.sel && tid == 0) atomicAdd(c.nsel + t.rel, (unsigned)sm_red[ST_X_NSEL]);
+    if (lane == 0 && (t.upd || (tid == 0 && t.sel))) tma_store_wait_all();
+    fence_proxy_async_global();
+    grid.sync();
+    fence_proxy_async_global();
+
+    bool bad = false;
+    int stop = s_loop[1];
+    if (t.upd) {
+      const float exact = __ldcg(reinterpret_cast<const float *>(a.gmax) + t.rel);
+      bad = exact != __int_as_float(s_loop[2]);
+      if (cta == 0 && tid == 0) {
+        *a.gcarry = exact;
+        if (bad) atomicMin(a.bad_at, t.rel);
+      }
+    }
+    if (t.sel) {
+      const unsigned ns = __ldcg(c.nsel + t.rel);
+      if (ns == 0u || ns == (unsigned)g.site_stride) {
+        stop = t.j + 1;
+        if (cta == 0 && tid == 0) *a.stop_at = stop;
+      }
+    }
+    if (bad) break;
+    if (tid == 0) {
+      s_loop[0] = t.rel + 1;
+      s_loop[1] = stop;
+    }
+    __syncthreads();
+  }
+}
+
+__global__ void __launch_bounds__(FTHREADS)
+k_chunk_rows(KArgs a, const double *ring) {
+  __shared__ double sm_red[8 * NSTAT];
+  const int i = blockIdx.x, rel = a.rel + i, j = a.j + i;
+  if (__ldcg(a.bad_at) < rel) return;
+  const int stop = __ldcg(a.stop_at);
+  if (stop >= 0 && (j > stop || (rel == 0 && j == stop))) return;
+  fold_partials(ring + (long long)i * a.g.ctas_per_rep * NSTAT, a.g.ctas_per_rep, sm_red);
+  if (threadIdx.x == 0) {
+    const bool upd = rel > 0;
+    const float g_exact = upd ? __ldcg(reinterpret_cast<const float *>(a.gmax) + rel) : 0.f;
+    fast_finish_row(sm_red, a.stats + (long long)rel * NSTAT, *a.rc, upd, g_exact);
+  }
 }
 
 constexpr int GWARPS = 8;
```
